# winlaic/ZipVoice

Hardware: AMD Instinct MI355X
Metric: generated mel-frames/s (whole job) + RTF, ZipVoice 123M N_steps=16 batch=32/GPU (higher is better)
Workload: dtype bf16; 1 GPU; C2: ZipVoice 123M, N_steps=16, batch=32/GPU x (3 s prompt + 10 s generated; T=1219 frames), CFG g=1.0 (64 decoder rows per GPU), t_shift=0.5; model=zipvoice (zipvoice_base.json, synthetic seeded weights), global_batch=32, seq_len=1219, parallelism=dp1

## Files before the change

### include/zipvoice_hip.h

```cpp
#ifndef ZIPVOICE_HIP_H
#define ZIPVOICE_HIP_H

#include <stdint.h>

#ifdef __cplusplus
extern "C" {
#endif

typedef struct zv_engine* zv_handle;

enum zv_variant { ZV_ZIPVOICE = 0, ZV_DISTILL = 1, ZV_DIALOG = 2, ZV_DIALOG_STEREO = 3 };
enum zv_precision { ZV_FP32 = 0, ZV_BF16 = 1, ZV_MIXED = 2, ZV_FP8 = 3 };

#define ZV_MAX_STACKS 8

typedef struct {
  int variant;
  int precision;
  int feat_dim;
  int num_stacks;
  int downsampling_factor[ZV_MAX_STACKS];
  int num_layers[ZV_MAX_STACKS];
  int cnn_module_kernel[ZV_MAX_STACKS];
  int fm_decoder_dim, fm_decoder_feedforward_dim, fm_decoder_num_heads;
  int text_encoder_num_layers, text_encoder_feedforward_dim, text_encoder_cnn_module_kernel;
  int text_encoder_num_heads, text_encoder_dim;
  int time_embed_dim, text_embed_dim;
  int query_head_dim, value_head_dim, pos_head_dim, pos_dim;
  int vocab_size, pad_id, spk_a_id, spk_b_id;
} zv_config;

const char* zv_last_error(void);
const char* zv_version(void);

zv_handle zv_create(const zv_config* cfg);
void zv_destroy(zv_handle h);

int zv_set_weight(zv_handle h, const char* name, const float* host_data, int64_t numel);
int zv_finalize(zv_handle h);
int zv_reserve(zv_handle h, int max_batch, int max_frames);
int64_t zv_device_bytes(zv_handle h);

int zv_profile(int enable);
int zv_profile_report(char* buf, int buflen);

int64_t zv_host_block_count(void);

int zv_attn_fallbacks(zv_handle h, int reset, int64_t* host_counts);

int zv_attn2_check(int kernel, int form, int B, int L, int H, int nv, const float* qkp, const float* P,
                   const uint8_t* key_pad, const float* v, const float* y, int force_exact, float* out,
                   int64_t* counts);

int zv_bench_gemm(int M, int N, int K, int variant, int iters, int out_mode, float* ms_out);

int zv_gemm_selftest(int M, int N, int K, int variant, int mode, float* maxdiff, float* maxref);

enum zv_linear_form {
  ZV_LIN_PLAIN = 0,
  ZV_LIN_PLAIN_F32 = 1,
  ZV_LIN_RESID = 2,
  ZV_LIN_RESID_BYP = 3,
  ZV_LIN_RESID_RV = 4,
  ZV_LIN_RESID_RV_COPY = 5,
  ZV_LIN_TRANS = 6,
  ZV_LIN_NA = 7,
  ZV_LIN_GLU = 8,
  ZV_LIN_GLU_DW = 9
};
typedef struct {
  int M, N, K, split, form, act;
  int rows_per_group;
  int rpb;
  int guard;
  const float* A; const float* W; const float* bias;
  const float* resid;
  const float* orig;
  const float* byp;
  const float* rowvec;
  const uint8_t* rowmask;
  const float* dw_w;
  const float* dw_b;
  int dw_ks, dw_L;
  float* C; int64_t ldc;
  uint16_t* Ch; uint16_t* Cl; int64_t ldch;
  uint16_t* Cth; uint16_t* Ctl; int64_t ldct;
  int launch[8];
  int num_cus;
} zv_linear_check_args;
int zv_linear_check(zv_linear_check_args* a);

typedef struct {
  int M, H, form, rows_per_group, part_slots, guard;
  float log_scale;
  const float* x; const float* W1; const float* b1; const float* W2; const float* b2;
  const float* resid;
  const float* rowvec;
  const float* orig;
  const float* byp;
  const float* nb;
  float* C; int64_t ldc;
  uint16_t* Ch; uint16_t* Cl; uint16_t* C2h; uint16_t* C2l; int64_t ldch;
  int launch[8];
  int num_cus;
} zv_ffn_check_args;
int zv_ffn_check(zv_ffn_check_args* a);

typedef struct {
  int B, L, C, ks, split, guard;
  const float* g; const float* w; const float* bias;
  int64_t ldin;
  uint16_t* Oh; uint16_t* Ol; int64_t ldout;
  uint8_t* q; uint8_t* qs; int64_t ldq;
  int launch[8];
  int num_cus;
} zv_dwconv_check_args;
int zv_dwconv_check(zv_dwconv_check_args* a);

enum zv_stackedge_kind { ZV_SE_DOWNSAMPLE = 0, ZV_SE_UPSAMPLE = 1, ZV_SE_MASK = 2, ZV_SE_ENTRY = 3, ZV_SE_BIASNORM = 4 };
typedef struct {
  int kind, B, L, C, ds, guard, rows_per_group;
  float log_scale;
  const float* x; const float* w; const float* nb; const float* orig; const float* rowvec;
  const uint8_t* mask;
  float* out;
  uint8_t* mout;
  uint16_t* h; uint16_t* l; uint16_t* h2; uint16_t* l2; int64_t ldact;
  uint8_t* q2; uint8_t* qs2; int64_t ldq;
  int launch[8];
  int num_cus;
} zv_stackedge_check_args;
int zv_stackedge_check(zv_stackedge_check_args* a);

enum zv_bigvgan_check_kind { ZV_BV_FILTER = 0, ZV_BV_ACT = 1, ZV_BV_CONV = 2, ZV_BV_CONVT = 3, ZV_BV_AVG = 4,
                             ZV_BV_POST = 5, ZV_BV_IM2COL = 6, ZV_BV_STEP = 7 };
typedef struct {
  int kind, split, mode, guard;
  int B, Lmax, Ls, halo, scale;
  int C, Cout, ks, d, u, n, layout, flag;
  float div, sub, bias0;
  unsigned stale;
  const int* lens;
  const float* x; const float* x1; const float* x2;
  const float* w; const float* bias; const float* alpha; const float* ibeta;
  const float* w2; const float* bias2; const float* alpha2; const float* ibeta2;
  const float* taps; const float* resid;
  const uint16_t* ah; const uint16_t* al;
  float* out; uint16_t* oh; uint16_t* ol; int64_t ld;
  int launch[8];
  int num_cus;
} zv_bigvgan_check_args;
int zv_bigvgan_check(zv_bigvgan_check_args* a);

int zv_attn_plan(int split, int sa_plo, int tpm, int L, int nv_na, int64_t* lds_sa, int64_t* lds_na,
                 int64_t* lds_stats, int* fits);

int zv_mx8_quantize(const float* x, int rows, int K, uint8_t* q, uint8_t* s);
int zv_mx8_gemm_check(int M, int N, int K, const float* A, const float* W, float* C, uint8_t* Aq,
                      uint8_t* As);

int zv_fm_decoder(zv_handle h, const float* t, const float* guidance, const float* xt,
                  const float* text_c, const float* speech_c, const uint8_t* pad, int N,
                  int T, int Fx, float* v_out, void* stream);

int zv_velocity(zv_handle h, float t, float guidance_scale, const float* x,
                const float* text_c, const float* speech_c, const uint8_t* pad, int B, int T,
                float* v_out, void* stream);

int zv_euler_sample(zv_handle h, float* x, const float* text_c, const float* speech_c,
                    const uint8_t* pad, int B, int T, int num_step, float guidance_scale,
                    float t_start, float t_end, float t_shift, void* stream);

int zv_velocity_rows(zv_handle h, float t, const float* guidance_rows, const float* x,
                     const float* text_c, const float* speech_c, const uint8_t* pad, int B,
                     int T, float* v_out, void* stream);
int zv_euler_sample_rows(zv_handle h, float* x, const float* text_c, const float* speech_c,
                         const uint8_t* pad, int B, int T, int num_step,
                         const float* guidance_rows, float t_start, float t_end,
                         float t_shift, void* stream);

int zv_text_encode(zv_handle h, const int64_t* tokens, const uint8_t* pad,
                   const int8_t* spk, int B, int S, float* out, void* stream);

int zv_text_condition(zv_handle h, const float* embed, int B, int S, const int32_t* tok_lens,
                      const int32_t* feat_lens, int T, float* out, void* stream);

int zv_speech_condition(zv_handle h, const float* prompt, int B, int Tp, int F,
                        const int32_t* prompt_lens, int T, float* out, void* stream);

typedef struct zv_vocoder* zv_vocoder_handle;

typedef struct {
  int precision;
  int n_mels;
  int dim;
  int intermediate_dim;
  int num_layers;
  int n_fft;
  int hop;
  int embed_kernel;
  int dw_kernel;
} zv_vocoder_config;

zv_vocoder_handle zv_vocoder_create(const zv_vocoder_config* cfg);
void zv_vocoder_destroy(zv_vocoder_handle v);
int zv_vocoder_set_weight(zv_vocoder_handle v, const char* name, const float* host_data,
                          int64_t numel);
int zv_vocoder_finalize(zv_vocoder_handle v);
int zv_vocoder_decode(zv_vocoder_handle v, const float* mel, int layout, float feat_scale,
                      float feat_bias, const int32_t* lens, int B, int T, float* wav, int clamp,
                      void* stream);
int64_t zv_vocoder_device_bytes(zv_vocoder_handle v);

typedef struct zv_bigvgan* zv_bigvgan_handle;

typedef struct {
  int precision;
  int num_mels;
  int upsample_initial_channel;
  int num_upsamples;
  int upsample_rates[8];
  int upsample_kernel_sizes[8];
  int num_kernels;
  int resblock_kernel_sizes[3];
  int resblock_dilation_sizes[3][3];
  int snake_logscale;
  int use_tanh_at_final;
  int use_bias_at_final;
} zv_bigvgan_config;

zv_bigvgan_handle zv_bigvgan_create(const zv_bigvgan_config* cfg);
void zv_bigvgan_destroy(zv_bigvgan_handle v);
int zv_bigvgan_set_weight(zv_bigvgan_handle v, const char* name, const float* host_data,
                          int64_t numel);
int zv_bigvgan_finalize(zv_bigvgan_handle v);
int zv_bigvgan_decode(zv_bigvgan_handle v, const float* mel, int layout, float feat_scale,
                      float feat_bias, const int32_t* lens, int B, int T, float* wav,
                      void* stream);
int64_t zv_bigvgan_device_bytes(zv_bigvgan_handle v);

typedef struct zv_fbank* zv_fbank_handle;
zv_fbank_handle zv_fbank_create(int n_fft, int hop, int n_mels, const float* host_window,
                                const float* host_fb);
void zv_fbank_destroy(zv_fbank_handle f);
int zv_fbank_configure(zv_fbank_handle f, int frame_offset, float mag_eps, float log_floor);
int zv_fbank_extract(zv_fbank_handle f, const float* wav, int64_t wav_ld, const int32_t* lens,
                     int B, int T_out, float* out, int64_t out_ld, void* stream);

typedef struct zv_resample* zv_resample_handle;
zv_resample_handle zv_resample_create(int o, int n, int S, const int32_t* host_start,
                                      const float* host_table);
void zv_resample_destroy(zv_resample_handle h);
int zv_resample_apply(zv_resample_handle h, const float* wav, int64_t wav_ld, const int32_t* lens,
                      int R, float* out, int64_t out_ld, int64_t out_cols, void* stream);
int64_t zv_resample_device_bytes(zv_resample_handle h);

typedef struct zv_wavjoin* zv_wavjoin_handle;
// ... 16 lines not shown
```

### zipvoice_amd/csrc/zv_checks.inc

```
#pragma once

namespace {

struct ChkDev {
  std::vector<void*> ptrs;
  void* raw(size_t bytes) {
    void* p = nullptr;
    ZV_CHECK(ZV_BLOCKING(hipMalloc(&p, bytes + 256)));
    ptrs.push_back(p);
    return p;
  }
  template <typename T> T* make(size_t n) { return reinterpret_cast<T*>(raw(n * sizeof(T))); }
  template <typename T> T* zero(size_t n) {
    T* d = make<T>(n);
    ZV_CHECK(ZV_BLOCKING(hipMemset(d, 0, n * sizeof(T))));
    return d;
  }
  template <typename T> T* up(const T* host, size_t n) {
    T* d = make<T>(n);
    ZV_CHECK(ZV_BLOCKING(hipMemcpy(d, host, n * sizeof(T), hipMemcpyHostToDevice)));
    return d;
  }
  template <typename T> void down(T* host, const T* dev, size_t n) {
    ZV_CHECK(ZV_BLOCKING(hipMemcpy(host, dev, n * sizeof(T), hipMemcpyDeviceToHost)));
// ... 302 lines not shown
  p.Bh = reinterpret_cast<const bf16*>(dWq); p.ldb = K; p.Bs = dWs; p.ldbs = K / MX8_BLOCK;
  p.bias = dev.zero<float>((size_t)N); p.C = dC; p.ldc = N; p.resid = dC; p.rows_per_group = 1; p.rpb = 1;
  launch_gemm<128, 128, 2, 2, 8, EPI_STD, 2, 2, MX8_KSTEP, 0, 0, 1>(p, 1, s, "mx8_check", true, -1);
  ZV_CHECK(ZV_BLOCKING(hipDeviceSynchronize()));
  dev.down(C, dC, (size_t)M * N);
  if (Aq) dev.down(Aq, dAq, (size_t)M * K);
  if (As) dev.down(As, dAs, (size_t)M * K / MX8_BLOCK);
  ZV_API_END
}

int zv_linear_check(zv_linear_check_args* a) {
  ZV_API_BEGIN
  ZV_REQUIRE(a && a->M > 0 && a->N > 0 && a->K > 0 && a->A && a->W && a->bias && a->guard >= 0 &&
                 (a->split == 1 || a->split == 2 || a->split == 3) && a->form >= ZV_LIN_PLAIN &&
                 a->form <= ZV_LIN_GLU_DW,
             "zv_linear_check: bad arguments");
  const int M = a->M, N = a->N, K = a->K, form = a->form, G = a->guard;
  const bool split3 = a->split == 3;
  const bool fused = form >= ZV_LIN_TRANS;
  const bool resid = form >= ZV_LIN_RESID && form <= ZV_LIN_RESID_RV_COPY;
  const bool rv = form == ZV_LIN_RESID_RV || form == ZV_LIN_RESID_RV_COPY;
  const bool wantC = form == ZV_LIN_PLAIN_F32 || (resid && form != ZV_LIN_RESID_RV_COPY);
  const bool wantT = form == ZV_LIN_TRANS || form == ZV_LIN_NA;
  ZV_REQUIRE(a->split != 2 || (form == ZV_LIN_PLAIN && !a->act) || form == ZV_LIN_TRANS,
             "zv_linear_check: split 2 is the plain form without activation, or TRANS");
  ZV_REQUIRE(wantC == (a->C != nullptr) && (!a->C || a->ldc >= N) && (!resid || a->resid) &&
                 (form != ZV_LIN_RESID_BYP || (a->orig && a->byp)) &&
                 (!rv || (a->rowvec && a->rows_per_group > 0)) && (form != ZV_LIN_RESID_RV_COPY || a->ldc >= N),
             "zv_linear_check: the form's fp32 operands");
  const bool glu = form == ZV_LIN_GLU || form == ZV_LIN_GLU_DW;
  const int wch = form == ZV_LIN_NA ? N / 3 : glu ? N / 2 : N;
  const bool needCh = form == ZV_LIN_PLAIN || form == ZV_LIN_RESID_RV_COPY || form == ZV_LIN_NA || glu;
  ZV_REQUIRE((!needCh || a->Ch) && (form != ZV_LIN_PLAIN_F32 || !a->Ch) && (form != ZV_LIN_TRANS || !a->Ch) &&
                 (!a->Ch || a->ldch >= wch) && (a->Cl != nullptr) == (split3 && a->Ch != nullptr),
             "zv_linear_check: the form's 16-bit outputs (Cl with split 3 only)");
  ZV_REQUIRE(wantT == (a->Cth != nullptr) && (!wantT || (a->rpb > 0 && a->ldct >= a->rpb)) &&
                 (a->Ctl != nullptr) == (split3 && wantT),
             "zv_linear_check: the transposed outputs");
  ZV_REQUIRE((form != ZV_LIN_NA || N % 48 == 0) && (!glu || N % 32 == 0), "zv_linear_check: NA / GLU widths");
  const int dwk = a->dw_ks;
  ZV_REQUIRE(form != ZV_LIN_GLU_DW || (a->dw_w && a->dw_b && a->dw_L > 0 && M % a->dw_L == 0),
             "zv_linear_check: GLU_DW needs the taps, the conv bias and whole utterances of dw_L rows");
  ZV_REQUIRE(form != ZV_LIN_GLU_DW || (a->split == 1 && N == 2 * 512 && (dwk == 7 || dwk == 15 || dwk == 31)),
             "zv_linear_check: GLU_DW is the 16-bit product at 512 channels with kernel size 7, 15 or 31");
  ZV_REQUIRE(form != ZV_LIN_GLU_DW || a->ldch % 8 == 0, "zv_linear_check: GLU_DW output rows of a multiple of 8 elements");

  LinearPolicy policy;
  WeightStore store;
  std::vector<int> perm(N);
  for (int n = 0; n < N; ++n) perm[n] = n;
  if (form == ZV_LIN_NA) perm = zv_engine::perm_na(N / 3);
  if (glu) perm = zv_engine::perm_glu(N / 2);
  std::vector<float> wp((size_t)N * K), bp(N);
  for (int n = 0; n < N; ++n) {
    memcpy(&wp[(size_t)n * K], a->W + (size_t)perm[n] * K, (size_t)K * sizeof(float));
    bp[n] = a->bias[perm[n]];
  }
  const Linear Lw = store.make_linear(wp.data(), N, K, bp.data());

  ChkDev dev;
  hipStream_t s = nullptr;
  Act A;
  {
    std::vector<bf16> h, l;
    A.ld = round_up(K, 64);
    chk_act(a->A, M, K, A.ld, split3, h, l);
    A.h = dev.up(h.data(), h.size());
    if (split3) A.l = dev.up(l.data(), l.size());
  }
  const long rows = (long)M + 2 * G;
  float* dC = nullptr;
  bf16 *dCh = nullptr, *dCl = nullptr, *dCth = nullptr, *dCtl = nullptr;
  const int nutt = wantT ? cdiv(M, a->rpb) : 0, rows_t = form == ZV_LIN_NA ? N / 3 : N;
  const long trows = wantT ? (long)nutt * rows_t + 2 * G : 0;
  if (a->C) {
    std::vector<float> hc(a->C, a->C + (size_t)rows * a->ldc);
    if (resid)
      for (long m = 0; m < M; ++m)
        memcpy(&hc[(size_t)(G + m) * a->ldc], a->resid + m * N, (size_t)N * sizeof(float));
    dC = dev.up(hc.data(), hc.size());
  }
  if (a->Ch) dCh = reinterpret_cast<bf16*>(dev.up(a->Ch, (size_t)rows * a->ldch));
  if (a->Cl) dCl = reinterpret_cast<bf16*>(dev.up(a->Cl, (size_t)rows * a->ldch));
  if (a->Cth) dCth = reinterpret_cast<bf16*>(dev.up(a->Cth, (size_t)trows * a->ldct));
  if (a->Ctl) dCtl = reinterpret_cast<bf16*>(dev.up(a->Ctl, (size_t)trows * a->ldct));
  const uint8_t* dmask = a->rowmask ? dev.up(a->rowmask, (size_t)M) : nullptr;

  if (!fused) {
    Out o;
    o.act_fn = a->act;
    if (dC) { o.C = dC + (size_t)G * a->ldc; o.ldc = a->ldc; }
    if (dCh) { o.act.h = dCh + (size_t)G * a->ldch; o.act.ld = a->ldch; }
    if (dCl) o.act.l = dCl + (size_t)G * a->ldch;
    if (resid) {
      if (o.C) {
        o.resid = o.C;
      } else {
        o.ldc = a->ldc;
        std::vector<float> r = chk_pad(a->resid, M, N, a->ldc);
        o.resid = dev.up(r.data(), r.size());
      }
    }
    if (form == ZV_LIN_RESID_BYP) {
      std::vector<float> og = chk_pad(a->orig, M, N, a->ldc);
      o.orig = dev.up(og.data(), og.size());
      o.byp = dev.up(a->byp, (size_t)N);
    }
    if (rv) {
      o.rowvec = dev.up(a->rowvec, (size_t)cdiv(M, a->rows_per_group) * N);
      o.rowvec_ld = N; o.rows_per_group = a->rows_per_group;
    }
    if (a->split == 2) policy.attn_in_wsplit(Lw, A, M, o, s);
    else if (split3) policy.linear16<3>(Lw, A, M, o, s);
    else policy.linear16<1>(Lw, A, M, o, s);
  } else {
    GemmParams p = LinearPolicy::gp_linear(Lw, A, M);
    if (a->split == 2) p.Al = nullptr;
    if (dCh) { p.Ch = dCh + (size_t)G * a->ldch; p.ldch = a->ldch; }
    if (dCl) p.Cl = dCl + (size_t)G * a->ldch;
    if (wantT) {
      p.Cth = dCth + (size_t)G * a->ldct;
      if (dCtl) p.Ctl = dCtl + (size_t)G * a->ldct;
      p.ldct = a->ldct; p.rpb = a->rpb; p.sCt = (long)rows_t * a->ldct;
    }
    if (glu) p.rowmask = dmask;
    if (form == ZV_LIN_GLU_DW) {
      p.dw_w = dev.up(a->dw_w, (size_t)(N / 2) * dwk); p.dw_b = dev.up(a->dw_b, (size_t)(N / 2));
      p.dw_out = p.Ch; p.ld_dw = p.ldch; p.dw_L = a->dw_L;
      ZV_REQUIRE(policy.glu_dw_fits(p, N / 2, dwk),
                 "zv_linear_check: GLU_DW operands (the engine would take the unfused pair)");
      policy.launch_glu_dw(p, dwk, s, "glu_dw_check");
    } else if (form == ZV_LIN_NA) {
      if (split3) policy.launch_na_in<3>(p, s); else policy.launch_na_in<1>(p, s);
    } else if (form == ZV_LIN_TRANS) {
      if (split3) policy.launch_value_t<3>(p, false, true, s);
      else policy.launch_value_t<1>(p, a->split == 2, Lw.lo != nullptr, s);
    } else {
      if (split3) policy.launch_glu_in<3>(p, false, s); else policy.launch_glu_in<1>(p, false, s);
    }
  }
  ZV_CHECK(ZV_BLOCKING(hipDeviceSynchronize()));
  chk_record(a->launch, &a->num_cus);
  if (a->C) dev.down(a->C, dC, (size_t)rows * a->ldc);
  if (a->Ch) dev.down(a->Ch, reinterpret_cast<uint16_t*>(dCh), (size_t)rows * a->ldch);
  if (a->Cl) dev.down(a->Cl, reinterpret_cast<uint16_t*>(dCl), (size_t)rows * a->ldch);
  if (a->Cth) dev.down(a->Cth, reinterpret_cast<uint16_t*>(dCth), (size_t)trows * a->ldct);
  if (a->Ctl) dev.down(a->Ctl, reinterpret_cast<uint16_t*>(dCtl), (size_t)trows * a->ldct);
  ZV_API_END
}

int zv_ffn_check(zv_ffn_check_args* a) {
  ZV_API_BEGIN
  ZV_REQUIRE(a && a->M > 0 && a->H > 0 && a->H % (2 * FFN_HC) == 0 && a->form >= 0 && a->form <= 3 &&
                 a->guard >= 0 && a->part_slots >= 0 && a->x && a->W1 && a->b1 && a->W2 && a->b2 &&
                 a->resid && a->C && a->ldc >= FFN_D && (!a->Ch || a->ldch >= FFN_D),
             "zv_ffn_check: bad arguments");
  const int M = a->M, H = a->H, form = a->form, G = a->guard, D = FFN_D;
  const bool norm = form == 3, byp = form == 2 || norm, rv = a->rowvec != nullptr;
  ZV_REQUIRE((form == 1) == (rv && !norm) || norm, "zv_ffn_check: the row vector belongs to form 1 (or 3)");
  ZV_REQUIRE((!rv || a->rows_per_group > 0) && (!byp || (a->orig && a->byp)) && (!norm || a->nb) &&
                 (form == 0 || a->Ch) && (norm || (!a->Cl && !a->C2h && !a->C2l)) &&
                 (!a->C2l || a->C2h),
             "zv_ffn_check: the form's operands");
  ZV_REQUIRE(a->part_slots <= zv_num_cus(), "zv_ffn_check: more lines than CUs");
  WeightStore store;
  const Linear L1 = store.make_linear(a->W1, H, D, a->b1);
  const Linear L2 = store.make_linear(a->W2, D, H, a->b2);
  ChkDev dev;
  hipStream_t s = nullptr;
  const long n = (long)H * D;
  bf16* w1f = dev.make<bf16>((size_t)n);
  bf16* w2f = dev.make<bf16>((size_t)n);
  ffn_pack_weights(L1, L2, H, w1f, w2f, s);
  FfnParams q{};
  q.H = H; q.nseg = 1;
  FfnSeg& g = q.seg[0];
  g.M = M;
  {
    std::vector<bf16> h, l;
    chk_act(a->x, M, D, D, false, h, l);
    g.X = dev.up(h.data(), h.size());
    q.ldx = D;
  }
  q.W1f = w1f; q.b1 = L1.b; q.W2f = w2f; q.b2 = L2.b;
  const long rows = (long)M + 2 * G;
  std::vector<float> hc(a->C, a->C + (size_t)rows * a->ldc);
  for (long m = 0; m < M; ++m)
    memcpy(&hc[(size_t)(G + m) * a->ldc], (norm ? a->orig : a->resid) + m * D, (size_t)D * sizeof(float));
  float* dC = dev.up(hc.data(), hc.size());
  g.C = dC + (size_t)G * a->ldc; q.ldc = a->ldc;
  auto padded = [&](const float* x) {
    std::vector<float> v = chk_pad(x, M, D, a->ldc);
    return dev.up(v.data(), v.size());
  };
  if (norm) { g.resid = padded(a->resid); g.orig = g.C; }
  else { g.resid = g.C; if (byp) g.orig = padded(a->orig); }
  if (byp) q.byp = dev.up(a->byp, (size_t)D);
  if (norm) { q.nb = dev.up(a->nb, (size_t)D); q.log_scale = a->log_scale; }
  if (rv) {
    g.rowvec = dev.up(a->rowvec, (size_t)cdiv(M, a->rows_per_group) * D);
    q.rowvec_ld = D; q.rows_per_group = a->rows_per_group;
  }
  uint16_t* host16[4] = {a->Ch, a->Cl, a->C2h, a->C2l};
  bf16* dev16[4] = {};
  for (int i = 0; i < 4; ++i)
    if (host16[i]) dev16[i] = reinterpret_cast<bf16*>(dev.up(host16[i], (size_t)rows * a->ldch));
  q.ldch = a->Ch ? a->ldch : 0;
  auto inner = [&](bf16* p) { return p ? p + (size_t)G * a->ldch : nullptr; };
  g.Ch = inner(dev16[0]); g.Cl = inner(dev16[1]); g.C2h = inner(dev16[2]); g.C2l = inner(dev16[3]);
  if (a->part_slots > 0) {
    q.part_slots = a->part_slots;
    q.part = dev.zero<float>((size_t)a->part_slots * FFN_PART_FLOATS);
    q.flag = dev.zero<unsigned>((size_t)a->part_slots + 64);
  }
  ZV_CHECK(ZV_BLOCKING(hipDeviceSynchronize()));
  launch_ffn(q, s, norm ? "ffn_norm_check" : "ffn_check");
  ZV_CHECK(ZV_BLOCKING(hipDeviceSynchronize()));
  chk_record(a->launch, &a->num_cus);
  volatile unsigned* e = zv_dev_err_host();
  if (*e != 0) {
    *e = 0;
    throw std::runtime_error("zv_ffn_check: the device error word was set (a C item outwaited its producer)");
  }
  dev.down(a->C, dC, (size_t)rows * a->ldc);
  for (int i = 0; i < 4; ++i)
    if (host16[i]) dev.down(host16[i], reinterpret_cast<uint16_t*>(dev16[i]), (size_t)rows * a->ldch);
  ZV_API_END
}

int zv_dwconv_check(zv_dwconv_check_args* a) {
  ZV_API_BEGIN
  ZV_REQUIRE(a && a->B > 0 && a->L > 0 && a->C > 0 && a->ks > 0 && (a->split == 1 || a->split == 3) &&
                 a->guard >= 0 && a->g && a->w && a->bias && a->Oh && a->ldin >= a->C && a->ldout >= a->C,
             "zv_dwconv_check: bad arguments");
  ZV_REQUIRE((a->Ol != nullptr) == (a->split == 3), "zv_dwconv_check: Ol with split 3 only");
  ZV_REQUIRE(!a->q || (a->qs && a->ldq >= a->C && a->ldq % MX8_KSTEP == 0),
             "zv_dwconv_check: the fp8 copy needs its scales and a row stride that is a multiple of 128");
  const int B = a->B, L = a->L, C = a->C, G = a->guard;
  const long M = (long)B * L, rows = M + 2 * G;
  const bool split3 = a->split == 3;
  ChkDev dev;
  hipStream_t s = nullptr;
  std::vector<bf16> h, l;
  chk_act(a->g, M, C, a->ldin, split3, h, l);
  const bf16* ih = dev.up(h.data(), h.size());
  const bf16* il = split3 ? dev.up(l.data(), l.size()) : nullptr;
  const float* w = dev.up(a->w, (size_t)C * a->ks);
  const float* bias = dev.up(a->bias, (size_t)C);
  bf16* dOh = reinterpret_cast<bf16*>(dev.up(a->Oh, (size_t)rows * a->ldout));
  bf16* dOl = split3 ? reinterpret_cast<bf16*>(dev.up(a->Ol, (size_t)rows * a->ldout)) : nullptr;
  const long ldqs = a->ldq / MX8_BLOCK;
  uint8_t* dq = a->q ? dev.up(a->q, (size_t)rows * a->ldq) : nullptr;
  uint8_t* dqs = a->q ? dev.up(a->qs, (size_t)rows * ldqs) : nullptr;
  launch_dwconv(ih, il, a->ldin, w, bias, dOh + (size_t)G * a->ldout, dOl ? dOl + (size_t)G * a->ldout : nullptr,
                a->ldout, B, L, C, a->ks, s, dq ? dq + (size_t)G * a->ldq : nullptr,
                dqs ? dqs + (size_t)G * ldqs : nullptr, a->ldq);
  ZV_CHECK(ZV_BLOCKING(hipDeviceSynchronize()));
  chk_record(a->launch, &a->num_cus);
  dev.down(a->Oh, reinterpret_cast<uint16_t*>(dOh), (size_t)rows * a->ldout);
  if (dOl) dev.down(a->Ol, reinterpret_cast<uint16_t*>(dOl), (size_t)rows * a->ldout);
  if (dq) {
    dev.down(a->q, dq, (size_t)rows * a->ldq);
    dev.down(a->qs, dqs, (size_t)rows * ldqs);
  }
  ZV_API_END
}

int zv_stackedge_check(zv_stackedge_check_args* a) {
  ZV_API_BEGIN
  ZV_REQUIRE(a && a->kind >= ZV_SE_DOWNSAMPLE && a->kind <= ZV_SE_BIASNORM && a->B > 0 && a->L > 0 &&
                 a->guard >= 0 && (a->kind == ZV_SE_MASK || (a->C > 0 && a->C % 4 == 0 && a->x)),
             "zv_stackedge_check: bad arguments");
  const int kind = a->kind, B = a->B, L = a->L, C = a->C, ds = a->ds, G = a->guard;
  const bool resample = kind <= ZV_SE_MASK;
  ZV_REQUIRE(!resample || ds >= 1, "zv_stackedge_check: the downsampling factor");
  const int dL = resample ? (L + ds - 1) / ds : 0;
  const long M = (long)B * L, Md = (long)B * dL;
  ChkDev dev;
  hipStream_t s = nullptr;
  EdgeLaunch ran{};
  auto up32 = [&](long n, const float* fill) {
    std::vector<float> hc(a->out, a->out + (size_t)(n + 2 * G) * C);
    if (fill) memcpy(&hc[(size_t)G * C], fill, (size_t)n * C * sizeof(float));
    return dev.up(hc.data(), hc.size());
  };
  auto up16 = [&](uint16_t* p, long n) {
    return p ? reinterpret_cast<bf16*>(dev.up(p, (size_t)(n + 2 * G) * a->ldact)) : nullptr;
  };
  auto in16 = [&](bf16* p) { return p ? p + (size_t)G * a->ldact : nullptr; };
  auto down16 = [&](uint16_t* p, bf16* d, long n) {
    if (p) dev.down(p, reinterpret_cast<uint16_t*>(d), (size_t)(n + 2 * G) * a->ldact);
  };
  if (kind == ZV_SE_DOWNSAMPLE) {
    ZV_REQUIRE(a->w && a->out, "zv_stackedge_check: downsample needs the weights and out");
    const float* in = dev.up(a->x, (size_t)M * C);
    const float* w = dev.up(a->w, (size_t)ds);
    float* d = up32(Md, nullptr);
    ran = launch_downsample(in, d + (size_t)G * C, B, L, dL, C, ds, w, s);
    ZV_CHECK(ZV_BLOCKING(hipDeviceSynchronize()));
    dev.down(a->out, d, (size_t)(Md + 2 * G) * C);
  } else if (kind == ZV_SE_UPSAMPLE) {
    ZV_REQUIRE(a->w && a->orig && a->out, "zv_stackedge_check: upsample needs the scale, orig and out");
    const float* d = dev.up(a->x, (size_t)Md * C);
    const float* sc = dev.up(a->w, (size_t)C);
    float* o = up32(M, a->orig);
    float* main = o + (size_t)G * C;
    ran = launch_upsample_combine(main, d, sc, main, B, L, dL, C, ds, s);
    ZV_CHECK(ZV_BLOCKING(hipDeviceSynchronize()));
    dev.down(a->out, o, (size_t)(M + 2 * G) * C);
  } else if (kind == ZV_SE_MASK) {
    ZV_REQUIRE(a->mask && a->mout, "zv_stackedge_check: the mask and its output");
    const uint8_t* in = dev.up(a->mask, (size_t)M);
    uint8_t* o = dev.up(a->mout, (size_t)(Md + 2 * G));
    ran = launch_mask_downsample(in, o + G, B, L, dL, ds, s);
    ZV_CHECK(ZV_BLOCKING(hipDeviceSynchronize()));
    dev.down(a->mout, o, (size_t)(Md + 2 * G));
  } else if (kind == ZV_SE_ENTRY) {
    ZV_REQUIRE(a->h && a->h2 && a->ldact >= C && a->ldact % 4 == 0 && (!a->rowvec || a->rows_per_group > 0),
               "zv_stackedge_check: stack entry writes h (src) and h2 (cur), rows of a multiple of 4");
    const float* src = dev.up(a->x, (size_t)M * C);
    const float* rv = a->rowvec ? dev.up(a->rowvec, (size_t)cdiv(M, a->rows_per_group) * C) : nullptr;
    float* cur = a->out ? up32(M, nullptr) : nullptr;
    bf16 *h = up16(a->h, M), *l = up16(a->l, M), *h2 = up16(a->h2, M), *l2 = up16(a->l2, M);
    ran = launch_stack_entry(src, rv, cur ? cur + (size_t)G * C : nullptr, in16(h), in16(l), in16(h2), in16(l2),
                             a->ldact, M, C, rv ? a->rows_per_group : 1, s);
    ZV_CHECK(ZV_BLOCKING(hipDeviceSynchronize()));
    if (cur) dev.down(a->out, cur, (size_t)(M + 2 * G) * C);
    down16(a->h, h, M); down16(a->l, l, M); down16(a->h2, h2, M); down16(a->l2, l2, M);
  } else {
    ZV_REQUIRE(a->nb && a->w && a->orig && a->out && a->h && a->ldact >= C && a->ldact % 4 == 0 &&
                   (!a->l2 || a->h2) && (!a->rowvec || a->rows_per_group > 0),
// ... 298 lines not shown
```

### zipvoice_amd/csrc/zv_engine.hip

```cpp
#include <math.h>
#include <stdlib.h>
#include <string.h>

#include <map>
#include <memory>
#include <mutex>
#include <string>
#include <exception>
#include <functional>
#include <tuple>
#include <vector>


#include "zv_common.h"
#include "zv_gemm.inc"
#include "zv_gemm256.inc"
#include "zv_ffn.inc"
#include "zv_attn.inc"
#include "zv_elem.inc"
#include "zv_flash.inc"
#include "zv_flash2.inc"
#include "zv_weights.inc"
#include "zv_linear.inc"
#include "../../include/zipvoice_hip.h"

static thread_local std::string g_last_error;
ZvProfiler g_zv_prof;

namespace {

struct LayerW {
  Linear attn_in;
  float* pos_w = nullptr;
  Linear sa_in[2], sa_out[2];
  Linear ff_in[3], ff_out[3];
  bf16* ffn_w1f[3] = {nullptr, nullptr, nullptr};
  bf16* ffn_w2f[3] = {nullptr, nullptr, nullptr};
  Linear na_in, na_out;
  Linear conv_in[2], conv_out[2];
  Linear conv_sa_out[2];
  float* dw_w[2] = {nullptr, nullptr};
  float* dw_b[2] = {nullptr, nullptr};
  int ks = 0;
  float* bypass = nullptr;
  float* bypass_mid = nullptr;
  float* norm_bias = nullptr;
  float norm_log_scale = 0.f;
};

struct StackW {
  int ds = 1;
  std::vector<LayerW> layers;
  float* pos_w_all = nullptr;
  Linear time_emb;
  float* ds_w = nullptr;
  float* combiner = nullptr;
};

struct ZipformerW {
  int dim = 0, ff = 0, heads = 0, qd = 0, pd = 0, vd = 0, pos_dim = 0, temb_dim = -1;
  std::vector<Linear> in_proj, out_proj;
  std::vector<StackW> stacks;
  bool has_time = false, has_guid = false;
  Linear te0, te2, guid;
  bool b2 = false;
};

static unsigned long g_ws_generation = 0;

struct DBuf {
  void* p = nullptr;
  size_t bytes = 0;
  template <typename T> T* get(size_t n) {
    size_t need = n * sizeof(T) + 256;
    if (need > bytes) {
      ++g_ws_generation;
      if (p) { ZV_CHECK(ZV_BLOCKING(hipDeviceSynchronize())); ZV_CHECK(ZV_BLOCKING(hipFree(p))); }
      ZV_CHECK(ZV_BLOCKING(hipMalloc(&p, need)));
      ZV_CHECK(ZV_BLOCKING(hipMemset(p, 0, need)));
      ZV_CHECK(ZV_BLOCKING(hipDeviceSynchronize()));
      bytes = need;
    }
    return reinterpret_cast<T*>(p);
  }
  ~DBuf() { if (p) (void)ZV_BLOCKING(hipFree(p)); }
};

struct ActBuf {
  DBuf h, l, q, qs;
  Act get(long rows, long ld, bool split, bool fp8 = false, long cols = 0, bool with16 = true) {
    Act a;
    a.ld = ld;
    a.h = with16 ? h.get<bf16>((size_t)rows * ld) : nullptr;
    a.l = split ? l.get<bf16>((size_t)rows * ld) : nullptr;
    if (fp8) {
      a.ldq = round_up(cols ? cols : ld, MX8_KSTEP);
      a.q = q.get<uint8_t>((size_t)rows * a.ldq);
      a.qs = qs.get<uint8_t>((size_t)rows * a.ldq / MX8_BLOCK);
    }
    return a;
  }
  size_t bytes() const { return h.bytes + l.bytes + q.bytes + qs.bytes; }
};

struct Workspace {
  DBuf main, dsrc, cur, temb0, temb1, tstack, tvec, gvec, posP, mask2, maskds, vout, stats;
  ActBuf xin, main_a, dsrc_a, cur_a, qkp, W, hidden, na_y, na_xt, na_o, sa_vt, sa_o, glu, dw, emb;
  ActBuf cur8;
  ActBuf dwo;
  DBuf ffn_part, ffn_flag;
  static constexpr int POSP_STACKS = 8;
  DBuf posPs[POSP_STACKS];
  struct PosPKey { int L = -1, nl = 0; const void* w = nullptr; const void* buf = nullptr; };
  PosPKey posk[POSP_STACKS];
  size_t bytes() const {
    size_t s = 0;
    for (const DBuf& b : posPs) s += b.bytes;
    for (const DBuf* b : {&main, &dsrc, &cur, &temb0, &temb1, &tstack, &tvec, &gvec, &posP, &mask2,
                          &maskds, &vout, &stats, &ffn_part, &ffn_flag})
      s += b->bytes;
    for (const ActBuf* b : {&xin, &main_a, &dsrc_a, &cur_a, &qkp, &W, &hidden, &na_y, &na_xt, &na_o,
                            &sa_vt, &sa_o, &glu, &dw, &emb, &cur8, &dwo})
      s += b->bytes();
    return s;
  }
};

struct Pass {
  bool io_split = false;
  bool posp_reuse = false;
  long batch_rows = 0;
};

constexpr int ZV_STREAM_SET = 4;
struct StreamSet { hipStream_t s[ZV_STREAM_SET] = {}; int dev = -1; };
static std::mutex g_stream_pool_mu;
static std::vector<StreamSet>& stream_pool_free() { static std::vector<StreamSet> v; return v; }
static StreamSet acquire_stream_set() {
  int dev = 0;
  ZV_CHECK(hipGetDevice(&dev));
  {
    std::lock_guard<std::mutex> lock(g_stream_pool_mu);
    auto& fr = stream_pool_free();
    for (size_t i = 0; i < fr.size(); ++i)
      if (fr[i].dev == dev) {
        StreamSet set = fr[i];
        fr.erase(fr.begin() + i);
        return set;
      }
  }
  StreamSet set;
  set.dev = dev;
  for (int i = 0; i < ZV_STREAM_SET; ++i)
    ZV_CHECK(ZV_BLOCKING(hipStreamCreateWithFlags(&set.s[i], hipStreamNonBlocking)));
  return set;
}
static void release_stream_set(const StreamSet& set) {
  if (set.dev < 0) return;
  for (hipStream_t st : set.s)
    if (st) (void)ZV_BLOCKING(hipStreamSynchronize(st));
  std::lock_guard<std::mutex> lock(g_stream_pool_mu);
  stream_pool_free().push_back(set);
}

}

struct zv_engine : LinearPolicy {
  zv_config cfg;
  WeightStore store;
  ZipformerW dec, txt;
  float* embed_table = nullptr;
  float* spk_table = nullptr;
  float* temb_freqs = nullptr;
  Workspace ws_dec, ws_txt;
  static constexpr int MAX_SPLIT = 4;
  Workspace ws_split[MAX_SPLIT - 1];
  int split_streams = 3;
  long split_min_rows = 0;
  hipStream_t split_stream[MAX_SPLIT - 1] = {};
  hipEvent_t split_fork = nullptr, split_join[MAX_SPLIT - 1] = {};

  bool materialize_attn = false;
  int ffn_fused = 2;
  long ffn_min_rows = 15000;
  int fp8_fuse = 7;
  int sa_tp = 1;
  bool mixed_sa = true;
  bool attn_b2 = false, attn_b2_dec = false;
  int attn2_exact = 0;
  int glu_dw = 1;
  unsigned* attn_fallback = nullptr;

  explicit zv_engine(const zv_config& c) : cfg(c) {
    auto envi = [](const char* k, int d) { const char* v = getenv(k); return v ? atoi(v) : d; };
    materialize_attn = envi("ZV_ATTN_MATERIALIZE", 0) == 1;
    graph_mode = envi("ZV_GRAPH", 2);
    sa_tp = envi("ZV_SA_TP", 1);
    fp8_fuse = envi("ZV_FP8_FUSE", 7);
    ffn_fused = envi("ZV_FFN", 2);
    ffn_min_rows = envi("ZV_FFN_MIN_ROWS", 15000);
    ffn_persist = envi("ZV_FFN_PERSIST", 1);
    split_streams = envi("ZV_SPLIT_STREAMS", 3);
    split_min_rows = envi("ZV_SPLIT_MIN_ROWS", 8192);
    mixed_sa = envi("ZV_MIXED_SA", 1) != 0;
    attn_b2 = envi("ZV_ATTN2", 1) != 0 && (cfg.precision == ZV_BF16 || cfg.precision == ZV_FP8);
    attn_b2_dec = attn_b2 || (envi("ZV_ATTN2", 1) != 0 && cfg.precision == ZV_MIXED);
    attn2_exact = envi("ZV_ATTN2_EXACT", 0) != 0;
    glu_dw = envi("ZV_GLU_DW", 1);
  }
  struct GraphKey {
    int B, T, N, has_pad;
    float g, t0, t1, shift;
    int cfg_mode;
    unsigned long gen;
    bool operator<(const GraphKey& o) const {
      return std::tie(B, T, N, has_pad, g, t0, t1, shift, cfg_mode, gen) <
             std::tie(o.B, o.T, o.N, o.has_pad, o.g, o.t0, o.t1, o.shift, o.cfg_mode, o.gen);
    }
  };
  static constexpr size_t MAX_GRAPHS = 8, MAX_SEEN = 256;
  struct GraphEntry { hipGraphExec_t exec; unsigned long last_use; };
  std::map<GraphKey, GraphEntry> graphs;
  std::map<GraphKey, int> graph_seen;
  unsigned long graph_clock = 0;
  hipStream_t gstream = nullptr;
  hipEvent_t gev_in = nullptr, gev_out = nullptr;
  DBuf gx, gtc, gsc, gpad, ggrows;
  int graph_mode = 2;

  int ffn_persist = 1;
  void attach_ffn_scratch(FfnParams& q, Workspace& ws) {
    if (!ffn_persist) return;
    const int cus = zv_num_cus();
    q.part = ws.ffn_part.get<float>((size_t)cus * FFN_PART_FLOATS);
    unsigned* fl = ws.ffn_flag.get<unsigned>((size_t)cus + 64);
    q.flag = fl;
    q.part_slots = cus;
  }
  void ffn_site(FfnParams q, Workspace& ws, hipStream_t s, const char* tag) {
    attach_ffn_scratch(q, ws);
    launch_ffn(q, s, tag);
  }

  void check_dev_err() {
    volatile unsigned* e = zv_dev_err_host();
    if (*e == 0) return;
    ZV_CHECK(ZV_BLOCKING(hipDeviceSynchronize()));
    auto clear = [](Workspace& w) {
      if (w.ffn_flag.p) ZV_CHECK(ZV_BLOCKING(hipMemset(w.ffn_flag.p, 0, w.ffn_flag.bytes)));
    };
    clear(ws_dec); clear(ws_txt);
    for (Workspace& w : ws_split) clear(w);
    ZV_CHECK(ZV_BLOCKING(hipDeviceSynchronize()));
    *e = 0;
    throw std::runtime_error("fused FeedForward: a C item waited more than 2 s for its producer's tiles; "
                             "the outputs of the calls since the previous one are invalid (schedule flags reset)");
  }

  void drop_graphs() {
    for (auto& kv : graphs) (void)ZV_BLOCKING(hipGraphExecDestroy(kv.second.exec));
    graphs.clear();
  }
  void evict_lru_graph() {
    auto victim = graphs.begin();
    for (auto it = graphs.begin(); it != graphs.end(); ++it)
      if (it->second.last_use < victim->second.last_use) victim = it;
    ZV_CHECK(ZV_BLOCKING(hipStreamSynchronize(gstream)));
    ZV_CHECK(ZV_BLOCKING(hipGraphExecDestroy(victim->second.exec)));
    graphs.erase(victim);
  }

  StreamSet streams;
  hipStream_t engine_stream(int slot) {
    static_assert(MAX_SPLIT <= ZV_STREAM_SET, "stream set holds the split streams and the graph stream");
    if (streams.dev < 0) streams = acquire_stream_set();
    if (!streams.s[slot]) ZV_CHECK(ZV_BLOCKING(hipStreamCreateWithFlags(&streams.s[slot], hipStreamNonBlocking)));
    return streams.s[slot];
  }

  ~zv_engine() {
    drop_graphs();
    release_stream_set(streams);
    if (gev_in) (void)ZV_BLOCKING(hipEventDestroy(gev_in));
    if (gev_out) (void)ZV_BLOCKING(hipEventDestroy(gev_out));
    for (int i = 0; i < MAX_SPLIT - 1; ++i)
      if (split_join[i]) (void)ZV_BLOCKING(hipEventDestroy(split_join[i]));
    if (split_fork) (void)ZV_BLOCKING(hipEventDestroy(split_fork));
  }

  Linear make_linear(const std::string& prefix, int N, int K, bool bias, bool keep_f32,
                     const std::vector<int>* perm = nullptr, bool fp8 = false) {
    const auto& w = store.take(prefix + ".weight", (size_t)N * K);
    const std::vector<float>* b = bias ? &store.take(prefix + ".bias", N) : nullptr;
    std::vector<float> wp, bp;
    if (perm) {
      wp.resize((size_t)N * K);
      for (int n = 0; n < N; ++n)
        memcpy(&wp[(size_t)n * K], &w[(size_t)(*perm)[n] * K], (size_t)K * sizeof(float));
      if (b) {
        bp.resize(N);
        for (int n = 0; n < N; ++n) bp[n] = (*b)[(*perm)[n]];
      }
    }
    const float* rows = perm ? wp.data() : w.data();
    Linear L = store.make_linear(rows, N, K, !b ? nullptr : perm ? bp.data() : b->data());
    if (fp8 && cfg.precision == ZV_FP8 && K % MX8_KSTEP == 0) {
      L.Kq = K;
      std::vector<float> wz((size_t)L.Npad * K, 0.f);
      memcpy(wz.data(), rows, (size_t)N * K * sizeof(float));
      std::vector<uint8_t> q((size_t)L.Npad * K), sc((size_t)L.Npad * K / MX8_BLOCK);
      mx8_quantize_host(wz.data(), K, L.Npad, K, q.data(), K, sc.data());
      L.q8 = store.upload(q.data(), q.size());
      L.s8 = store.upload(sc.data(), sc.size());
    }
    if (keep_f32) L.w32 = store.upload(w.data(), (size_t)N * K);
    return L;
  }
  Linear make_linear_kcat(const std::string& pa, int Ka, const std::string& pb, int Kb, int N,
                          bool b_split = false) {
    const int K = Ka + (b_split ? 3 : 1) * Kb;
    const auto& wa = store.take(pa + ".weight", (size_t)N * Ka);
    const auto& wb = store.take(pb + ".weight", (size_t)N * Kb);
    std::vector<float> w((size_t)N * K);
    for (int n = 0; n < N; ++n) {
      float* row = &w[(size_t)n * K];
      memcpy(row, &wa[(size_t)n * Ka], (size_t)Ka * sizeof(float));
      for (int blk = 0; Ka + blk * Kb < K; ++blk)
        for (int k = 0; k < Kb; ++k) {
          const float v = wb[(size_t)n * Kb + k];
          row[Ka + blk * Kb + k] = blk == 2 ? v - (float)(bf16)v : v;
        }
    }
    const auto& ba = store.take(pa + ".bias", N);
    const auto& bb = store.take(pb + ".bias", N);
    std::vector<float> b(N);
    for (int n = 0; n < N; ++n) b[n] = ba[n] + bb[n];
    return store.make_linear(w.data(), N, K, b.data());
  }
  static std::vector<int> perm_na(int hid) {
    std::vector<int> p(3 * hid);
    for (int g = 0; g < hid / 16; ++g)
      for (int i = 0; i < 16; ++i) {
        p[g * 48 + i] = g * 16 + i;
        p[g * 48 + 16 + i] = hid + g * 16 + i;
        p[g * 48 + 32 + i] = 2 * hid + g * 16 + i;
      }
    return p;
  }
  static std::vector<int> perm_glu(int C) {
    std::vector<int> p(2 * C);
    for (int g = 0; g < C / 16; ++g)
      for (int i = 0; i < 16; ++i) {
        p[g * 32 + i] = g * 16 + i;
        p[g * 32 + 16 + i] = C + g * 16 + i;
      }
    return p;
  }
  std::string stage_rows_scaled(const std::string& prefix, int N, int K, int r0, int r1, float f) {
    std::vector<float> w = store.take(prefix + ".weight", (size_t)N * K), b = store.take(prefix + ".bias", N);
    for (int n = r0; n < r1; ++n) {
      for (int k = 0; k < K; ++k) w[(size_t)n * K + k] *= f;
      b[n] *= f;
    }
    const std::string np = prefix + "#b2";
    store.derived[np + ".weight"] = std::move(w);
    store.derived[np + ".bias"] = std::move(b);
    return np;
  }
  std::string stage_value_heads16(const std::string& prefix, int heads, int vd, int K) {
    const auto& w = store.take(prefix + ".weight", (size_t)heads * vd * K);
    const auto& b = store.take(prefix + ".bias", (size_t)heads * vd);
    std::vector<float> w2((size_t)heads * 16 * K, 0.f), b2((size_t)heads * 16, 0.f);
    for (int h = 0; h < heads; ++h) {
      for (int d = 0; d < vd; ++d) {
        memcpy(&w2[(size_t)(h * 16 + d) * K], &w[(size_t)(h * vd + d) * K], (size_t)K * sizeof(float));
        b2[h * 16 + d] = b[h * vd + d];
      }
      b2[h * 16 + 12] = 1.f;
    }
    const std::string np = prefix + "#v16";
    store.derived[np + ".weight"] = std::move(w2);
    store.derived[np + ".bias"] = std::move(b2);
    return np;
  }
  Linear make_small(const std::string& prefix, int N, int K, bool bias) {
    Linear L;
    L.N = N; L.K = K;
    L.w32 = store.upload_key(prefix + ".weight", (size_t)N * K);
    if (bias) L.b = store.upload_key(prefix + ".bias", N);
    return L;
  }

  void build_zipformer(ZipformerW& Z, const std::string& pre, int dim, int ff, int heads,
                       const std::vector<int>& ds, const std::vector<int>& layers,
                       const std::vector<int>& ks, std::vector<int> in_dims,
                       std::vector<int> out_dims, bool two_stream, int temb_dim, bool guid,
                       bool is_decoder = false, bool b2 = false) {
    Z.dim = dim; Z.ff = ff; Z.heads = heads; Z.b2 = b2;
    Z.qd = cfg.query_head_dim; Z.pd = cfg.pos_head_dim; Z.vd = cfg.value_head_dim;
    Z.pos_dim = cfg.pos_dim; Z.temb_dim = temb_dim;
    ZV_REQUIRE(Z.qd == ATT_QD && Z.pd == ATT_PD, "engine supports query_head_dim=32, pos_head_dim=4");
    ZV_REQUIRE(Z.pos_dim % 2 == 0 && Z.pos_dim <= POSP_MAXD, "pos_dim must be even and <= 64");
    ZV_REQUIRE(heads * Z.vd <= 64, "num_heads * value_head_dim must be <= 64");
    for (size_t i = 0; i < in_dims.size(); ++i) {
      std::string s = two_stream ? "." + std::to_string(i) : "";
      Z.in_proj.push_back(make_linear(pre + "in_proj" + s, dim, in_dims[i], true, false));
      Z.out_proj.push_back(make_linear(pre + "out_proj" + s, out_dims[i], dim, true, false));
    }
    const int qkp = (2 * Z.qd + Z.pd) * heads;
    for (size_t s = 0; s < ds.size(); ++s) {
      StackW S;
      S.ds = ds[s];
      std::string sp = pre + "encoders." + std::to_string(s) + ".";
      std::string ep = S.ds != 1 ? sp + "encoder." : sp;
      if (S.ds != 1) {
        ZV_REQUIRE(S.ds <= 8, "downsampling factor > 8 unsupported");
        const auto& b = store.take(sp + "downsample.bias", S.ds);
        float mx = -INFINITY;
        for (float v : b) mx = std::max(mx, v);
        std::vector<float> w(S.ds);
        float sum = 0.f;
        for (int k = 0; k < S.ds; ++k) { w[k] = expf(b[k] - mx); sum += w[k]; }
        for (int k = 0; k < S.ds; ++k) w[k] /= sum;
        S.ds_w = store.dalloc<float>(S.ds);
        ZV_CHECK(ZV_BLOCKING(hipMemcpy(S.ds_w, w.data(), S.ds * sizeof(float), hipMemcpyHostToDevice)));
        S.combiner = store.upload_key(sp + "out_combiner.bypass_scale", dim);
      }
      if (temb_dim > 0) S.time_emb = make_small(ep + "time_emb.1", dim, temb_dim, true);
      const size_t pw_n = (size_t)heads * Z.pd * Z.pos_dim;
      S.pos_w_all = store.dalloc<float>(pw_n * std::max(layers[s], 1));
      for (int li = 0; li < layers[s]; ++li) {
        std::string lp = ep + "layers." + std::to_string(li) + ".";
        LayerW W;
        W.attn_in = make_linear(b2 ? stage_rows_scaled(lp + "self_attn_weights.in_proj", qkp, dim,
                                                            heads * Z.qd, qkp, 1.4426950408889634f)
                                        : lp + "self_attn_weights.in_proj",
                                qkp, dim, true, false);
        {
          const auto& pw = store.take(lp + "self_attn_weights.linear_pos.weight", pw_n);
          W.pos_w = S.pos_w_all + li * pw_n;
          ZV_CHECK(ZV_BLOCKING(hipMemcpy(W.pos_w, pw.data(), pw_n * sizeof(float), hipMemcpyHostToDevice)));
        }
        for (int a = 0; a < 2; ++a) {
          std::string ap = lp + "self_attn" + std::to_string(a + 1) + ".";
          if (b2) {
            ZV_REQUIRE(Z.vd <= 12, "value_head_dim <= 12 for the padded value heads");
            W.sa_in[a] = make_linear(stage_value_heads16(ap + "in_proj", heads, Z.vd, dim), heads * 16, dim,
                                     true, false);
          } else {
            W.sa_in[a] = make_linear(ap + "in_proj", heads * Z.vd, dim, true, false);
          }
          W.sa_out[a] = make_linear(ap + "out_proj", dim, heads * Z.vd, true, false);
        }
        const int hs[3] = {ff * 3 / 4, ff, ff * 5 / 4};
        for (int f = 0; f < 3; ++f) {
          std::string fp = lp + "feed_forward" + std::to_string(f + 1) + ".";
          W.ff_in[f] = make_linear(fp + "in_proj", hs[f], dim, true, false, nullptr, is_decoder);
          W.ff_out[f] = make_linear(fp + "out_proj", dim, hs[f], true, false, nullptr, is_decoder);
          if (ffn_fused && is_decoder && dim == FFN_D && hs[f] % (2 * FFN_HC) == 0 &&
              (cfg.precision == ZV_BF16 || cfg.precision == ZV_MIXED)) {
            const long n = (long)hs[f] * FFN_D;
            W.ffn_w1f[f] = store.dalloc<bf16>(n);
            W.ffn_w2f[f] = store.dalloc<bf16>(n);
            ffn_pack_weights(W.ff_in[f], W.ff_out[f], hs[f], W.ffn_w1f[f], W.ffn_w2f[f], nullptr);
            ZV_CHECK(ZV_BLOCKING(hipDeviceSynchronize()));
          }
        }
        const int hid = 3 * dim / 4;
        ZV_REQUIRE(hid % 16 == 0 && dim % 64 == 0, "encoder dim must be a multiple of 64");
        const std::vector<int> pna = perm_na(hid), pglu = perm_glu(dim);
        W.na_in = make_linear(lp + "nonlin_attention.in_proj", 3 * hid, dim, true, false, &pna);
        W.na_out = make_linear(lp + "nonlin_attention.out_proj", dim, hid, true, false, nullptr, is_decoder);
        W.ks = ks[s];
        for (int c = 0; c < 2; ++c) {
          std::string cp = lp + "conv_module" + std::to_string(c + 1) + ".";
          W.conv_in[c] = make_linear(cp + "in_proj", 2 * dim, dim, true, false, &pglu, is_decoder);
          W.conv_out[c] = make_linear(cp + "out_proj", dim, dim, true, false, nullptr, is_decoder);
          if (is_decoder && (cfg.precision == ZV_BF16 || cfg.precision == ZV_MIXED))
            W.conv_sa_out[c] = make_linear_kcat(cp + "out_proj", dim,
                                                lp + "self_attn" + std::to_string(c + 1) + ".out_proj",
                                                heads * Z.vd, dim, cfg.precision == ZV_MIXED && mixed_sa);
          W.dw_w[c] = store.upload_key(cp + "depthwise_conv.weight", (size_t)dim * W.ks);
          W.dw_b[c] = store.upload_key(cp + "depthwise_conv.bias", dim);
        }
        W.bypass = store.upload_key(lp + "bypass.bypass_scale", dim);
        W.bypass_mid = store.upload_key(lp + "bypass_mid.bypass_scale", dim);
        W.norm_bias = store.upload_key(lp + "norm.bias", dim);
        W.norm_log_scale = store.take(lp + "norm.log_scale", 1)[0];
        S.layers.push_back(std::move(W));
      }
      Z.stacks.push_back(std::move(S));
    }
    if (temb_dim > 0) {
      Z.has_time = true;
      Z.te0 = make_small(pre + "time_embed.0", 2 * temb_dim, temb_dim, true);
      Z.te2 = make_small(pre + "time_embed.2", temb_dim, 2 * temb_dim, true);
      if (guid) {
        Z.has_guid = true;
        Z.guid = make_small(pre + "guidance_scale_embed", temb_dim, temb_dim, false);
      }
    }
  }

  bool stereo() const { return cfg.variant == ZV_DIALOG_STEREO; }
  bool distill() const { return cfg.variant == ZV_DISTILL; }
  bool dialog() const { return cfg.variant == ZV_DIALOG || cfg.variant == ZV_DIALOG_STEREO; }

  void finalize() {
    const int F = cfg.feat_dim;
    std::vector<int> ds, nl, ks;
    for (int s = 0; s < cfg.num_stacks; ++s) {
      ds.push_back(cfg.downsampling_factor[s]);
      nl.push_back(cfg.num_layers[s]);
      ks.push_back(cfg.cnn_module_kernel[s]);
    }
    std::vector<int> in_dims = stereo() ? std::vector<int>{5 * F, 3 * F} : std::vector<int>{3 * F};
    std::vector<int> out_dims = stereo() ? std::vector<int>{2 * F, F} : std::vector<int>{F};
    build_zipformer(dec, "fm_decoder.", cfg.fm_decoder_dim, cfg.fm_decoder_feedforward_dim,
                    cfg.fm_decoder_num_heads, ds, nl, ks, in_dims, out_dims, stereo(),
                    cfg.time_embed_dim, distill(), true, attn_b2_dec);
    build_zipformer(txt, "text_encoder.", cfg.text_encoder_dim, cfg.text_encoder_feedforward_dim,
                    cfg.text_encoder_num_heads, {1}, {cfg.text_encoder_num_layers},
                    {cfg.text_encoder_cnn_module_kernel}, {cfg.text_embed_dim}, {F}, false, -1,
                    false, attn_b2);
    embed_table = store.upload_key("embed.weight", (size_t)cfg.vocab_size * cfg.text_embed_dim);
    if (dialog()) spk_table = store.upload_key("spk_embed.weight", (size_t)2 * F);
    const int half = cfg.time_embed_dim / 2;
    std::vector<float> fr(half);
    for (int k = 0; k < half; ++k)
      fr[k] = expf((float)(-log(10000.0)) * (float)k / (float)half);
    temb_freqs = store.dalloc<float>(half);
    ZV_CHECK(ZV_BLOCKING(hipMemcpy(temb_freqs, fr.data(), half * sizeof(float), hipMemcpyHostToDevice)));
    attn_fallback = store.dalloc<unsigned>(4);
    ZV_CHECK(ZV_BLOCKING(hipMemset(attn_fallback, 0, 4 * sizeof(unsigned))));
    size_t expected = count_expected();
    if (expected != store.staged.size())
      throw std::invalid_argument("state dict has " + std::to_string(store.staged.size()) +
                                  " tensors, config expects " + std::to_string(expected) +
                                  " (unexpected keys present)");
    store.staged.clear();
    store.derived.clear();
    store.ready = true;
  }

  size_t count_expected() const {
    auto zf = [&](const ZipformerW& Z) {
      size_t n = 4 * Z.in_proj.size();
      for (const auto& S : Z.stacks) {
        if (S.ds != 1) n += 2;
        if (Z.temb_dim > 0) n += 2;
        n += S.layers.size() * 43;
      }
      if (Z.has_time) n += 4;
      if (Z.has_guid) n += 1;
      return n;
    };
    return zf(dec) + zf(txt) + 1 + (dialog() ? 1 : 0);
  }

  void small_linear(const Linear& L, const float* in, int ldin, int M, float* out, int ldout,
                    int pre, const float* add, hipStream_t s) {
    if (M > 0 && L.K <= 8192) {
      hipLaunchKernelGGL(zv_small_linear_rows_kernel, dim3((unsigned)M, (unsigned)cdiv(L.N, SL_NB)), dim3(256),
                         (size_t)L.K * sizeof(float), s,
                         in, ldin, L.w32, L.K, L.b, add, out, ldout, M, L.N, L.K, pre);
    } else {
      const long n = (long)M * L.N;
      hipLaunchKernelGGL(zv_small_linear_kernel, dim3((unsigned)cdiv(n, 4L)), dim3(256), 0, s, in, ldin, L.w32,
                         L.K, L.b, add, out, ldout, M, L.N, L.K, pre);
    }
    ZV_LAUNCH_CHECK();
  }

  bool fp8_mode() const { return cfg.precision == ZV_FP8; }

  template <int SPLIT, int TPM>
  static void attn_na_v1(const FlashParams& f, int hid, hipStream_t s) {
    constexpr int QTILES = SPLIT == 3 ? 4 : 8;
    if (hid <= 128) launch_attn_na<SPLIT, 1, QTILES, TPM>(f, s);
    else if (hid <= 256) launch_attn_na<SPLIT, 2, QTILES, TPM>(f, s);
    else launch_attn_na<SPLIT, 3, QTILES, TPM>(f, s);
  }
  template <int SPLIT>
  void attn_na(const FlashParams& f, int hid, bool a2, bool tp_na, hipStream_t s) {
    if constexpr (SPLIT == 1) {
      if (a2) return launch_attn_na_b2(f, hid, na_b2_form(f.L), s);
      if (tp_na) return attn_na_v1<1, 1>(f, hid, s);
    }
    attn_na_v1<SPLIT, 0>(f, hid, s);
  }
  template <int SPLIT>
  void attn_sa(const FlashParams& f, bool a2, hipStream_t s) {
    if constexpr (SPLIT == 1) {
      if (a2) return launch_attn_sa_b2(f, sa_b2_form(f.L), s);
      if (sa_tp) {
        if (sa_tp == 3) launch_attn_sa_tp<0, 1>(f, s);
        else launch_attn_sa_tp<0>(f, s);
        return;
      }
    }
    launch_attn_sa<SPLIT>(f, s);
  }

  template <int SPLIT>
  void layer(const Pass& pass, const ZipformerW& Z, const LayerW& W, Workspace& ws, float* src,
             Act src_a, float* cur, Act cur_a, int B, int L, const uint8_t* pad, const float* posP,
             const float* temb, bool has_next, hipStream_t s, bool fresh8 = false) {
    const bool split = SPLIT == 3;
    const long M = (long)B * L;
    const long Mtot = pass.batch_rows > 0 ? pass.batch_rows * (long)L : M;
    const int D = Z.dim, H = Z.heads;
    const long Lpad = round_up(L, 64);
    const char* tag_att = split ? "gemm_attn_fp32" : "gemm_attn_bf16";
    const int qkpN = W.attn_in.N;
    Act qkp = ws.qkp.get(M, qkpN, split);
    {
      Out o; o.act = qkp;
      if (SPLIT == 1 && pass.io_split) attn_in_wsplit(W.attn_in, src_a, M, o, s);
      else linear<SPLIT>(W.attn_in, src_a, M, o, s);
    }
    const bool tp_na = SPLIT == 1 && sa_tp;
    const int sa_plo = (SPLIT == 1 && sa_tp) ? 0 : -1;
    const bool a2 = SPLIT == 1 && Z.b2;
    const bool materialize = materialize_attn || (a2 ? !fused_attn2_fits(L, W.na_in.N / 3)
                                                     : !fused_attn_fits<SPLIT>(L, W.na_in.N / 3, sa_plo, tp_na ? 1 : 0));
    Act Wt;
    FlashParams fp{};
    if (materialize) {
      Wt = ws.W.get((long)H * M, Lpad, split);
      AttnParams ap{qkp.h, qkp.l, qkpN, posP, pad, Wt.h, Wt.l, Lpad, B, L, H, a2 ? 1 : 0};
      launch_attn_softmax<SPLIT>(ap, s);
    } else {
      fp.qh = qkp.h; fp.ql = qkp.l; fp.ldq = qkpN; fp.P = posP; fp.key_pad = pad;
      fp.B = B; fp.L = L; fp.H = H;
      fp.force_exact = attn2_exact; fp.fallback = attn_fallback;
      if (!a2) {
        fp.stats = ws.stats.get<float2>((size_t)M);
        if constexpr (SPLIT == 1)
          if (tp_na) launch_attn_stats<1, 1>(fp, s);
          else launch_attn_stats<1>(fp, s);
        else launch_attn_stats<SPLIT>(fp, s);
      }
    }
    const bool f8 = SPLIT == 1 && fp8_mode() && W.ff_in[0].q8 != nullptr;
    Act c8;
    if (f8) {
      c8 = ws.cur8.get(M, D, false, true, D, false);
      cur_a.q = c8.q; cur_a.qs = c8.qs; cur_a.ldq = c8.ldq;
      if (!fresh8 || !(fp8_fuse & 4)) pack8(cur_a, M, D, s);
    }
    Out res;
    res.C = cur; res.ldc = D; res.resid = cur; res.act = cur_a;
    auto ffn_params = [&](int f) {
      FfnParams q{};
      q.H = W.ff_in[f].N; q.nseg = 1;
      q.seg[0].M = (int)M; q.seg[0].X = cur_a.h; q.ldx = cur_a.ld;
      q.W1f = W.ffn_w1f[f]; q.b1 = W.ff_in[f].b; q.W2f = W.ffn_w2f[f]; q.b2 = W.ff_out[f].b;
      return q;
    };
    auto ff = [&](int f, const Out& oe) {
      if constexpr (SPLIT == 1) {
        if (ffn_fused && W.ffn_w1f[f] && !(f8 && W.ff_in[f].q8) && oe.C && oe.resid &&
            !oe.act.l && !oe.residh && Mtot >= ffn_min_rows && cur_a.ld % 8 == 0) {
          FfnParams q = ffn_params(f);
          FfnSeg& g = q.seg[0];
          g.resid = oe.resid; g.C = oe.C; q.ldc = oe.ldc; g.Ch = oe.act.h; q.ldch = oe.act.ld;
          g.rowvec = oe.rowvec; q.rowvec_ld = oe.rowvec_ld; q.rows_per_group = oe.rows_per_group;
          g.orig = oe.orig; q.byp = oe.byp;
          ffn_site(q, ws, s, "ffn_bf16");
          return;
        }
      }
      const bool f8f = f8 && W.ff_in[f].q8 && W.ff_out[f].q8;
      Act hid = ws.hidden.get(M, W.ff_in[f].N, split, f8f, W.ff_in[f].N, !f8f);
      Out o1; o1.act = hid; o1.act_fn = 1;
      linear<SPLIT>(W.ff_in[f], cur_a, M, o1, s);
      linear<SPLIT>(W.ff_out[f], hid, M, oe, s);
    };
    {
      Out e1 = res;
      e1.resid = src;
      if (temb) { e1.rowvec = temb; e1.rowvec_ld = D; e1.rows_per_group = L; }
      ff(0, e1);
    }
    {
      const int hid = W.na_in.N / 3;
      Act y = ws.na_y.get(M, hid, split);
      Act xt = ws.na_xt.get((long)B * hid, Lpad, split);
      GemmParams p = gp_linear(W.na_in, cur_a, M);
      p.Ch = y.h; p.Cl = y.l; p.ldch = y.ld;
      p.Cth = xt.h; p.Ctl = xt.l; p.ldct = Lpad; p.rpb = L; p.sCt = (long)hid * Lpad;
      launch_na_in<SPLIT>(p, s);
      Act nao = ws.na_o.get(M, round_up(hid, 64), split, f8, hid);
      if (materialize) {
        GemmParams q{};
        q.M = L; q.N = hid; q.K = L; q.nz2 = B; q.Brows = hid;
        q.Ah = Wt.h; q.Al = Wt.l; q.lda = Lpad; q.sA2 = (long)L * Lpad;
        q.Bh = xt.h; q.Bl = xt.l; q.ldb = Lpad; q.sB2 = (long)hid * Lpad;
        q.Ch = nao.h; q.Cl = nao.l; q.ldch = nao.ld; q.sCh2 = (long)L * nao.ld;
        q.mulh = y.h; q.mull = y.l; q.ldmul = y.ld; q.smul2 = (long)L * y.ld;
        q.rows_per_group = 1; q.rpb = 1;
        launch_gemm<128, 128, 2, 2, SPLIT, EPI_STD>(q, B, s, tag_att);
      } else {
        FlashParams f = fp;
        f.vh = xt.h; f.vl = xt.l; f.ldv = Lpad; f.sv_b = (long)hid * Lpad; f.vrows_per_head = 0;
        f.nv = hid;
        f.mulh = y.h; f.mull = y.l; f.ldmul = y.ld;
        f.oh = nao.h; f.ol = nao.l; f.ldo = nao.ld; f.ocol_per_head = 0;
        attn_na<SPLIT>(f, hid, a2, tp_na, s);
      }
      if (f8) pack8(nao, M, hid, s);
      linear<SPLIT>(W.na_out, nao, M, res, s);
    }
    const bool kcat = SPLIT == 1 && !f8 && temb && W.conv_sa_out[0].hi &&
                      !materialize && (W.conv_sa_out[0].K == D + H * Z.vd || sa_tp);
    Act dwo;
    if (kcat) dwo = ws.dwo.get(M, round_up(W.conv_sa_out[0].K, 64), false);
    const bool sa_split = kcat && pass.io_split && W.conv_sa_out[0].K == D + 3 * H * Z.vd;
    ZV_REQUIRE(!kcat || sa_split || W.conv_sa_out[0].K == D + H * Z.vd, "conv + SelfAttention out-projection width");
    auto self_attn = [&](int a) {
      const int vd = Z.vd, HV = H * vd;
      const int VR = W.sa_in[a].N, vph = VR / H;
      Act vt = ws.sa_vt.get((long)B * VR, Lpad, split);
      Act o = ws.sa_o.get(M, 64, split);
      if (kcat) { o = dwo; o.h += D; }
      GemmParams p = gp_linear(W.sa_in[a], cur_a, M);
      p.Cth = vt.h; p.Ctl = vt.l; p.ldct = Lpad; p.rpb = L; p.sCt = (long)VR * Lpad;
      launch_value_t<SPLIT>(p, sa_split, W.sa_in[a].lo != nullptr, s);
      if (materialize) {
        GemmParams q{};
        q.M = L; q.N = vd; q.K = L; q.nz2 = B; q.Brows = vd;
        q.Ah = Wt.h; q.Al = Wt.l; q.lda = Lpad; q.sA1 = M * Lpad; q.sA2 = (long)L * Lpad;
        q.Bh = vt.h; q.Bl = vt.l; q.ldb = Lpad; q.sB1 = (long)vph * Lpad; q.sB2 = (long)VR * Lpad;
        q.Ch = o.h; q.Cl = o.l; q.ldch = o.ld; q.sCh1 = vd; q.sCh2 = (long)L * o.ld;
        q.rows_per_group = 1; q.rpb = 1;
        launch_gemm<128, 16, 4, 1, SPLIT, EPI_STD>(q, H * B, s, tag_att);
      } else {
        FlashParams f = fp;
        f.vh = vt.h; f.vl = vt.l; f.ldv = Lpad; f.sv_b = (long)VR * Lpad; f.vrows_per_head = vph;
        f.nv = vd;
        f.oh = o.h; f.ol = o.l; f.ldo = o.ld; f.ocol_per_head = vd;
        if (sa_split) { f.ol = o.h + HV; f.oh2 = o.h + 2 * HV; }
        attn_sa<SPLIT>(f, a2, s);
      }
      Out e = res;
      if (temb) { e.rowvec = temb; e.rowvec_ld = D; e.rows_per_group = L; }
      if (kcat) e.C = nullptr;
      linear<SPLIT>(W.sa_out[a], o, M, e, s);
    };
    auto conv = [&](int c) {
      const bool g8 = f8 && W.conv_in[c].q8;
      Act dw = kcat ? dwo : ws.dw.get(M, D, split, f8, D);
      bool fused = false;
      if constexpr (SPLIT == 1) {
        if (glu_dw && !f8) {
          GemmParams p = gp_linear(W.conv_in[c], cur_a, M);
          p.Ch = dw.h; p.ldch = dw.ld; p.rowmask = pad;
          p.dw_w = W.dw_w[c]; p.dw_b = W.dw_b[c]; p.dw_out = dw.h; p.ld_dw = dw.ld; p.dw_L = L;
          fused = glu_dw_fits(p, D, W.ks);
          if (fused) launch_glu_dw(p, W.ks, s, "gemm_bf16_glu_dw");
        }
      }
      if (!fused) {
        Act g = ws.glu.get(M, D, split);
        GemmParams p = g8 ? gp_linear8(W.conv_in[c], cur_a, M) : gp_linear(W.conv_in[c], cur_a, M);
        p.Ch = g.h; p.Cl = g.l; p.ldch = g.ld; p.rowmask = pad;
        launch_glu_in<SPLIT>(p, g8, s);
        const bool dq = f8 && (fp8_fuse & 2);
        launch_dwconv(g.h, g.l, g.ld, W.dw_w[c], W.dw_b[c], dw.h, dw.l, dw.ld, B, L, D, W.ks, s,
                      dq ? dw.q : nullptr, dw.qs, dw.ldq);
        if (f8 && !dq) pack8(dw, M, D, s);
      }
      if (kcat) {
        Out e = res;
        e.rowvec = temb; e.rowvec_ld = D; e.rows_per_group = L;
        linear<SPLIT>(W.conv_sa_out[c], dw, M, e, s);
      } else {
        linear<SPLIT>(W.conv_out[c], dw, M, res, s);
      }
    };
    self_attn(0);
    conv(0);
    {
      Out e = res; e.byp = W.bypass_mid;
      e.orig = src;
      ff(1, e);
    }
    self_attn(1);
    conv(1);
    const bool ffn_norm = SPLIT == 1 && ffn_fused >= 2 && W.ffn_w1f[2] && !f8 && D == FFN_D &&
                          Mtot >= ffn_min_rows && cur_a.ld == src_a.ld && cur_a.ld % 8 == 0;
    if (ffn_norm) {
      FfnParams q = ffn_params(2);
      FfnSeg& g = q.seg[0];
      g.resid = cur; g.orig = src; g.C = src; q.ldc = D;
      g.Ch = src_a.h; g.Cl = src_a.l; q.ldch = src_a.ld;
      q.byp = W.bypass; q.nb = W.norm_bias; q.log_scale = W.norm_log_scale;
      g.rowvec = temb; q.rowvec_ld = D; q.rows_per_group = L;
      g.C2h = has_next ? cur_a.h : nullptr; g.C2l = has_next ? cur_a.l : nullptr;
      ffn_site(q, ws, s, "ffn_norm_bf16");
    } else {
      Out e = res;
      e.act = Act{};
      ff(2, e);
    }
    if (!ffn_norm) {
      const bool q2 = f8 && has_next && (fp8_fuse & 4);
      ZV_REQUIRE(!q2 || D % 256 == 0, "fp8 BiasNorm copy: channels a multiple of 256");
      launch_biasnorm_bypass(cur, src, W.norm_bias, W.norm_log_scale, W.bypass, src, src_a.h, src_a.l,
                             has_next ? cur_a.h : nullptr, has_next ? cur_a.l : nullptr, D, temb, L, M, D,
                             q2 ? c8.q : nullptr, q2 ? c8.qs : nullptr, q2 ? c8.ldq : 0L, s);
    }
  }

  template <int SPLIT>
  void stack(const Pass& pass, const ZipformerW& Z, const StackW& S, int si, Workspace& ws, float* src,
             Act src_a, int B, int L, const uint8_t* pad, const float* temb, hipStream_t s) {
    const long M = (long)B * L;
    const bool split = SPLIT == 3;
    float* cur = ws.cur.get<float>(M * Z.dim);
    Act cur_a = ws.cur_a.get(M, Z.dim, split);
    launch_stack_entry(src, temb, nullptr, src_a.h, src_a.l, cur_a.h, cur_a.l, Z.dim, M, Z.dim, L, s);
    const int R = 2 * L - 1, HPD = Z.heads * Z.pd, nl = (int)S.layers.size();
    const size_t pn = (size_t)std::max(nl, 1) * R * HPD;
    const bool own = si >= 0 && si < Workspace::POSP_STACKS;
    float* posP = own ? ws.posPs[si].get<float>(pn) : ws.posP.get<float>(pn);
    bool reuse = false;
    if (own) {
      Workspace::PosPKey& k = ws.posk[si];
      reuse = pass.posp_reuse && k.L == L && k.nl == nl && k.w == S.pos_w_all && k.buf == posP;
      k = Workspace::PosPKey{L, nl, S.pos_w_all, posP};
    }
    if (!reuse) {
      hipLaunchKernelGGL(zv_posp_kernel, dim3((unsigned)cdiv((long)nl * R * HPD, 256L)), dim3(256), 0, s, S.pos_w_all, posP,
                         L, nl, HPD, Z.pos_dim);
      ZV_LAUNCH_CHECK();
    }
    for (size_t li = 0; li < S.layers.size(); ++li)
      layer<SPLIT>(pass, Z, S.layers[li], ws, src, src_a, cur, cur_a, B, L, pad,
                   posP + li * (size_t)R * HPD, temb, li + 1 < S.layers.size(), s, li > 0);
  }

  template <int SPLIT>
  void zipformer(const Pass& pass, const ZipformerW& Z, Workspace& ws, Act xin, int sidx, int N,
                 int T, const uint8_t* pad, const float* t, const float* g, float* out, hipStream_t s) {
    const long M = (long)N * T;
    const int D = Z.dim;
    const bool split = SPLIT == 3;
    float* main = ws.main.get<float>(M * D);
    const bool ios = SPLIT == 1 && pass.io_split;
    Act main_a = ws.main_a.get(M, D, split || ios);
    {
      Out o; o.C = main; o.ldc = D;
      if (ios) linear<3>(Z.in_proj[sidx], xin, M, o, s);
      else linear<SPLIT>(Z.in_proj[sidx], xin, M, o, s);
    }
    float* tstack = nullptr;
    if (Z.has_time) {
      const int E = Z.temb_dim;
      float* e0 = ws.temb0.get<float>((size_t)N * 2 * E);
      float* e1 = ws.temb1.get<float>((size_t)N * 2 * E);
      hipLaunchKernelGGL(zv_timestep_embed_kernel, grid1d(N * E), dim3(256), 0, s, t, temb_freqs,
                         e0, N, E);
      ZV_LAUNCH_CHECK();
      if (Z.has_guid) {
        hipLaunchKernelGGL(zv_timestep_embed_kernel, grid1d(N * E), dim3(256), 0, s, g,
                           temb_freqs, e1, N, E);
        ZV_LAUNCH_CHECK();
        small_linear(Z.guid, e1, E, N, e0, E, 0, e0, s);
      }
      small_linear(Z.te0, e0, E, N, e1, 2 * E, 0, nullptr, s);
      small_linear(Z.te2, e1, 2 * E, N, e0, E, 1, nullptr, s);
      tstack = ws.tstack.get<float>(Z.stacks.size() * (size_t)N * D);
      for (size_t si = 0; si < Z.stacks.size(); ++si)
        small_linear(Z.stacks[si].time_emb, e0, E, N, tstack + si * (size_t)N * D, D, 1, nullptr,
                     s);
    }
    for (size_t si = 0; si < Z.stacks.size(); ++si) {
      const StackW& S = Z.stacks[si];
      const float* te = tstack ? tstack + si * (size_t)N * D : nullptr;
      if (S.ds == 1) {
        stack<SPLIT>(pass, Z, S, (int)si, ws, main, main_a, N, T, pad, te, s);
      } else {
        const int dL = (T + S.ds - 1) / S.ds;
        float* d = ws.dsrc.get<float>((size_t)N * dL * D);
        Act d_a = ws.dsrc_a.get((long)N * dL, D, split || ios);
        launch_downsample(main, d, N, T, dL, D, S.ds, S.ds_w, s);
        uint8_t* pds = nullptr;
        if (pad) {
          pds = ws.maskds.get<uint8_t>((size_t)N * dL);
          launch_mask_downsample(pad, pds, N, T, dL, S.ds, s);
        }
        stack<SPLIT>(pass, Z, S, (int)si, ws, d, d_a, N, dL, pds, te, s);
        launch_upsample_combine(main, d, S.combiner, main, N, T, dL, D, S.ds, s);
      }
    }
    ZV_REQUIRE(Z.stacks.back().ds == 1, "last stack must have downsampling factor 1");
    {
      Out o; o.C = out; o.ldc = Z.out_proj[sidx].N;
      if (ios) linear<3>(Z.out_proj[sidx], main_a, M, o, s);
      else linear<SPLIT>(Z.out_proj[sidx], main_a, M, o, s);
    }
  }

  Act build_xin(Workspace& ws, const float* x, const float* tc, const float* sc, int B, int T,
                int Fx, int copies, int zero_speech, hipStream_t s) {
    const int Ft = cfg.feat_dim, Fin = 2 * Fx + Ft;
    const bool split = cfg.precision == ZV_FP32 || cfg.precision == ZV_MIXED;
    const long N = (long)copies * B;
    Act xin = ws.xin.get(N * T, round_up(Fin, 64), split);
    if (Fx % 4 == 0 && Ft % 4 == 0 && xin.ld % 4 == 0)
      hipLaunchKernelGGL(zv_build_input4_kernel, grid1d(N * T * Fin / 4), dim3(256), 0, s, x, tc, sc,
                         xin.h, xin.l, xin.ld, B, T, Fx, Ft, Fx, copies, zero_speech);
    else
      hipLaunchKernelGGL(zv_build_input_kernel, grid1d(N * T * Fin), dim3(256), 0, s, x, tc, sc,
                         xin.h, xin.l, xin.ld, B, T, Fx, Ft, Fx, copies, zero_speech);
    ZV_LAUNCH_CHECK();
    return xin;
  }

  void decoder_rows(const Pass& pass, Workspace& ws, Act xin, int sidx, int N, int T,
                    const uint8_t* pad, const float* t, const float* g, float* out, hipStream_t s) {
    if (cfg.precision == ZV_FP32) zipformer<3>(pass, dec, ws, xin, sidx, N, T, pad, t, g, out, s);
    else zipformer<1>(pass, dec, ws, xin, sidx, N, T, pad, t, g, out, s);
  }

  bool cfg_doubles(float g, const float* grows, bool cfg_rows) const {
    return !distill() && (grows ? cfg_rows : g != 0.0f);
  }
  bool splits_rows(long N, int T) const { return split_streams >= 2 && N >= 2 && N * T >= split_min_rows; }

  void decoder(Act xin, int Fin, int N, int T, const uint8_t* pad, const float* t, const float* g,
               float* out, bool posp_reuse, hipStream_t s) {
    int sidx = 0;
    if (stereo()) sidx = (Fin == dec.in_proj[0].K) ? 0 : 1;
    ZV_REQUIRE(Fin == dec.in_proj[sidx].K, "decoder input width does not match in_proj");
    Pass pass;
    pass.io_split = cfg.precision == ZV_MIXED;
    pass.posp_reuse = posp_reuse;
    if (!splits_rows(N, T)) {
      decoder_rows(pass, ws_dec, xin, sidx, N, T, pad, t, g, out, s);
      return;
    }
    const int parts = std::min(split_streams, std::min(N, MAX_SPLIT));
    if (!split_fork) {
      ZV_CHECK(ZV_BLOCKING(hipEventCreateWithFlags(&split_fork, hipEventDisableTiming)));
      for (int i = 0; i < MAX_SPLIT - 1; ++i)
        ZV_CHECK(ZV_BLOCKING(hipEventCreateWithFlags(&split_join[i], hipEventDisableTiming)));
    }
    for (int i = 1; i < parts; ++i)
      if (!split_stream[i - 1]) split_stream[i - 1] = engine_stream(i - 1);
    const int outN = dec.out_proj[sidx].N;
// ... 628 lines not shown
```

### zipvoice_amd/csrc/zv_ffn.inc

```
#pragma once
#include <cstddef>
#include "zv_gemm256.inc"
#include "zv_weights.inc"

typedef unsigned v4u32_t __attribute__((ext_vector_type(4)));
typedef unsigned v2u32_t __attribute__((ext_vector_type(2)));
constexpr int FFN_D = 512, FFN_BM = 128, FFN_HC = 32, FFN_SLOT = 32768, FFN_MAXSEG = 4;
constexpr long FFN_PART_FLOATS = (long)FFN_BM * FFN_D;

struct FfnSeg {
  int M, rb0;
  const bf16* X;
  const float* resid; float* C;
  bf16* Ch;
  const float* rowvec;
  const float* orig;
  bf16* Cl; bf16* C2h; bf16* C2l;
};

struct FfnParams {
  int H;
  int R, nseg;
  FfnSeg seg[FFN_MAXSEG];
  long ldx, ldc, ldch, rowvec_ld; int rows_per_group;
  const bf16* W1f; const float* b1;
  const bf16* W2f; const float* b2;
  const float* byp;
  const float* nb; float log_scale;
  float norm_scale;
  float* sink;
  int w;
  float* part; unsigned* flag; int part_slots;
  unsigned* err;
  unsigned long long* dbg;
};

#ifndef FFN_NORM_LDS
#define FFN_NORM_LDS 1
#endif
#ifndef FFN_XOVL
#define FFN_XOVL 1
#endif
constexpr int FFN_NCONST = 3 * FFN_D + 4 * 2 * FFN_D;
inline size_t ffn_lds_bytes(int H, bool norm = false) {
  return 4 * FFN_SLOT + ((size_t)H + FFN_HC) * 4 +
         (norm && FFN_NORM_LDS ? FFN_NCONST * 4 : 0);
}

#ifdef ZV_OPERAND_F16
#define FFN_MFMA "v_mfma_f32_32x32x16_f16"
#else
#define FFN_MFMA "v_mfma_f32_32x32x16_bf16"
#endif
#ifndef FFN_BIAS_ACC
#define FFN_BIAS_ACC 1
#endif
__device__ __forceinline__ void ffn_mma_v0(f32x16& acc, const bf16x8& a, const bf16x8& b) {
  asm volatile(FFN_MFMA " %0, %1, %2, 0" : "=&v"(acc) : "v"(a), "v"(b));
}
__device__ __forceinline__ void ffn_mma_v(f32x16& acc, const bf16x8& a, const bf16x8& b) {
  asm volatile(FFN_MFMA " %0, %1, %2, %0" : "+v"(acc) : "v"(a), "v"(b));
}
#ifndef FFN_OUT_ASM
#define FFN_OUT_ASM 1
#endif
__device__ __forceinline__ void ffn_mma_a(f32x16& acc, const bf16x8& a, const bf16x8& b) {
#if FFN_OUT_ASM
  asm volatile(FFN_MFMA " %0, %1, %2, %0" : "+a"(acc) : "v"(a), "v"(b));
#else
  acc = ZV_MFMA_32x32x16(a, b, acc, 0, 0, 0);
#endif
}
struct FfnAct { float t, m, q; };
__device__ __forceinline__ void ffn_act_op(int sub, float& y, FfnAct& a, float b, float c0, float cq) {
  if (sub == 0) {
#if FFN_BIAS_ACC
    asm volatile("v_fmamk_f32 %0, %1, 0x3fb8aa3b, %2" : "=&v"(a.t) : "v"(y), "v"(c0));
#else
    asm volatile("v_add_f32 %0, %0, %2\n\tv_fmamk_f32 %1, %0, 0x3fb8aa3b, %3" : "+&v"(y), "=&v"(a.t) : "v"(b), "v"(c0));
#endif
  } else if (sub == 1) {
    asm volatile("v_min_f32 %0, 0x42fc0000, %1\n\tv_exp_f32 %0, %0" : "=&v"(a.m) : "v"(a.t));
  } else if (sub == 2) {
    asm volatile("v_add_f32 %0, 1.0, %0\n\tv_log_f32 %0, %0" : "+v"(a.m));
  } else {
    asm volatile("v_fmamk_f32 %1, %0, 0xbda3d70a, %4\n\tv_max_f32 %2, %2, %3\n\tv_fmamk_f32 %0, %2, 0x3f317218, %1"
                 : "+&v"(y), "=&v"(a.q), "+&v"(a.m) : "v"(a.t), "v"(cq));
  }
}

#ifndef FFN_DMA_K0
#define FFN_DMA_K0 1
#define FFN_DMA_K1 17
#define FFN_DMA_K2 33
#define FFN_DMA_K3 49
#endif
#ifndef FFN_TIMING
#define FFN_TIMING 0
#endif
#ifndef FFN_PD
#define FFN_PD 12
#endif
#ifndef FFN_PD_OPRE
#define FFN_PD_OPRE 8
#endif
#ifndef FFN_PD_NORM
#define FFN_PD_NORM 16
#endif
constexpr int FFN_DBG_WORDS = 10;
#ifndef FFN_X_NOACT
#define FFN_X_NOACT 0
#endif
#ifndef FFN_X_NOW1
#define FFN_X_NOW1 0
#endif
#ifndef FFN_X_NOW2
#define FFN_X_NOW2 0
#endif
#ifndef FFN_EPI_T
#define FFN_EPI_T 1
#endif
#ifndef FFN_PT
#define FFN_PT 16
#endif
#ifndef FFN_EPI_NT
#define FFN_EPI_NT 1
#endif
#ifndef FFN_PT_NORM
#define FFN_PT_NORM 8
#endif
constexpr unsigned long long FFN_SPIN_TICKS = 200000000;

template <bool RV, bool ORIG, bool COPY, int ABL = 0, int NORM = 0, bool TP = true>
__global__ __launch_bounds__(256, 1) void zv_ffn_kernel(FfnParams p) {
  extern __shared__ __attribute__((aligned(16))) unsigned char smem[];
  const int tid = threadIdx.x, lane = tid & 63;
  const int wave = __builtin_amdgcn_readfirstlane(tid >> 6);
  const int tl = lane & 31, hh = lane >> 5;
  const int nc = p.H / FFN_HC;
  float* b1s = reinterpret_cast<float*>(smem + 4 * FFN_SLOT);
  const long Wtot = (long)p.R * nc;
  const long start = (long)blockIdx.x * p.w;
  if (start >= Wtot) return;
  const long end = min(start + (long)p.w, Wtot);

  auto dma = [&](const bf16* W, int c, int slot, int half) {
    const unsigned long long a = (unsigned long long)W + (unsigned long long)((long)c * FFN_SLOT + wave * 8192 + half * 4096);
    const unsigned long long b =
        ((unsigned long long)(unsigned)__builtin_amdgcn_readfirstlane((unsigned)(a >> 32)) << 32) |
        (unsigned long long)(unsigned)__builtin_amdgcn_readfirstlane((unsigned)a);
    glds16s_x4(reinterpret_cast<const void*>(b), (unsigned)lane * 16u, smem + slot * FFN_SLOT + wave * 8192 + half * 4096);
  };
  auto item_at = [&](long ps, int& r, int& ca, int& cb) {
    r = (int)(ps / nc);
    const int c = (int)(ps - (long)r * nc);
    if (c != 0) { ca = 0; cb = nc - c; }
    else if (ps + nc <= end) { ca = 0; cb = nc; }
    else { ca = nc - (int)(end - ps); cb = nc; }
  };

  int r, ca, cb;
  item_at(start, r, ca, cb);
  dma(p.W1f, ca, 0, 0); dma(p.W1f, ca, 0, 1);
  dma(p.W1f, ca + 1, 1, 0); dma(p.W1f, ca + 1, 1, 1);
  for (int i = tid; i < p.H + FFN_HC; i += 256) b1s[i] = i < p.H ? p.b1[i] : 0.f;
  constexpr bool NLDS = NORM && FFN_NORM_LDS;
  float* ncs = b1s + p.H + FFN_HC;
  if constexpr (NLDS) {
    for (int i = tid; i < FFN_D; i += 256) {
      ncs[i] = p.b2[i];
      ncs[FFN_D + i] = p.nb[i];
      ncs[2 * FFN_D + i] = p.byp[i];
    }
  }

  float c0 = -5.77078016355585362f, cq = -0.035f;
  asm volatile("" : "+v"(c0), "+v"(cq));
  const int lfrag = lane * 16;
  int lfrag2 = lane * 16 + 2 * FFN_SLOT;
  asm volatile("" : "+v"(lfrag2));
  auto w1f = [&](int sl, int s) { return *reinterpret_cast<const bf16x8*>(smem + sl * FFN_SLOT + s * 1024 + lfrag); };
  auto w2f = [&](int sl, int i) { return *reinterpret_cast<const bf16x8*>(smem + sl * FFN_SLOT + i * 1024 + lfrag2); };
  auto put = [&](bf16x8 (&hb)[2], int rr, float y) { hb[rr >> 3][rr & 7] = (bf16)y; };
  const __amdgpu_buffer_rsrc_t part_rs = __builtin_amdgcn_make_buffer_rsrc(p.part, 0, 0x7fffffff, 0x00020000);

#if FFN_TIMING
  unsigned long long tm_vm = 0, tm_bar = 0, tm_steps = 0, tm_epi = 0, tm_x = 0, tm_items = 0, tm_loop = 0;
  const unsigned long long tm_t0 = __builtin_amdgcn_s_memtime(), tm_r0 = __builtin_amdgcn_s_memrealtime();
#endif
  auto item = [&](auto KIND_, int r, int ca, int cb, bool has_next, int nca) {
    constexpr int KIND = decltype(KIND_)::value;
    constexpr bool split_in = KIND == 2, split_out = KIND == 1;
    const int nxt_c0 = has_next ? nca : cb - 1;
    const int nxt_c1 = has_next ? nca + 1 : cb - 1;
    f32x16 out[16];
    int sg = 0;
#pragma unroll
    for (int i = 1; i < FFN_MAXSEG; ++i) sg = (i < p.nseg && r >= p.seg[i].rb0) ? i : sg;
    typedef __attribute__((address_space(4))) const FfnSeg KSeg;
    KSeg& S = ((KSeg*)((__attribute__((address_space(4))) const char*)__builtin_amdgcn_kernarg_segment_ptr() +
                       offsetof(FfnParams, seg)))[sg];
    const int t0 = (r - S.rb0) * FFN_BM + wave * 32;

    if constexpr (split_in) {
      if (tid == 0) {
        GLOBAL unsigned* fl = (GLOBAL unsigned*)(p.flag + blockIdx.x + 1);
        const unsigned long long t_give_up = wall_clock64() + FFN_SPIN_TICKS;
        while (__hip_atomic_load(fl, __ATOMIC_RELAXED, __HIP_MEMORY_SCOPE_AGENT) == 0u) {
          __builtin_amdgcn_s_sleep(2);
          if (wall_clock64() > t_give_up) {
            if (p.err) __hip_atomic_store(p.err, 1u, __ATOMIC_RELAXED, __HIP_MEMORY_SCOPE_SYSTEM);
            break;
          }
        }
        __builtin_amdgcn_fence(__ATOMIC_ACQUIRE, "agent");
        __hip_atomic_store(fl, 0u, __ATOMIC_RELAXED, __HIP_MEMORY_SCOPE_AGENT);
      }
      asm volatile("s_waitcnt vmcnt(0)" ::: "memory");
      __syncthreads();
      int lv = lane;
      asm volatile("" : "+v"(lv));
      const f32x4* src = reinterpret_cast<const f32x4*>(p.part + (long)(blockIdx.x + 1) * FFN_PART_FLOATS) + wave * 4096 + lv;
      static_for<16>([&](auto J_) {
        constexpr int j = decltype(J_)::value;
        f32x4 v[4];
#pragma unroll
        for (int q = 0; q < 4; ++q) v[q] = src[(j * 4 + q) * 64];
        out[j] = f32x16{v[0][0], v[0][1], v[0][2], v[0][3], v[1][0], v[1][1], v[1][2], v[1][3],
                        v[2][0], v[2][1], v[2][2], v[2][3], v[3][0], v[3][1], v[3][2], v[3][3]};
        __builtin_amdgcn_sched_barrier(0);
      });
    } else {
#pragma unroll
      for (int j = 0; j < 16; ++j) out[j] = f32x16{};
    }
#pragma unroll
    for (int j = 0; j < 16; ++j) asm volatile("" : "+a"(out[j]));
#if FFN_TIMING
    const unsigned long long tx0 = __builtin_amdgcn_s_memtime();
    ++tm_items;
#endif
    const bool nrv = NLDS && !split_out && S.rowvec != nullptr && p.rows_per_group >= 32;
    const int nrv_g0 = nrv ? min(t0, S.M - 1) / p.rows_per_group : 0;
    f32x4 nrvv[4];
    if constexpr (NLDS && !split_out) {
      if (nrv) {
        const int g1 = min(nrv_g0 + 1, (S.M - 1) / p.rows_per_group);
#pragma unroll
        for (int q = 0; q < 4; ++q) {
          const int f = (q * 64 + lane) * 4;
          const int grp = f < FFN_D ? nrv_g0 : g1;
          nrvv[q] = *reinterpret_cast<const f32x4*>(S.rowvec + (long)grp * p.rowvec_ld + (f & (FFN_D - 1)));
        }
      }
    }
    bf16x8 xf[32];
    {
      const int tr = min(t0 + tl, S.M - 1);
      const bf16* xr = S.X + (long)tr * p.ldx + 8 * hh;
#pragma unroll
      for (int s = 0; s < 32; ++s) xf[s] = *reinterpret_cast<const bf16x8*>(xr + 16 * s);
    }
    wait_vmcnt<FFN_XOVL ? 32 : 0>();
    if constexpr (NLDS && !split_out) {
      if (nrv) {
#pragma unroll
        for (int q = 0; q < 4; ++q)
          *reinterpret_cast<f32x4*>(ncs + 3 * FFN_D + wave * 2 * FFN_D + (q * 64 + lane) * 4) = nrvv[q];
      }
    }
    __syncthreads();
#if FFN_TIMING
    tm_x += __builtin_amdgcn_s_memtime() - tx0;
#endif

    auto bias4 = [&](int c, int q) { return *reinterpret_cast<const f32x4*>(b1s + c * FFN_HC + 8 * q + 4 * hh); };
    auto bias_tile = [&](int c) {
      const f32x4 q0 = bias4(c, 0), q1 = bias4(c, 1), q2 = bias4(c, 2), q3 = bias4(c, 3);
      return f32x16{q0[0], q0[1], q0[2], q0[3], q1[0], q1[1], q1[2], q1[3],
                    q2[0], q2[1], q2[2], q2[3], q3[0], q3[1], q3[2], q3[3]};
    };
    f32x16 h0, h1;
#if FFN_BIAS_ACC
    h0 = bias_tile(ca);
    h1 = bias_tile(ca + 1);
#endif
    {
      bf16x8 f[4];
#pragma unroll
      for (int q = 0; q < 4; ++q) f[q] = w1f(0, q);
      static_for<32>([&](auto S_) {
        constexpr int s = decltype(S_)::value;
        if constexpr (s == 0 && !FFN_BIAS_ACC) ffn_mma_v0(h0, f[0], xf[0]);
        else ffn_mma_v(h0, f[s & 3], xf[s]);
        if constexpr (s + 4 < 32) f[s & 3] = w1f(0, s + 4);
      });
    }
    asm volatile("s_nop 7\n\ts_nop 7\n\ts_nop 3" : "+v"(h0));
    __builtin_amdgcn_s_barrier();

    auto sync = [&]() {
#if FFN_TIMING
      const unsigned long long ts0 = __builtin_amdgcn_s_memtime();
#endif
      wait_vmcnt<0>();
      asm volatile("s_waitcnt lgkmcnt(0)" ::: "memory");
#if FFN_TIMING
      const unsigned long long ts1 = __builtin_amdgcn_s_memtime();
#endif
      __builtin_amdgcn_s_barrier();
#if FFN_TIMING
      const unsigned long long ts2 = __builtin_amdgcn_s_memtime();
      tm_vm += ts1 - ts0;
      tm_bar += ts2 - ts1;
      ++tm_steps;
#endif
      asm volatile("s_nop 7\n\ts_nop 7\n\ts_nop 3" ::: "memory");
    };
    auto w1_next = [&](int c) { return c + 2 <= cb - 1 ? c + 2 : (c + 2 == cb ? nxt_c0 : nxt_c1); };

    bf16x8 hb0[2], hb1[2];
    {
      const int c1 = w1_next(ca);
      dma(p.W1f, c1, 0, 0); dma(p.W1f, c1, 0, 1);
      dma(p.W2f, ca, 2, 0); dma(p.W2f, ca, 2, 1);
      f32x4 bq = FFN_BIAS_ACC ? f32x4{} : bias4(ca, 0);
      FfnAct a{};
      bf16x8 f[4];
#pragma unroll
      for (int q = 0; q < 4; ++q) f[q] = w1f(1, q);
      static_for<32>([&](auto S_) {
        constexpr int s = decltype(S_)::value, rr = s >> 1;
        if constexpr (s == 0 && !FFN_BIAS_ACC) ffn_mma_v0(h1, f[0], xf[0]);
        else ffn_mma_v(h1, f[s & 3], xf[s]);
        if constexpr (s + 4 < 32) f[s & 3] = w1f(1, s + 4);
        if constexpr ((rr & 3) == 0 && (s & 1) == 0 && !FFN_BIAS_ACC) bq = bias4(ca, rr >> 2);
        float y = h0[rr];
        ffn_act_op(2 * (s & 1), y, a, bq[rr & 3], c0, cq);
        ffn_act_op(2 * (s & 1) + 1, y, a, bq[rr & 3], c0, cq);
        h0[rr] = y;
        if constexpr (s & 1) put(hb0, rr, y);
      });
#if FFN_BIAS_ACC
      h0 = bias_tile(min(ca + 2, nc));
#endif
      asm volatile("s_nop 7\n\ts_nop 7\n\ts_nop 3" : "+v"(h1));
      sync();
      asm volatile("" ::"v"(f[0]), "v"(f[1]), "v"(f[2]), "v"(f[3]));
    }

    const int m = t0 + tl;
    const bool row_ok = m < S.M;
    const long mr = min(m, S.M - 1);
    const float* rrow = S.resid + mr * p.ldc;
    const float* orow = (ORIG || NORM) ? S.orig + mr * p.ldc : nullptr;
    constexpr bool OPRE = ORIG && !NORM;
    constexpr int PD = NORM ? FFN_PD_NORM : OPRE ? FFN_PD_OPRE : FFN_PD;
    f32x4 rr[32][2], ro[OPRE ? 32 : 1][2];
    auto prefetch = [&](int g) {
      if (g < 32) {
        const int n = 16 * g + 8 * hh;
        rr[g][0] = *reinterpret_cast<const f32x4*>(rrow + n);
        rr[g][1] = *reinterpret_cast<const f32x4*>(rrow + n + 4);
        if constexpr (OPRE) {
          ro[g][0] = *reinterpret_cast<const f32x4*>(orow + n);
          ro[g][1] = *reinterpret_cast<const f32x4*>(orow + n + 4);
        }
      }
    };

    constexpr bool EPT = FFN_EPI_T && TP && !NORM && ABL != 3;
    constexpr bool EPN = FFN_EPI_NT && TP && NORM && NLDS && ABL != 3 && !split_out;
    constexpr bool TORIG = EPT && ORIG;
    constexpr int PT = NORM ? FFN_PT_NORM : FFN_PT;
    int lve = lane;
    asm volatile("" : "+v"(lve));
    const int lr = lve >> 5, lc = lve & 31, ltl = lve & 31, lhh = lve >> 5;
    const int wrows = max(0, min(32, S.M - t0));
    f32x4 tq[EPT ? 64 : EPN ? 128 : 1], to[TORIG ? 64 : 1];
    const __amdgpu_buffer_rsrc_t rs_r =
        __builtin_amdgcn_make_buffer_rsrc(const_cast<float*>(S.resid + (long)t0 * p.ldc), 0, wrows * (int)p.ldc * 4, 0x00020000);
    const __amdgpu_buffer_rsrc_t rs_o = __builtin_amdgcn_make_buffer_rsrc(
        (TORIG || EPN) ? const_cast<float*>(S.orig + (long)t0 * p.ldc) : p.sink, 0,
        (TORIG || EPN) ? wrows * (int)p.ldc * 4 : 0, 0x00020000);
    const int toff = (lr * (int)p.ldc + 4 * lc) * 4, tstep = 2 * (int)p.ldc * 4;
    const bool has_rv = EPT && RV;
    const bool rv_two = has_rv && p.rows_per_group >= 32;
    const int rv_g0 = has_rv ? min(t0, S.M - 1) / p.rows_per_group : 0;
    const int rv_g1 = has_rv ? min(rv_g0 + 1, (S.M - 1) / p.rows_per_group) : 0;
    const int rv_bnd = has_rv ? (rv_g0 + 1) * p.rows_per_group - t0 : 0;
    constexpr bool TCONST = EPT && !ORIG;
    f32x4 cb2[TCONST ? 4 : 1], cby[TCONST ? 4 : 1], crv0[TCONST ? 4 : 1], crv1[TCONST ? 4 : 1];
    auto load_consts = [&]() {
      if constexpr (TCONST) {
#pragma unroll
        for (int ps = 0; ps < 4; ++ps) {
          const int col = ps * 128 + 4 * lc;
          if constexpr (EPT) cb2[ps] = *reinterpret_cast<const f32x4*>(p.b2 + col);
          if constexpr (TORIG) cby[ps] = *reinterpret_cast<const f32x4*>(p.byp + col);
          if (rv_two) {
            crv0[ps] = *reinterpret_cast<const f32x4*>(S.rowvec + (long)rv_g0 * p.rowvec_ld + col);
            crv1[ps] = *reinterpret_cast<const f32x4*>(S.rowvec + (long)rv_g1 * p.rowvec_ld + col);
          }
        }
      }
    };
    auto tprefetch = [&](int k) {
      if constexpr (EPN) {
        if (k < 128) {
          int so = (k & 15) * tstep;
          asm volatile("" : "+s"(so));
          tq[k] = __builtin_bit_cast(f32x4, __builtin_amdgcn_raw_buffer_load_b128(
              k < 64 ? rs_r : rs_o, toff, so + ((k >> 4) & 3) * 512, 0));
        }
      }
      if constexpr (EPT) {
        if (k < 64) {
          const int off = toff + (k & 15) * tstep + (k >> 4) * 512;
          tq[k] = __builtin_bit_cast(f32x4, __builtin_amdgcn_raw_buffer_load_b128(rs_r, off, 0, 0));
          if constexpr (ORIG) to[k] = __builtin_bit_cast(f32x4, __builtin_amdgcn_raw_buffer_load_b128(rs_o, off, 0, 0));
        }
      }
    };

    auto step = [&](auto MODE_, auto PAR_, int c, f32x16& cur, f32x16& nxt, bf16x8 (&hbw)[2], const bf16x8 (&hbr)[2]) {
      constexpr int MODE = decltype(MODE_)::value, PAR = decltype(PAR_)::value;
      constexpr int s1 = (PAR + 1) & 1, s2 = (PAR + 1) & 1;
      const int c1 = w1_next(c);
      if constexpr (MODE == 2) {
        if constexpr ((EPT || EPN) && !split_out) {
          load_consts();
#pragma unroll
          for (int k = 0; k < PT; ++k) tprefetch(k);
        } else {
#pragma unroll
          for (int g = 0; g < PD; ++g) prefetch(g);
        }
        __builtin_amdgcn_sched_barrier(0);
      }
      bf16x8 fa[4], fb[4];
#pragma unroll
      for (int q = 0; q < 4; ++q) {
        if constexpr (MODE == 0) fa[q] = w1f(s1, q);
        fb[q] = w2f(s2, q);
      }
      f32x4 bq = FFN_BIAS_ACC ? f32x4{} : bias4(c, 0);
      FfnAct a{};
      float y = 0.f;
      static_for<64>([&](auto K_) {
        constexpr int k = decltype(K_)::value, i = k >> 1;
        if constexpr ((k & 1) == 0) {
          if constexpr (MODE == 0) {
            if constexpr (i == 0 && !FFN_BIAS_ACC) ffn_mma_v0(nxt, fa[0], xf[0]);
            else ffn_mma_v(nxt, fa[i & 3], xf[i]);
            if constexpr (i + 4 < 32 && !FFN_X_NOW1) fa[i & 3] = w1f(s1, i + 4);
          }
        } else {
          ffn_mma_a(out[i >> 1], fb[i & 3], hbr[i & 1]);
          if constexpr (i + 4 < 32 && !FFN_X_NOW2) fb[i & 3] = w2f(s2, i + 4);
        }
        if constexpr (ABL != 1 && MODE <= 1) {
          if constexpr (k == FFN_DMA_K0) dma(p.W1f, c1, PAR, 0);
          if constexpr (k == FFN_DMA_K1) dma(p.W1f, c1, PAR, 1);
          if constexpr (k == FFN_DMA_K2) dma(p.W2f, c, 2 + PAR, 0);
          if constexpr (k == FFN_DMA_K3) dma(p.W2f, c, 2 + PAR, 1);
        }
        if constexpr (MODE <= 1) {
          constexpr int rg = k >> 2, sub = k & 3;
          if constexpr (sub == 0) {
            if constexpr ((rg & 3) == 0 && !FFN_BIAS_ACC) bq = bias4(c, rg >> 2);
            y = cur[rg];
          }
          if constexpr (!FFN_X_NOACT) ffn_act_op(sub, y, a, bq[rg & 3], c0, cq);
          if constexpr (sub == 3) put(hbw, rg, y);
        }
      });
#if FFN_BIAS_ACC
      if constexpr (MODE == 0) {
        asm volatile("" ::"v"(hbw[0]), "v"(hbw[1]));
        cur = bias_tile(c + 2);
      }
#endif
      if constexpr (MODE <= 1) sync();
      if constexpr (MODE == 0)
        asm volatile("" ::"v"(hbr[0]), "v"(hbr[1]), "v"(fa[0]), "v"(fa[1]), "v"(fa[2]), "v"(fa[3]),
                     "v"(fb[0]), "v"(fb[1]), "v"(fb[2]), "v"(fb[3]));
      else
        asm volatile("" ::"v"(hbr[0]), "v"(hbr[1]), "v"(fb[0]), "v"(fb[1]), "v"(fb[2]), "v"(fb[3]));
    };
    using M0 = std::integral_constant<int, 0>;
    using P0 = std::integral_constant<int, 0>;
    using P1 = std::integral_constant<int, 1>;
#if FFN_TIMING
    const unsigned long long tl0 = __builtin_amdgcn_s_memtime();
#endif
    for (int c = ca + 1; c <= cb - 3; c += 2) {
      step(M0{}, P1{}, c, h1, h0, hb1, hb0);
      step(M0{}, P0{}, c + 1, h0, h1, hb0, hb1);
    }
#if FFN_TIMING
    tm_loop += __builtin_amdgcn_s_memtime() - tl0;
#endif
    step(std::integral_constant<int, 1>{}, P1{}, cb - 1, h1, h0, hb1, hb0);
    step(std::integral_constant<int, 2>{}, P0{}, cb, h0, h1, hb0, hb1);
    asm volatile("s_nop 7\n\ts_nop 7\n\ts_nop 3" ::: "memory");
#if FFN_TIMING
    const unsigned long long te0 = __builtin_amdgcn_s_memtime();
#endif

    float* Cp = S.C;
    bf16* Chp = S.Ch;
    if constexpr (NORM) asm volatile("" : "+s"(Cp), "+s"(Chp));
    const unsigned long long c_base = row_ok ? (unsigned long long)(Cp + (long)m * p.ldc) : (unsigned long long)(p.sink + lane * 8);
    const unsigned c_mul = row_ok ? 4u : 0u;
    const unsigned long long h_base = (COPY && row_ok) ? (unsigned long long)(Chp + (long)m * p.ldch)
                                                       : (unsigned long long)(p.sink + 512 + lane * 4);
    const unsigned h_mul = (COPY && row_ok) ? 2u : 0u;
    if constexpr (ABL == 3 && !split_out) {
#pragma unroll
      for (int j = 0; j < 16; ++j) asm volatile("" : "+a"(out[j]));
    } else if constexpr (split_out) {
      int lv = lane;
      asm volatile("" : "+v"(lv));
      const int base = (wave * 4096 + lv) * 16;
#pragma unroll
      for (int j = 0; j < 16; ++j) asm volatile("" : "+a"(out[j]));
      static_for<16>([&](auto J_) {
        constexpr int j = decltype(J_)::value;
#pragma unroll
        for (int q = 0; q < 4; ++q) {
          const f32x4 v = {out[j][4 * q], out[j][4 * q + 1], out[j][4 * q + 2], out[j][4 * q + 3]};
          __builtin_amdgcn_raw_buffer_store_b128(v, part_rs, base + (j * 4 + q) * 1024,
                                                 (int)(blockIdx.x * FFN_PART_FLOATS * 4), 16);
        }
        __builtin_amdgcn_sched_barrier(0);
      });
      asm volatile("s_waitcnt vmcnt(0)" ::: "memory");
      __syncthreads();
      if (tid == 0) {
        unsigned long long fa = (unsigned long long)(p.flag + blockIdx.x);
        asm volatile("" : "+v"(fa));
        __hip_atomic_store((GLOBAL unsigned*)fa, 1u, __ATOMIC_RELAXED, __HIP_MEMORY_SCOPE_AGENT);
      }
    } else if constexpr (EPN) {
      __builtin_amdgcn_s_barrier();
      float* tb = reinterpret_cast<float*>(smem + 2 * FFN_SLOT) + wave * 4096;
      float ssr[16];
#pragma unroll
      for (int i = 0; i < 16; ++i) ssr[i] = 0.f;
      static_for<4>([&](auto P_) {
        constexpr int ps = decltype(P_)::value;
        static_for<4>([&](auto J_) {
          constexpr int jj = decltype(J_)::value, j = 4 * ps + jj;
#pragma unroll
          for (int q = 0; q < 4; ++q) {
            const int ch = (8 * jj + 2 * q + lhh) ^ (ltl & 7);
            *reinterpret_cast<f32x4*>(tb + ltl * 128 + ch * 4) =
                f32x4{out[j][4 * q], out[j][4 * q + 1], out[j][4 * q + 2], out[j][4 * q + 3]};
          }
        });
        __builtin_amdgcn_sched_barrier(0);
        int plr = lr, plc = lc;
        asm volatile("" : "+v"(plr), "+v"(plc));
        const int col = ps * 128 + 4 * plc;
        const f32x4 bb = *reinterpret_cast<const f32x4*>(ncs + col);
        const f32x4 nbv = *reinterpret_cast<const f32x4*>(ncs + FFN_D + col);
        static_for<16>([&](auto I_) {
          constexpr int i = decltype(I_)::value, k = 16 * ps + i;
          tprefetch(k + PT);
          const int row = 2 * i + plr;
          const f32x4 a = *reinterpret_cast<const f32x4*>(tb + row * 128 + ((plc ^ (row & 7)) * 4));
#pragma unroll
          for (int e = 0; e < 4; ++e) {
            const float x = tq[k][e] + (a[e] + bb[e]);
            const float d = x - nbv[e];
            ssr[i] += d * d;
            out[4 * ps + (i >> 2)][4 * (i & 3) + e] = x;
          }
          if constexpr ((i & 3) == 3) asm volatile("" : "+a"(out[4 * ps + (i >> 2)]));
          __builtin_amdgcn_sched_barrier(0);
        });
      });
#pragma unroll
      for (int i = 0; i < 16; ++i) {
#pragma unroll
        for (int o = 1; o < 32; o <<= 1) ssr[i] += __shfl_xor(ssr[i], o, 64);
        ssr[i] = rsqrtf(ssr[i] / (float)FFN_D) * p.norm_scale;
      }
      auto rsrc = [&](void* base, long ld, int esz) {
        return __builtin_amdgcn_make_buffer_rsrc(base ? base : (void*)p.sink, 0, base ? wrows * (int)ld * esz : 0, 0x00020000);
      };
      bf16* Clp = S.Cl;
      bf16* C2hp = S.C2h;
      bf16* C2lp = S.C2l;
      asm volatile("" : "+s"(Clp), "+s"(C2hp), "+s"(C2lp));
      const __amdgpu_buffer_rsrc_t rs_c = rsrc(Cp + (long)t0 * p.ldc, p.ldc, 4);
      const __amdgpu_buffer_rsrc_t rs_h = rsrc(Chp + (long)t0 * p.ldch, p.ldch, 2);
      const __amdgpu_buffer_rsrc_t rs_l = rsrc(Clp ? Clp + (long)t0 * p.ldch : nullptr, p.ldch, 2);
      const __amdgpu_buffer_rsrc_t rs_2h = rsrc(C2hp ? C2hp + (long)t0 * p.ldch : nullptr, p.ldch, 2);
      const __amdgpu_buffer_rsrc_t rs_2l = rsrc(C2lp ? C2lp + (long)t0 * p.ldch : nullptr, p.ldch, 2);
      const int hoff = (lr * (int)p.ldch + 4 * lc) * 2, hstep = 2 * (int)p.ldch * 2;
      const int rv_b = nrv ? (nrv_g0 + 1) * p.rows_per_group - t0 : 1 << 30;
      static_for<4>([&](auto P_) {
        constexpr int ps = decltype(P_)::value;
        int plr = lr, plc = lc;
        asm volatile("" : "+v"(plr), "+v"(plc));
        const int col = ps * 128 + 4 * plc;
        const f32x4 byv = *reinterpret_cast<const f32x4*>(ncs + 2 * FFN_D + col);
        f32x4 w0{}, w1{};
        if (nrv) {
          w0 = *reinterpret_cast<const f32x4*>(ncs + 3 * FFN_D + wave * 2 * FFN_D + col);
          w1 = *reinterpret_cast<const f32x4*>(ncs + 3 * FFN_D + wave * 2 * FFN_D + FFN_D + col);
        }
        static_for<16>([&](auto I_) {
          constexpr int i = decltype(I_)::value, k = 16 * ps + i;
          tprefetch(64 + k + PT);
          const int row = 2 * i + plr;
          f32x4 y;
#pragma unroll
          for (int e = 0; e < 4; ++e) {
            const float o = tq[64 + k][e];
            y[e] = o + (out[4 * ps + (i >> 2)][4 * (i & 3) + e] * ssr[i] - o) * byv[e];
          }
          int fo = i * tstep, ho = i * hstep;
          asm volatile("" : "+s"(fo), "+s"(ho));
          fo += ps * 512;
          ho += ps * 256;
          __builtin_amdgcn_raw_buffer_store_b128(__builtin_bit_cast(v4u32_t, y), rs_c, toff, fo, 0);
          bf16x4 h, l;
#pragma unroll
          for (int e = 0; e < 4; ++e) h[e] = (bf16)y[e];
          __builtin_amdgcn_raw_buffer_store_b64(__builtin_bit_cast(v2u32_t, h), rs_h, hoff, ho, 0);
          if (Clp) {
#pragma unroll
            for (int e = 0; e < 4; ++e) l[e] = (bf16)(y[e] - (float)h[e]);
            __builtin_amdgcn_raw_buffer_store_b64(__builtin_bit_cast(v2u32_t, l), rs_l, hoff, ho, 0);
          }
          if (C2hp) {
            if (nrv) {
              const bool second = row >= rv_b;
#pragma unroll
              for (int e = 0; e < 4; ++e) y[e] += second ? w1[e] : w0[e];
            }
#pragma unroll
            for (int e = 0; e < 4; ++e) h[e] = (bf16)y[e];
            __builtin_amdgcn_raw_buffer_store_b64(__builtin_bit_cast(v2u32_t, h), rs_2h, hoff, ho, 0);
            if (C2lp) {
#pragma unroll
              for (int e = 0; e < 4; ++e) l[e] = (bf16)(y[e] - (float)h[e]);
              __builtin_amdgcn_raw_buffer_store_b64(__builtin_bit_cast(v2u32_t, l), rs_2l, hoff, ho, 0);
            }
          }
          __builtin_amdgcn_sched_barrier(0);
        });
      });
    } else if constexpr (NORM) {
      float ss = 0.f;
      f32x4 rq[32][2];
      auto pre_o = [&](int g) {
        if (g < 32) {
          const int n = 16 * g + 8 * hh;
          rq[g][0] = *reinterpret_cast<const f32x4*>(orow + n);
          rq[g][1] = *reinterpret_cast<const f32x4*>(orow + n + 4);
        }
      };
      static_for<32>([&](auto G_) {
        constexpr int g = decltype(G_)::value, j = g >> 1, pp = g & 1;
        if constexpr (g + PD < 32) prefetch(g + PD);
        else pre_o(g + PD - 32);
        const int n = 16 * g + 8 * hh;
        float v[8];
#pragma unroll
        for (int e = 0; e < 4; ++e) {
          const auto sw = __builtin_amdgcn_permlane32_swap(__float_as_uint(out[j][8 * pp + e]),
                                                           __float_as_uint(out[j][8 * pp + 4 + e]), false, false);
          v[e] = __uint_as_float(sw[0]);
          v[4 + e] = __uint_as_float(sw[1]);
        }
        const float* b2c = NLDS ? ncs : p.b2;
        const f32x4 b0 = *reinterpret_cast<const f32x4*>(b2c + n);
        const f32x4 b1 = *reinterpret_cast<const f32x4*>(b2c + n + 4);
        const float* nbc = NLDS ? ncs + FFN_D : p.nb;
        const f32x4 n0 = *reinterpret_cast<const f32x4*>(nbc + n);
        const f32x4 n1 = *reinterpret_cast<const f32x4*>(nbc + n + 4);
#pragma unroll
        for (int e = 0; e < 4; ++e) {
          v[e] = rr[g][0][e] + (v[e] + b0[e]);
          v[4 + e] = rr[g][1][e] + (v[4 + e] + b1[e]);
          const float d0 = v[e] - n0[e], d1 = v[4 + e] - n1[e];
          ss += d0 * d0 + d1 * d1;
          out[j][8 * pp + e] = v[e];
          out[j][8 * pp + 4 + e] = v[4 + e];
        }
      });
      ss += __shfl_xor(ss, 32, 64);
      const float scale = rsqrtf(ss / (float)FFN_D) * p.norm_scale;
      const float* vrow = (S.rowvec && !nrv) ? S.rowvec + (mr / p.rows_per_group) * p.rowvec_ld : nullptr;
      const int vl_off = 3 * FFN_D + wave * 2 * FFN_D + ((t0 + tl >= (nrv_g0 + 1) * p.rows_per_group) ? FFN_D : 0);
      bf16* Clp = S.Cl;
      bf16* C2hp = S.C2h;
      bf16* C2lp = S.C2l;
      asm volatile("" : "+s"(Clp), "+s"(C2hp), "+s"(C2lp));
      auto adr16 = [&](bf16* base, long oh) {
        unsigned long long a = row_ok ? (unsigned long long)(base + oh) : (unsigned long long)(p.sink + 512 + lane * 4);
        asm volatile("" : "+v"(a));
        return (GLOBAL bf16x8*)a;
      };
      auto adr32 = [&](float* base, long o) {
        unsigned long long a = row_ok ? (unsigned long long)(base + o) : (unsigned long long)(p.sink + lane * 8);
        asm volatile("" : "+v"(a));
        return (GLOBAL f32x4*)a;
      };
      static_for<32>([&](auto G_) {
        constexpr int g = decltype(G_)::value, j = g >> 1, pp = g & 1;
        pre_o(g + PD);
        const int n = 16 * g + 8 * hh;
        const float* byc = NLDS ? ncs + 2 * FFN_D : p.byp;
        const f32x4 c0v = *reinterpret_cast<const f32x4*>(byc + n);
        const f32x4 c1v = *reinterpret_cast<const f32x4*>(byc + n + 4);
        float y[8];
#pragma unroll
        for (int e = 0; e < 4; ++e) {
          y[e] = rq[g][0][e] + (out[j][8 * pp + e] * scale - rq[g][0][e]) * c0v[e];
          y[4 + e] = rq[g][1][e] + (out[j][8 * pp + 4 + e] * scale - rq[g][1][e]) * c1v[e];
        }
        const long o = (long)m * p.ldc + n, oh = (long)m * p.ldch + n;
        GLOBAL f32x4* ca = adr32(Cp, o);
        ca[0] = f32x4{y[0], y[1], y[2], y[3]};
        ca[1] = f32x4{y[4], y[5], y[6], y[7]};
        bf16x8 h, l;
#pragma unroll
        for (int e = 0; e < 8; ++e) h[e] = (bf16)y[e];
        *adr16(Chp, oh) = h;
        if (Clp) {
#pragma unroll
          for (int e = 0; e < 8; ++e) l[e] = (bf16)(y[e] - (float)h[e]);
          if (row_ok) *reinterpret_cast<bf16x8*>(Clp + oh) = l;
        }
        if (C2hp) {
          if (nrv) {
            const f32x4 w0 = *reinterpret_cast<const f32x4*>(ncs + vl_off + n);
            const f32x4 w1 = *reinterpret_cast<const f32x4*>(ncs + vl_off + n + 4);
#pragma unroll
            for (int e = 0; e < 4; ++e) { y[e] += w0[e]; y[4 + e] += w1[e]; }
          } else if (vrow) {
            const f32x4 w0 = *reinterpret_cast<const f32x4*>(vrow + n);
            const f32x4 w1 = *reinterpret_cast<const f32x4*>(vrow + n + 4);
#pragma unroll
            for (int e = 0; e < 4; ++e) { y[e] += w0[e]; y[4 + e] += w1[e]; }
          }
#pragma unroll
          for (int e = 0; e < 8; ++e) { h[e] = (bf16)y[e]; l[e] = (bf16)(y[e] - (float)h[e]); }
          if (row_ok) {
            *reinterpret_cast<bf16x8*>(C2hp + oh) = h;
            if (C2lp) *reinterpret_cast<bf16x8*>(C2lp + oh) = l;
          }
        }
      });
    } else if constexpr (EPT) {
      __builtin_amdgcn_s_barrier();
      float* tb = reinterpret_cast<float*>(smem + 2 * FFN_SLOT) + wave * 4096;
      const __amdgpu_buffer_rsrc_t rs_c = __builtin_amdgcn_make_buffer_rsrc(Cp + (long)t0 * p.ldc, 0, wrows * (int)p.ldc * 4, 0x00020000);
      const __amdgpu_buffer_rsrc_t rs_h =
          __builtin_amdgcn_make_buffer_rsrc(COPY ? (void*)(Chp + (long)t0 * p.ldch) : (void*)p.sink, 0, COPY ? wrows * (int)p.ldch * 2 : 0, 0x00020000);
      const int hoff = (lr * (int)p.ldch + 4 * lc) * 2, hstep = 2 * (int)p.ldch * 2;
      static_for<4>([&](auto P_) {
        constexpr int ps = decltype(P_)::value;
        static_for<4>([&](auto J_) {
          constexpr int jj = decltype(J_)::value, j = 4 * ps + jj;
#pragma unroll
          for (int q = 0; q < 4; ++q) {
            const int ch = (8 * jj + 2 * q + lhh) ^ (ltl & 7);
            *reinterpret_cast<f32x4*>(tb + ltl * 128 + ch * 4) =
                f32x4{out[j][4 * q], out[j][4 * q + 1], out[j][4 * q + 2], out[j][4 * q + 3]};
          }
        });
        __builtin_amdgcn_sched_barrier(0);
        const int col = ps * 128 + 4 * lc;
        f32x4 bb, sc4{};
        if constexpr (TCONST) bb = cb2[ps];
        else {
          bb = *reinterpret_cast<const f32x4*>(p.b2 + col);
          if constexpr (ORIG) sc4 = *reinterpret_cast<const f32x4*>(p.byp + col);
        }
        const f32x4 rv0 = crv0[ps], rv1 = crv1[ps];
        static_for<16>([&](auto I_) {
          constexpr int i = decltype(I_)::value, k = 16 * ps + i;
          tprefetch(k + PT);
          const int row = 2 * i + lr;
          const f32x4 a = *reinterpret_cast<const f32x4*>(tb + row * 128 + ((lc ^ (row & 7)) * 4));
          f32x4 v;
#pragma unroll
          for (int e = 0; e < 4; ++e) v[e] = tq[k][e] + (a[e] + bb[e]);
          const int mrow = t0 + row;
          if constexpr (RV) {
            const bool second = row >= rv_bnd;
            f32x4 w;
#pragma unroll
            for (int e = 0; e < 4; ++e) w[e] = second ? rv1[e] : rv0[e];
#pragma unroll
            for (int e = 0; e < 4; ++e) v[e] += w[e];
          }
          if constexpr (ORIG) {
#pragma unroll
            for (int e = 0; e < 4; ++e) v[e] = to[k][e] + (v[e] - to[k][e]) * sc4[e];
          }
          __builtin_amdgcn_raw_buffer_store_b128(__builtin_bit_cast(v4u32_t, v), rs_c, toff + i * tstep + ps * 512, 0, 0);
          if constexpr (COPY) {
            bf16x4 h;
#pragma unroll
            for (int e = 0; e < 4; ++e) h[e] = (bf16)v[e];
            __builtin_amdgcn_raw_buffer_store_b64(__builtin_bit_cast(v2u32_t, h), rs_h, hoff + i * hstep + ps * 256, 0, 0);
          }
          __builtin_amdgcn_sched_barrier(0);
        });
      });
    } else {
      const float* vrow = RV ? S.rowvec + (mr / p.rows_per_group) * p.rowvec_ld : nullptr;
      static_for<32>([&](auto G_) {
        constexpr int g = decltype(G_)::value, j = g >> 1, pp = g & 1;
        prefetch(g + PD);
        const int n = 16 * g + 8 * hh;
        float v[8];
#pragma unroll
        for (int e = 0; e < 4; ++e) {
          const auto sw = __builtin_amdgcn_permlane32_swap(__float_as_uint(out[j][8 * pp + e]),
                                                           __float_as_uint(out[j][8 * pp + 4 + e]), false, false);
          v[e] = __uint_as_float(sw[0]);
          v[4 + e] = __uint_as_float(sw[1]);
        }
        const f32x4 b0 = *reinterpret_cast<const f32x4*>(p.b2 + n);
        const f32x4 b1 = *reinterpret_cast<const f32x4*>(p.b2 + n + 4);
#pragma unroll
        for (int e = 0; e < 4; ++e) {
          v[e] = rr[g][0][e] + (v[e] + b0[e]);
          v[4 + e] = rr[g][1][e] + (v[4 + e] + b1[e]);
        }
        if constexpr (RV) {
          const f32x4 w0 = *reinterpret_cast<const f32x4*>(vrow + n);
          const f32x4 w1 = *reinterpret_cast<const f32x4*>(vrow + n + 4);
#pragma unroll
          for (int e = 0; e < 4; ++e) { v[e] += w0[e]; v[4 + e] += w1[e]; }
        }
        if constexpr (ORIG) {
          const f32x4 s0 = *reinterpret_cast<const f32x4*>(p.byp + n);
          const f32x4 s1 = *reinterpret_cast<const f32x4*>(p.byp + n + 4);
#pragma unroll
          for (int e = 0; e < 4; ++e) {
            v[e] = ro[g][0][e] + (v[e] - ro[g][0][e]) * s0[e];
            v[4 + e] = ro[g][1][e] + (v[4 + e] - ro[g][1][e]) * s1[e];
          }
        }
        unsigned long long cadr = c_base + (unsigned long long)(n * c_mul);
        asm volatile("" : "+v"(cadr));
        *(GLOBAL f32x4*)(cadr) = f32x4{v[0], v[1], v[2], v[3]};
        *(GLOBAL f32x4*)(cadr + 16) = f32x4{v[4], v[5], v[6], v[7]};
        if constexpr (COPY) {
          bf16x8 h;
#pragma unroll
          for (int e = 0; e < 8; ++e) h[e] = (bf16)v[e];
          unsigned long long ha2 = h_base + (unsigned long long)(n * h_mul);
          asm volatile("" : "+v"(ha2));
          *(GLOBAL bf16x8*)(ha2) = h;
        }
      });
    }
#if FFN_TIMING
    asm volatile("s_waitcnt vmcnt(0)" ::: "memory");
    tm_epi += __builtin_amdgcn_s_memtime() - te0;
#endif
  };

  long pos = start;
  for (;;) {
    const bool split_in = ca > 0, split_out = cb < nc;
    const long npos = split_out ? (long)(r + 1) * nc : (split_in ? end : pos + nc);
    const bool has_next = npos < end;
    int nr = 0, nca = 0, ncb = 0;
    if (has_next) item_at(npos, nr, nca, ncb);
    if (split_out) item(std::integral_constant<int, 1>{}, r, ca, cb, has_next, nca);
    else if (split_in) item(std::integral_constant<int, 2>{}, r, ca, cb, has_next, nca);
    else item(std::integral_constant<int, 0>{}, r, ca, cb, has_next, nca);
    if (!has_next) break;
    pos = npos; r = nr; ca = nca; cb = ncb;
  }
#if FFN_TIMING
  if (lane == 0) {
    unsigned long long* d = p.dbg + ((long)blockIdx.x * 4 + wave) * FFN_DBG_WORDS;
    d[0] = __builtin_amdgcn_s_memtime() - tm_t0;
    d[1] = __builtin_amdgcn_s_memrealtime() - tm_r0;
    d[2] = tm_vm; d[3] = tm_bar; d[4] = tm_steps; d[5] = (unsigned long long)p.w;
    d[6] = tm_epi; d[7] = tm_x; d[8] = tm_items; d[9] = tm_loop;
  }
#endif
}

static __global__ void zv_ffn_pack_w1_kernel(const bf16* W, long ldw, int H, bf16* out) {
  const long i = blockIdx.x * 256L + threadIdx.x;
  if (i >= (long)H * FFN_D) return;
  const int j = (int)(i & 7);
  long r = i >> 3;
  const int l = (int)(r & 63); r >>= 6;
  const int s = (int)(r & 31), c = (int)(r >> 5);
  out[i] = W[(long)(32 * c + (l & 31)) * ldw + 16 * s + 8 * (l >> 5) + j];
}
static __global__ void zv_ffn_pack_w2_kernel(const bf16* W, long ldw, int H, bf16* out) {
  const long i = blockIdx.x * 256L + threadIdx.x;
  if (i >= (long)H * FFN_D) return;
  const int j = (int)(i & 7);
  long r = i >> 3;
  const int l = (int)(r & 63); r >>= 6;
  const int s = (int)(r & 1); r >>= 1;
  const int jb = (int)(r & 15), c = (int)(r >> 4);
  out[i] = W[(long)(32 * jb + (l & 31)) * ldw + 32 * c + 16 * s + 8 * (j >> 2) + 4 * (l >> 5) + (j & 3)];
}
static void ffn_pack_weights(const Linear& L1, const Linear& L2, int H, bf16* w1f, bf16* w2f, hipStream_t s) {
  const long n = (long)H * FFN_D;
  hipLaunchKernelGGL(zv_ffn_pack_w1_kernel, dim3(cdiv(n, 256)), dim3(256), 0, s, L1.hi, (long)L1.Kpad, H, w1f);
  hipLaunchKernelGGL(zv_ffn_pack_w2_kernel, dim3(cdiv(n, 256)), dim3(256), 0, s, L2.hi, (long)L2.Kpad, H, w2f);
  ZV_LAUNCH_CHECK();
}

struct FfnSchedule { int w, blocks; };
inline FfnSchedule ffn_schedule(int R, int nc, int blocks_max, bool persistent) {
  if (!persistent || R <= blocks_max) return {nc, R};
  const long W = (long)R * nc;
  long w = (W + blocks_max - 1) / blocks_max;
  w = std::max<long>(round_up(w, 2), nc);
  return {(int)w, (int)((W + w - 1) / w)};
}

template <bool RV, bool ORIG, bool COPY, int ABL = 0, int NORM = 0, bool TP = true>
static void launch_ffn_t(const FfnParams& p, int blocks, hipStream_t s, const char* tag) {
  static unsigned long long attr = 0;
  const size_t lds = ffn_lds_bytes(p.H, NORM != 0);
  if (!((attr >> zv_cur_device()) & 1)) {
    ZV_CHECK(hipFuncSetAttribute((const void*)zv_ffn_kernel<RV, ORIG, COPY, ABL, NORM, TP>,
                                 hipFuncAttributeMaxDynamicSharedMemorySize, 160 * 1024));
    attr |= 1ull << zv_cur_device();
  }
  double M = 0, extra = 0;
  for (int i = 0; i < p.nseg; ++i) {
    const FfnSeg& g = p.seg[i];
    M += g.M;
    if (NORM) extra += (double)g.M * FFN_D * ((g.Cl ? 2 : 0) + (g.C2h ? 2 : 0) + (g.C2l ? 2 : 0));
  }
  const double outs = M * FFN_D;
  const double bytes = outs * 2 + 2.0 * FFN_D * p.H * 2 +
                       (NORM ? outs * (4 + 4 + 4 + 2) + extra : outs * (8 + (COPY ? 2 : 0) + (ORIG ? 4 : 0)));
  g_zv_last_launch = ZvLaunchRec{FFN_BM, FFN_D, 1, (int)RV | (int)ORIG << 1 | (int)COPY << 2 | (int)TP << 3, NORM,
                                 0, blocks, p.w};
  ZvProfScope prof(tag, 4.0 * M * FFN_D * (double)p.H, bytes, s);
  hipLaunchKernelGGL((zv_ffn_kernel<RV, ORIG, COPY, ABL, NORM, TP>), dim3(blocks), dim3(256), lds, s, p);
  ZV_LAUNCH_CHECK();
}

template <int ABL = 0>
static void launch_ffn(FfnParams p, hipStream_t s, const char* tag, int blocks_max = 0) {
  ZV_REQUIRE(p.H > 0 && p.H % (2 * FFN_HC) == 0 && ffn_lds_bytes(p.H, p.nb != nullptr) <= 160 * 1024,
             "fused FeedForward: hidden width a multiple of 64 (LDS: at most 8160, 2496 with the BiasNorm epilogue)");
  ZV_REQUIRE(p.nseg >= 1 && p.nseg <= FFN_MAXSEG, "fused FeedForward: 1..4 row ranges");
  ZV_REQUIRE(p.W1f && p.W2f && p.b1 && p.b2 && p.ldx % 8 == 0 && p.ldx >= FFN_D && p.ldc % 4 == 0 &&
                 p.ldc >= FFN_D && (p.ldch == 0 || (p.ldch % 8 == 0 && p.ldch >= FFN_D)),
             "fused FeedForward operands (16-B aligned rows of at least 512)");
  const bool rv = p.seg[0].rowvec != nullptr, og = p.seg[0].orig != nullptr, cp = p.seg[0].Ch != nullptr;
  int R = 0;
  for (int i = 0; i < p.nseg; ++i) {
    FfnSeg& g = p.seg[i];
    ZV_REQUIRE(g.M > 0 && g.X && g.resid && g.C && (g.Ch != nullptr) == cp && (g.rowvec != nullptr) == rv &&
                   (g.orig != nullptr) == og && (!g.Ch || p.ldch > 0),
               "fused FeedForward row range operands");
    g.rb0 = R;
    R += cdiv(g.M, FFN_BM);
  }
  ZV_REQUIRE(og == (p.byp != nullptr) && (!rv || p.rows_per_group > 0), "fused FeedForward bypass / row vector");
  p.R = R;
  p.sink = zv_epi_sink();
  p.err = zv_dev_err_word();
  const int nc = p.H / FFN_HC;
  const bool pers = p.part && p.flag;
  int bmax = blocks_max > 0 ? std::min(blocks_max, zv_num_cus()) : zv_num_cus();
  if (pers) {
    ZV_REQUIRE(p.part_slots > 0, "fused FeedForward: persistent scratch without its slot count");
    bmax = std::min(bmax, p.part_slots);
  }
  const FfnSchedule sc = ffn_schedule(R, nc, bmax, pers);
  ZV_REQUIRE(!pers || sc.w == nc || sc.blocks <= bmax, "fused FeedForward: more lines than scratch slots");
  p.w = sc.w;
  if (p.nb) {
    for (int i = 0; i < p.nseg; ++i)
      ZV_REQUIRE(p.seg[i].orig && p.seg[i].C == p.seg[i].orig && p.seg[i].Ch,
                 "fused FeedForward + BiasNorm operands");
    ZV_REQUIRE(p.byp, "fused FeedForward + BiasNorm bypass");
    p.norm_scale = expf(p.log_scale);
    if (p.seg[0].rowvec && p.rows_per_group < 32) launch_ffn_t<false, false, true, 0, 1, false>(p, sc.blocks, s, tag);
    else launch_ffn_t<false, false, true, 0, 1>(p, sc.blocks, s, tag);
    return;
  }
  if constexpr (ABL != 0) { launch_ffn_t<false, false, true, ABL>(p, sc.blocks, s, tag); return; }
  if (!rv && !og && cp) launch_ffn_t<false, false, true>(p, sc.blocks, s, tag);
  else if (!rv && !og && !cp) launch_ffn_t<false, false, false>(p, sc.blocks, s, tag);
  else if (rv && !og && cp) {
    if (p.rows_per_group >= 32) launch_ffn_t<true, false, true>(p, sc.blocks, s, tag);
    else launch_ffn_t<true, false, true, 0, 0, false>(p, sc.blocks, s, tag);
  }
  else if (!rv && og && cp) launch_ffn_t<false, true, true>(p, sc.blocks, s, tag);
  else throw std::invalid_argument("fused FeedForward: unsupported epilogue combination");
}
```

### zipvoice_amd/engine.py

```python
from __future__ import annotations

import ctypes
import os
from typing import Dict, Optional

import numpy as np
import torch

from .config import ModelConfig
from .weights import check_state_dict

LIB_NAME = "libzipvoice_hip.so"
LIB_PATH = os.path.join(os.path.dirname(os.path.abspath(__file__)), LIB_NAME)
LIB_F16_PATH = os.path.join(os.path.dirname(os.path.abspath(__file__)), "libzipvoice_hip_f16.so")
MAX_STACKS = 8
VARIANT_ID = {"zipvoice": 0, "zipvoice_distill": 1, "zipvoice_dialog": 2,
              "zipvoice_dialog_stereo": 3}
PRECISION_ID = {"fp32": 0, "bf16": 1}
MODES = {"fp32": ("bf16", 0), "bf16": ("bf16", 1), "fp16": ("f16", 2),
         "fp16_plain": ("f16", 1), "bf16_mixed": ("bf16", 2), "fp8": ("bf16", 3)}


class ZvConfig(ctypes.Structure):
    _fields_ = [
        ("variant", ctypes.c_int), ("precision", ctypes.c_int), ("feat_dim", ctypes.c_int),
        ("num_stacks", ctypes.c_int),
        ("downsampling_factor", ctypes.c_int * MAX_STACKS),
        ("num_layers", ctypes.c_int * MAX_STACKS),
        ("cnn_module_kernel", ctypes.c_int * MAX_STACKS),
        ("fm_decoder_dim", ctypes.c_int), ("fm_decoder_feedforward_dim", ctypes.c_int),
        ("fm_decoder_num_heads", ctypes.c_int),
        ("text_encoder_num_layers", ctypes.c_int), ("text_encoder_feedforward_dim", ctypes.c_int),
        ("text_encoder_cnn_module_kernel", ctypes.c_int),
        ("text_encoder_num_heads", ctypes.c_int), ("text_encoder_dim", ctypes.c_int),
        ("time_embed_dim", ctypes.c_int), ("text_embed_dim", ctypes.c_int),
        ("query_head_dim", ctypes.c_int), ("value_head_dim", ctypes.c_int),
        ("pos_head_dim", ctypes.c_int), ("pos_dim", ctypes.c_int),
        ("vocab_size", ctypes.c_int), ("pad_id", ctypes.c_int), ("spk_a_id", ctypes.c_int),
        ("spk_b_id", ctypes.c_int),
    ]


class ZvLinearCheckArgs(ctypes.Structure):
    _fields_ = [(n, ctypes.c_int) for n in ("M", "N", "K", "split", "form", "act", "rows_per_group",
                                            "rpb", "guard")] + [
        (n, ctypes.c_void_p) for n in ("A", "W", "bias", "resid", "orig", "byp", "rowvec", "rowmask",
                                       "dw_w", "dw_b")] + [
        ("dw_ks", ctypes.c_int), ("dw_L", ctypes.c_int),
        ("C", ctypes.c_void_p), ("ldc", ctypes.c_int64),
        ("Ch", ctypes.c_void_p), ("Cl", ctypes.c_void_p), ("ldch", ctypes.c_int64),
        ("Cth", ctypes.c_void_p), ("Ctl", ctypes.c_void_p), ("ldct", ctypes.c_int64),
        ("launch", ctypes.c_int * 8), ("num_cus", ctypes.c_int)]


class ZvFfnCheckArgs(ctypes.Structure):
    _fields_ = [(n, ctypes.c_int) for n in ("M", "H", "form", "rows_per_group", "part_slots", "guard")] + [
        ("log_scale", ctypes.c_float)] + [
        (n, ctypes.c_void_p) for n in ("x", "W1", "b1", "W2", "b2", "resid", "rowvec", "orig", "byp", "nb")] + [
        ("C", ctypes.c_void_p), ("ldc", ctypes.c_int64),
        ("Ch", ctypes.c_void_p), ("Cl", ctypes.c_void_p), ("C2h", ctypes.c_void_p), ("C2l", ctypes.c_void_p),
        ("ldch", ctypes.c_int64),
        ("launch", ctypes.c_int * 8), ("num_cus", ctypes.c_int)]


class ZvDwconvCheckArgs(ctypes.Structure):
    _fields_ = [(n, ctypes.c_int) for n in ("B", "L", "C", "ks", "split", "guard")] + [
        (n, ctypes.c_void_p) for n in ("g", "w", "bias")] + [
        ("ldin", ctypes.c_int64),
        ("Oh", ctypes.c_void_p), ("Ol", ctypes.c_void_p), ("ldout", ctypes.c_int64),
        ("q", ctypes.c_void_p), ("qs", ctypes.c_void_p), ("ldq", ctypes.c_int64),
        ("launch", ctypes.c_int * 8), ("num_cus", ctypes.c_int)]


class ZvStackedgeCheckArgs(ctypes.Structure):
    _fields_ = [(n, ctypes.c_int) for n in ("kind", "B", "L", "C", "ds", "guard", "rows_per_group")] + [
        ("log_scale", ctypes.c_float)] + [
        (n, ctypes.c_void_p) for n in ("x", "w", "nb", "orig", "rowvec", "mask", "out", "mout",
                                       "h", "l", "h2", "l2")] + [
        ("ldact", ctypes.c_int64),
        ("q2", ctypes.c_void_p), ("qs2", ctypes.c_void_p), ("ldq", ctypes.c_int64),
        ("launch", ctypes.c_int * 8), ("num_cus", ctypes.c_int)]


class ZvBigvganCheckArgs(ctypes.Structure):
    _fields_ = [(n, ctypes.c_int) for n in ("kind", "split", "mode", "guard", "B", "Lmax", "Ls", "halo", "scale",
                                            "C", "Cout", "ks", "d", "u", "n", "layout", "flag")] + [
        (n, ctypes.c_float) for n in ("div", "sub", "bias0")] + [
        ("stale", ctypes.c_uint)] + [
        (n, ctypes.c_void_p) for n in ("lens", "x", "x1", "x2", "w", "bias", "alpha", "ibeta", "w2", "bias2",
                                       "alpha2", "ibeta2", "taps", "resid", "ah", "al", "out", "oh", "ol")] + [
        ("ld", ctypes.c_int64),
        ("launch", ctypes.c_int * 8), ("num_cus", ctypes.c_int)]


_P = ctypes.c_void_p
_I = ctypes.c_int
_F = ctypes.c_float
SIGNATURES = {
    "zv_last_error": (ctypes.c_char_p, []),
    "zv_version": (ctypes.c_char_p, []),
    "zv_create": (_P, [ctypes.POINTER(ZvConfig)]),
    "zv_destroy": (None, [_P]),
    "zv_set_weight": (_I, [_P, ctypes.c_char_p, _P, ctypes.c_int64]),
    "zv_finalize": (_I, [_P]),
    "zv_reserve": (_I, [_P, _I, _I]),
    "zv_device_bytes": (ctypes.c_int64, [_P]),
    "zv_profile": (_I, [_I]),
    "zv_bench_gemm": (_I, [_I, _I, _I, _I, _I, _I, ctypes.POINTER(ctypes.c_float)]),
    "zv_gemm_selftest": (_I, [_I, _I, _I, _I, _I, ctypes.POINTER(ctypes.c_float), ctypes.POINTER(ctypes.c_float)]),
    "zv_linear_check": (_I, [ctypes.POINTER(ZvLinearCheckArgs)]),
    "zv_ffn_check": (_I, [ctypes.POINTER(ZvFfnCheckArgs)]),
    "zv_dwconv_check": (_I, [ctypes.POINTER(ZvDwconvCheckArgs)]),
    "zv_stackedge_check": (_I, [ctypes.POINTER(ZvStackedgeCheckArgs)]),
    "zv_bigvgan_check": (_I, [ctypes.POINTER(ZvBigvganCheckArgs)]),
    "zv_profile_report": (_I, [ctypes.c_char_p, _I]),
    "zv_host_block_count": (ctypes.c_int64, []),
    "zv_attn_fallbacks": (_I, [_P, _I, _P]),
    "zv_attn2_check": (_I, [_I, _I, _I, _I, _I, _I, _P, _P, _P, _P, _P, _I, _P, _P]),
    "zv_attn_plan": (_I, [_I, _I, _I, _I, _I, _P, _P, _P, _P]),
    "zv_mx8_quantize": (_I, [_P, _I, _I, _P, _P]),
    "zv_mx8_gemm_check": (_I, [_I, _I, _I, _P, _P, _P, _P, _P]),
    "zv_fm_decoder": (_I, [_P, _P, _P, _P, _P, _P, _P, _I, _I, _I, _P, _P]),
    "zv_velocity": (_I, [_P, _F, _F, _P, _P, _P, _P, _I, _I, _P, _P]),
    "zv_euler_sample": (_I, [_P, _P, _P, _P, _P, _I, _I, _I, _F, _F, _F, _F, _P]),
    "zv_velocity_rows": (_I, [_P, _F, _P, _P, _P, _P, _P, _I, _I, _P, _P]),
    "zv_euler_sample_rows": (_I, [_P, _P, _P, _P, _P, _I, _I, _I, _P, _F, _F, _F, _P]),
    "zv_text_encode": (_I, [_P, _P, _P, _P, _I, _I, _P, _P]),
    "zv_text_condition": (_I, [_P, _P, _I, _I, _P, _P, _I, _P, _P]),
    "zv_speech_condition": (_I, [_P, _P, _I, _I, _I, _P, _I, _P, _P]),
    "zv_vocoder_create": (_P, [_P]),
    "zv_vocoder_destroy": (None, [_P]),
    "zv_vocoder_set_weight": (_I, [_P, ctypes.c_char_p, _P, ctypes.c_int64]),
    "zv_vocoder_finalize": (_I, [_P]),
    "zv_vocoder_decode": (_I, [_P, _P, _I, _F, _F, _P, _I, _I, _P, _I, _P]),
    "zv_vocoder_device_bytes": (ctypes.c_int64, [_P]),
    "zv_bigvgan_create": (_P, [_P]),
    "zv_bigvgan_destroy": (None, [_P]),
    "zv_bigvgan_set_weight": (_I, [_P, ctypes.c_char_p, _P, ctypes.c_int64]),
    "zv_bigvgan_finalize": (_I, [_P]),
    "zv_bigvgan_decode": (_I, [_P, _P, _I, _F, _F, _P, _I, _I, _P, _P]),
    "zv_bigvgan_device_bytes": (ctypes.c_int64, [_P]),
    "zv_fbank_create": (_P, [_I, _I, _I, _P, _P]),
    "zv_fbank_destroy": (None, [_P]),
    "zv_fbank_extract": (_I, [_P, _P, ctypes.c_int64, _P, _I, _I, _P, ctypes.c_int64, _P]),
    "zv_fbank_configure": (_I, [_P, _I, _F, _F]),
    "zv_resample_create": (_P, [_I, _I, _I, _P, _P]),
    "zv_resample_destroy": (None, [_P]),
    "zv_resample_apply": (_I, [_P, _P, ctypes.c_int64, _P, _I, _P, ctypes.c_int64, ctypes.c_int64, _P]),
    "zv_resample_device_bytes": (ctypes.c_int64, [_P]),
    "zv_wavjoin_create": (_P, [_I, _F, _I, _I, _I]),
    "zv_wavjoin_destroy": (None, [_P]),
    "zv_wavjoin_apply": (_I, [_P, _P, ctypes.c_int64, _P, _P, _I, _I, _P, ctypes.c_int64,
                              ctypes.c_int64, _P, _P, _P]),
    "zv_wavjoin_apply_docs": (_I, [_P, _P, ctypes.c_int64, _P, _P, _I, _I, _P, _I, _P,
                                   ctypes.c_int64, ctypes.c_int64, _P, _P, _P]),
    "zv_wavjoin_device_bytes": (ctypes.c_int64, [_P]),
}

_libs: Dict[str, ctypes.CDLL] = {}
_lib = None


def load_library(path: Optional[str] = None, operand: str = "bf16"):
    global _lib
    if path is None:
        path = ((os.environ.get("ZV_LIB_F16_PATH") or LIB_F16_PATH) if operand == "f16"
                else (os.environ.get("ZV_LIB_PATH") or LIB_PATH))
    if path in _libs:
        return _libs[path]
    if not os.path.exists(path):
        raise RuntimeError(
            f"{os.path.basename(path)} not found at {path}: build it with "
            "`python zipvoice_amd/csrc/build.py` (or __graft_entry__.build()). "
            "There is no CPU fallback for the ZipVoice hot path.")
    lib = ctypes.CDLL(path, mode=ctypes.RTLD_LOCAL)
    for name, (res, args) in SIGNATURES.items():
        if path not in (LIB_PATH, LIB_F16_PATH) and not hasattr(lib, name):
            continue
        fn = getattr(lib, name)
        fn.restype = res
        fn.argtypes = args
    _libs[path] = lib
    if operand != "f16" and _lib is None:
        _lib = lib
    return lib


def _check(rc: int, lib=None):
    if rc != 0:
        msg = (lib or _lib).zv_last_error().decode()
        if "missing weight" in msg or "expected" in msg or "unexpected" in msg:
            raise KeyError(msg)
        raise RuntimeError(f"zipvoice_hip: {msg}")


def make_zv_config(cfg: ModelConfig, precision: str) -> ZvConfig:
    c = ZvConfig()
    c.variant = VARIANT_ID[cfg.variant]
    c.precision = MODES[precision][1]
    c.feat_dim = cfg.feat_dim
    n = len(cfg.fm_decoder_downsampling_factor)
    if n > MAX_STACKS:
        raise ValueError(f"at most {MAX_STACKS} decoder stacks supported")
    c.num_stacks = n
    for i in range(n):
        c.downsampling_factor[i] = cfg.fm_decoder_downsampling_factor[i]
        c.num_layers[i] = cfg.fm_decoder_num_layers[i]
        c.cnn_module_kernel[i] = cfg.fm_decoder_cnn_module_kernel[i]
    for f in ("fm_decoder_dim", "fm_decoder_feedforward_dim", "fm_decoder_num_heads",
              "text_encoder_num_layers", "text_encoder_feedforward_dim",
              "text_encoder_cnn_module_kernel", "text_encoder_num_heads", "text_encoder_dim",
              "time_embed_dim", "text_embed_dim", "query_head_dim", "value_head_dim",
              "pos_head_dim", "pos_dim", "vocab_size", "pad_id", "spk_a_id", "spk_b_id"):
        setattr(c, f, int(getattr(cfg, f)))
    return c
# ... 207 lines not shown
```

Baseline: 81570 mel-frames/s.

## Fuse conv/self-attention out-projection into the following fused FeedForward kernel

Adds a PRE mode to the fused FFN kernel that computes the conv+SelfAttention out-projection (with bias, time-embedding row vector and residual) inside the FFN block, then feeds the bf16 result straight into the first FFN matmul. This removes a separate linear launch and the write and re-read of its output activation between the two stages. Weights for the pre-projection and a re-laid-out W1 are packed at load time. It is enabled by default by raising ZV_FFN to 3. The cost is extra per-block work and register/LDS pressure in an already heavy kernel, and more complex numerics (bf16 rounding of the intermediate in registers).

After: 84960 mel-frames/s (median of 6 runs). +4.2%, better.

```diff
diff --git a/include/zipvoice_hip.h b/include/zipvoice_hip.h
--- a/include/zipvoice_hip.h
+++ b/include/zipvoice_hip.h
@@ -103,6 +103,10 @@
   uint16_t* Ch; uint16_t* Cl; uint16_t* C2h; uint16_t* C2l; int64_t ldch;
   int launch[8];
   int num_cus;
+  int K;
+  const float* A;
+  const float* Wp;
+  const float* bp;
 } zv_ffn_check_args;
 int zv_ffn_check(zv_ffn_check_args* a);
 
diff --git a/zipvoice_amd/csrc/zv_checks.inc b/zipvoice_amd/csrc/zv_checks.inc
--- a/zipvoice_amd/csrc/zv_checks.inc
+++ b/zipvoice_amd/csrc/zv_checks.inc
@@ -478,12 +478,14 @@
 int zv_ffn_check(zv_ffn_check_args* a) {
   ZV_API_BEGIN
   ZV_REQUIRE(a && a->M > 0 && a->H > 0 && a->H % (2 * FFN_HC) == 0 && a->form >= 0 && a->form <= 3 &&
-                 a->guard >= 0 && a->part_slots >= 0 && a->x && a->W1 && a->b1 && a->W2 && a->b2 &&
+                 a->guard >= 0 && a->part_slots >= 0 && (a->x || a->K > 0) && a->W1 && a->b1 && a->W2 && a->b2 &&
                  a->resid && a->C && a->ldc >= FFN_D && (!a->Ch || a->ldch >= FFN_D),
              "zv_ffn_check: bad arguments");
   const int M = a->M, H = a->H, form = a->form, G = a->guard, D = FFN_D;
   const bool norm = form == 3, byp = form == 2 || norm, rv = a->rowvec != nullptr;
-  ZV_REQUIRE((form == 1) == (rv && !norm) || norm, "zv_ffn_check: the row vector belongs to form 1 (or 3)");
+  const bool pre = a->K > 0;
+  ZV_REQUIRE(!pre || (byp && a->A && a->Wp && a->bp), "zv_ffn_check: the pre-projection belongs to forms 2 and 3");
+  ZV_REQUIRE((form == 1) == (rv && !norm) || norm || pre, "zv_ffn_check: the row vector belongs to form 1 (or 3)");
   ZV_REQUIRE((!rv || a->rows_per_group > 0) && (!byp || (a->orig && a->byp)) && (!norm || a->nb) &&
                  (form == 0 || a->Ch) && (norm || (!a->Cl && !a->C2h && !a->C2l)) &&
                  (!a->C2l || a->C2h),
@@ -502,7 +504,17 @@
   q.H = H; q.nseg = 1;
   FfnSeg& g = q.seg[0];
   g.M = M;
-  {
+  if (pre) {
+    const int K = a->K;
+    const Linear Lp = store.make_linear(a->Wp, D, K, a->bp);
+    const int nkp = ffn_pre_chunks(K);
+    bf16* wpf = dev.make<bf16>((size_t)nkp * FFN_HC * D);
+    ffn_pack_pre_weights(L1, H, w1f, Lp, wpf, s);
+    q.Wpf = wpf; q.bp = Lp.b; q.nkp = nkp; q.lda = (long)nkp * FFN_HC + 8;
+    std::vector<bf16> h, l;
+    chk_act(a->A, M, K, q.lda, false, h, l);
+    g.A = dev.up(h.data(), h.size());
+  } else {
     std::vector<bf16> h, l;
     chk_act(a->x, M, D, D, false, h, l);
     g.X = dev.up(h.data(), h.size());
diff --git a/zipvoice_amd/csrc/zv_engine.hip b/zipvoice_amd/csrc/zv_engine.hip
--- a/zipvoice_amd/csrc/zv_engine.hip
+++ b/zipvoice_amd/csrc/zv_engine.hip
@@ -36,6 +36,8 @@
   Linear ff_in[3], ff_out[3];
   bf16* ffn_w1f[3] = {nullptr, nullptr, nullptr};
   bf16* ffn_w2f[3] = {nullptr, nullptr, nullptr};
+  bf16* ffn_w1fp[3] = {nullptr, nullptr, nullptr};
+  bf16* ffn_wpf[2] = {nullptr, nullptr};
   Linear na_in, na_out;
   Linear conv_in[2], conv_out[2];
   Linear conv_sa_out[2];
@@ -181,7 +183,7 @@
   hipEvent_t split_fork = nullptr, split_join[MAX_SPLIT - 1] = {};
 
   bool materialize_attn = false;
-  int ffn_fused = 2;
+  int ffn_fused = 3;
   long ffn_min_rows = 15000;
   int fp8_fuse = 7;
   int sa_tp = 1;
@@ -197,7 +199,7 @@
     graph_mode = envi("ZV_GRAPH", 2);
     sa_tp = envi("ZV_SA_TP", 1);
     fp8_fuse = envi("ZV_FP8_FUSE", 7);
-    ffn_fused = envi("ZV_FFN", 2);
+    ffn_fused = envi("ZV_FFN", 3);
     ffn_min_rows = envi("ZV_FFN_MIN_ROWS", 15000);
     ffn_persist = envi("ZV_FFN_PERSIST", 1);
     split_streams = envi("ZV_SPLIT_STREAMS", 3);
@@ -480,6 +482,13 @@
             W.conv_sa_out[c] = make_linear_kcat(cp + "out_proj", dim,
                                                 lp + "self_attn" + std::to_string(c + 1) + ".out_proj",
                                                 heads * Z.vd, dim, cfg.precision == ZV_MIXED && mixed_sa);
+          if (ffn_fused >= 3 && W.conv_sa_out[c].hi && W.ffn_w1f[c + 1]) {
+            const int f = c + 1;
+            W.ffn_w1fp[f] = store.dalloc<bf16>((long)hs[f] * FFN_D);
+            W.ffn_wpf[c] = store.dalloc<bf16>((long)ffn_pre_chunks(W.conv_sa_out[c].K) * FFN_HC * FFN_D);
+            ffn_pack_pre_weights(W.ff_in[f], hs[f], W.ffn_w1fp[f], W.conv_sa_out[c], W.ffn_wpf[c], nullptr);
+            ZV_CHECK(ZV_BLOCKING(hipDeviceSynchronize()));
+          }
           W.dw_w[c] = store.upload_key(cp + "depthwise_conv.weight", (size_t)dim * W.ks);
           W.dw_b[c] = store.upload_key(cp + "depthwise_conv.bias", dim);
         }
@@ -658,7 +667,8 @@
       q.W1f = W.ffn_w1f[f]; q.b1 = W.ff_in[f].b; q.W2f = W.ffn_w2f[f]; q.b2 = W.ff_out[f].b;
       return q;
     };
-    auto ff = [&](int f, const Out& oe) {
+    std::function<void(FfnParams&, int)> ffn_pre_operands;
+    auto ff = [&](int f, const Out& oe, int pre_c = -1) {
       if constexpr (SPLIT == 1) {
         if (ffn_fused && W.ffn_w1f[f] && !(f8 && W.ff_in[f].q8) && oe.C && oe.resid &&
             !oe.act.l && !oe.residh && Mtot >= ffn_min_rows && cur_a.ld % 8 == 0) {
@@ -667,10 +677,12 @@
           g.resid = oe.resid; g.C = oe.C; q.ldc = oe.ldc; g.Ch = oe.act.h; q.ldch = oe.act.ld;
           g.rowvec = oe.rowvec; q.rowvec_ld = oe.rowvec_ld; q.rows_per_group = oe.rows_per_group;
           g.orig = oe.orig; q.byp = oe.byp;
+          if (pre_c >= 0) ffn_pre_operands(q, pre_c);
           ffn_site(q, ws, s, "ffn_bf16");
           return;
         }
       }
+      ZV_REQUIRE(pre_c < 0, "the pre-projection site fell off the fused FeedForward");
       const bool f8f = f8 && W.ff_in[f].q8 && W.ff_out[f].q8;
       Act hid = ws.hidden.get(M, W.ff_in[f].N, split, f8f, W.ff_in[f].N, !f8f);
       Out o1; o1.act = hid; o1.act_fn = 1;
@@ -718,6 +730,21 @@
     if (kcat) dwo = ws.dwo.get(M, round_up(W.conv_sa_out[0].K, 64), false);
     const bool sa_split = kcat && pass.io_split && W.conv_sa_out[0].K == D + 3 * H * Z.vd;
     ZV_REQUIRE(!kcat || sa_split || W.conv_sa_out[0].K == D + H * Z.vd, "conv + SelfAttention out-projection width");
+    const bool ffn_norm = SPLIT == 1 && ffn_fused >= 2 && W.ffn_w1f[2] && !f8 && D == FFN_D &&
+                          Mtot >= ffn_min_rows && cur_a.ld == src_a.ld && cur_a.ld % 8 == 0;
+    auto pre_fits = [&](int c) {
+      return kcat && ffn_fused >= 3 && D == FFN_D && W.ffn_w1fp[c + 1] && W.ffn_wpf[c] && !cur_a.l &&
+             Mtot >= ffn_min_rows && cur_a.ld % 8 == 0 && dwo.ld % 8 == 0 &&
+             dwo.ld >= (long)ffn_pre_chunks(W.conv_sa_out[c].K) * FFN_HC;
+    };
+    const bool pre_site[2] = {pre_fits(0), pre_fits(1) && ffn_norm};
+    ffn_pre_operands = [&](FfnParams& q, int c) {
+      FfnSeg& g = q.seg[0];
+      g.X = nullptr; g.A = dwo.h; q.lda = dwo.ld;
+      q.W1f = W.ffn_w1fp[c + 1]; q.Wpf = W.ffn_wpf[c]; q.bp = W.conv_sa_out[c].b;
+      q.nkp = ffn_pre_chunks(W.conv_sa_out[c].K);
+      g.rowvec = temb; q.rowvec_ld = D; q.rows_per_group = L;
+    };
     auto self_attn = [&](int a) {
       const int vd = Z.vd, HV = H * vd;
       const int VR = W.sa_in[a].N, vph = VR / H;
@@ -771,7 +798,8 @@
                       dq ? dw.q : nullptr, dw.qs, dw.ldq);
         if (f8 && !dq) pack8(dw, M, D, s);
       }
-      if (kcat) {
+      if (kcat && pre_site[c]) {
+      } else if (kcat) {
         Out e = res;
         e.rowvec = temb; e.rowvec_ld = D; e.rows_per_group = L;
         linear<SPLIT>(W.conv_sa_out[c], dw, M, e, s);
@@ -784,12 +812,10 @@
     {
       Out e = res; e.byp = W.bypass_mid;
       e.orig = src;
-      ff(1, e);
+      ff(1, e, pre_site[0] ? 0 : -1);
     }
     self_attn(1);
     conv(1);
-    const bool ffn_norm = SPLIT == 1 && ffn_fused >= 2 && W.ffn_w1f[2] && !f8 && D == FFN_D &&
-                          Mtot >= ffn_min_rows && cur_a.ld == src_a.ld && cur_a.ld % 8 == 0;
     if (ffn_norm) {
       FfnParams q = ffn_params(2);
       FfnSeg& g = q.seg[0];
@@ -798,6 +824,7 @@
       q.byp = W.bypass; q.nb = W.norm_bias; q.log_scale = W.norm_log_scale;
       g.rowvec = temb; q.rowvec_ld = D; q.rows_per_group = L;
       g.C2h = has_next ? cur_a.h : nullptr; g.C2l = has_next ? cur_a.l : nullptr;
+      if (pre_site[1]) ffn_pre_operands(q, 1);
       ffn_site(q, ws, s, "ffn_norm_bf16");
     } else {
       Out e = res;
diff --git a/zipvoice_amd/csrc/zv_ffn.inc b/zipvoice_amd/csrc/zv_ffn.inc
--- a/zipvoice_amd/csrc/zv_ffn.inc
+++ b/zipvoice_amd/csrc/zv_ffn.inc
@@ -11,6 +11,7 @@
 struct FfnSeg {
   int M, rb0;
   const bf16* X;
+  const bf16* A;
   const float* resid; float* C;
   bf16* Ch;
   const float* rowvec;
@@ -26,6 +27,7 @@
   const bf16* W1f; const float* b1;
   const bf16* W2f; const float* b2;
   const float* byp;
+  const bf16* Wpf; const float* bp; long lda; int nkp;
   const float* nb; float log_scale;
   float norm_scale;
   float* sink;
@@ -131,7 +133,7 @@
 #endif
 constexpr unsigned long long FFN_SPIN_TICKS = 200000000;
 
-template <bool RV, bool ORIG, bool COPY, int ABL = 0, int NORM = 0, bool TP = true>
+template <bool RV, bool ORIG, bool COPY, int ABL = 0, int NORM = 0, bool TP = true, bool PRE = false>
 __global__ __launch_bounds__(256, 1) void zv_ffn_kernel(FfnParams p) {
   extern __shared__ __attribute__((aligned(16))) unsigned char smem[];
   const int tid = threadIdx.x, lane = tid & 63;
@@ -230,12 +232,14 @@
                         v[2][0], v[2][1], v[2][2], v[2][3], v[3][0], v[3][1], v[3][2], v[3][3]};
         __builtin_amdgcn_sched_barrier(0);
       });
-    } else {
+    } else if constexpr (!PRE) {
 #pragma unroll
       for (int j = 0; j < 16; ++j) out[j] = f32x16{};
     }
-#pragma unroll
-    for (int j = 0; j < 16; ++j) asm volatile("" : "+a"(out[j]));
+    if constexpr (!PRE || split_in) {
+#pragma unroll
+      for (int j = 0; j < 16; ++j) asm volatile("" : "+a"(out[j]));
+    }
 #if FFN_TIMING
     const unsigned long long tx0 = __builtin_amdgcn_s_memtime();
     ++tm_items;
@@ -255,13 +259,21 @@
       }
     }
     bf16x8 xf[32];
-    {
+    if constexpr (!PRE) {
       const int tr = min(t0 + tl, S.M - 1);
       const bf16* xr = S.X + (long)tr * p.ldx + 8 * hh;
 #pragma unroll
       for (int s = 0; s < 32; ++s) xf[s] = *reinterpret_cast<const bf16x8*>(xr + 16 * s);
+    } else if constexpr (split_in) {
+      const int tr = min(t0 + tl, S.M - 1);
+      const bf16* xr = S.Ch + (long)tr * p.ldch + 4 * hh;
+#pragma unroll
+      for (int s = 0; s < 32; ++s) {
+        const bf16x4 lo = *reinterpret_cast<const bf16x4*>(xr + 16 * s), hi = *reinterpret_cast<const bf16x4*>(xr + 16 * s + 8);
+        xf[s] = bf16x8{lo[0], lo[1], lo[2], lo[3], hi[0], hi[1], hi[2], hi[3]};
+      }
     }
-    wait_vmcnt<FFN_XOVL ? 32 : 0>();
+    wait_vmcnt<(FFN_XOVL && !PRE) ? 32 : 0>();
     if constexpr (NLDS && !split_out) {
       if (nrv) {
 #pragma unroll
@@ -273,6 +285,132 @@
 #if FFN_TIMING
     tm_x += __builtin_amdgcn_s_memtime() - tx0;
 #endif
+
+    if constexpr (PRE && !split_in) {
+      int lvp = lane;
+      asm volatile("" : "+v"(lvp));
+      const int ptl = lvp & 31, phh = lvp >> 5;
+      const int wr = max(0, min(32, S.M - t0));
+      const __amdgpu_buffer_rsrc_t rs_a =
+          __builtin_amdgcn_make_buffer_rsrc(const_cast<bf16*>(S.A + (long)t0 * p.lda), 0, wr * (int)p.lda * 2, 0x00020000);
+      const __amdgpu_buffer_rsrc_t rs_pr =
+          __builtin_amdgcn_make_buffer_rsrc(const_cast<float*>(S.resid + (long)t0 * p.ldc), 0, wr * (int)p.ldc * 4, 0x00020000);
+      const int a_off = (ptl * (int)p.lda + 8 * phh) * 2, r_off = (ptl * (int)p.ldc + 4 * phh) * 4;
+      auto load_a = [&](int kc, int s) {
+        return __builtin_bit_cast(bf16x8, __builtin_amdgcn_raw_buffer_load_b128(rs_a, a_off + kc * 64 + s * 32, 0, 0));
+      };
+      dma(p.Wpf, 0, 2, 0); dma(p.Wpf, 0, 2, 1);
+      bf16x8 ac[2], an[2];
+      ac[0] = load_a(0, 0); ac[1] = load_a(0, 1);
+      const bool hrv = S.rowvec != nullptr;
+      const int rpg = hrv ? p.rows_per_group : 1;
+      auto tile_of = [&](const f32x4 (&v)[4]) {
+        return f32x16{v[0][0], v[0][1], v[0][2], v[0][3], v[1][0], v[1][1], v[1][2], v[1][3],
+                      v[2][0], v[2][1], v[2][2], v[2][3], v[3][0], v[3][1], v[3][2], v[3][3]};
+      };
+      if (!hrv || rpg >= 32) {
+        float* cvs = reinterpret_cast<float*>(smem + 3 * FFN_SLOT) + wave * 2 * FFN_D;
+        const int g0 = hrv ? min(t0, S.M - 1) / rpg : 0;
+        const int g1 = hrv ? min(g0 + 1, (S.M - 1) / rpg) : 0;
+#pragma unroll
+        for (int q = 0; q < 4; ++q) {
+          const int f = (q * 64 + lvp) * 4, ch = f & (FFN_D - 1);
+          f32x4 v = *reinterpret_cast<const f32x4*>(p.bp + ch);
+          if (hrv) v += *reinterpret_cast<const f32x4*>(S.rowvec + (long)(f < FFN_D ? g0 : g1) * p.rowvec_ld + ch);
+          *reinterpret_cast<f32x4*>(cvs + f) = v;
+        }
+        asm volatile("s_waitcnt lgkmcnt(0)" ::: "memory");
+        __builtin_amdgcn_wave_barrier();
+        const float* cvp = cvs + ((hrv && t0 + ptl >= (g0 + 1) * rpg) ? FFN_D : 0) + 4 * phh;
+        constexpr int PDT = 6;
+        f32x4 ri[16][4];
+        auto pf = [&](int j) {
+          if (j < 16) {
+#pragma unroll
+            for (int q = 0; q < 4; ++q)
+              ri[j][q] = __builtin_bit_cast(f32x4, __builtin_amdgcn_raw_buffer_load_b128(rs_pr, r_off + (32 * j + 8 * q) * 4, 0, 0));
+          }
+        };
+#pragma unroll
+        for (int j = 0; j < PDT; ++j) pf(j);
+        static_for<16>([&](auto J_) {
+          constexpr int j = decltype(J_)::value;
+          pf(j + PDT);
+          f32x4 v[4];
+#pragma unroll
+          for (int q = 0; q < 4; ++q) v[q] = ri[j][q] + *reinterpret_cast<const f32x4*>(cvp + 32 * j + 8 * q);
+          out[j] = tile_of(v);
+          asm volatile("" : "+a"(out[j]));
+          __builtin_amdgcn_sched_barrier(0);
+        });
+      } else {
+        const int grp = min(t0 + ptl, S.M - 1) / rpg;
+        const float* vrow = S.rowvec + (long)grp * p.rowvec_ld + 4 * phh;
+        const float* bpl = p.bp + 4 * phh;
+        static_for<16>([&](auto J_) {
+          constexpr int j = decltype(J_)::value;
+          f32x4 v[4];
+#pragma unroll
+          for (int q = 0; q < 4; ++q) {
+            const f32x4 r4 = __builtin_bit_cast(f32x4, __builtin_amdgcn_raw_buffer_load_b128(rs_pr, r_off + (32 * j + 8 * q) * 4, 0, 0));
+            v[q] = r4 + (*reinterpret_cast<const f32x4*>(bpl + 32 * j + 8 * q) + *reinterpret_cast<const f32x4*>(vrow + 32 * j + 8 * q));
+          }
+          out[j] = tile_of(v);
+          asm volatile("" : "+a"(out[j]));
+          if constexpr ((j & 3) == 3) __builtin_amdgcn_sched_barrier(0);
+        });
+      }
+      auto pstep = [&](auto PAR_, int kc) {
+        constexpr int PAR = decltype(PAR_)::value;
+        wait_vmcnt<0>();
+        asm volatile("s_waitcnt lgkmcnt(0)" ::: "memory");
+        __builtin_amdgcn_s_barrier();
+        asm volatile("s_nop 7\n\ts_nop 7\n\ts_nop 3" ::: "memory");
+        if (kc + 1 < p.nkp) { dma(p.Wpf, kc + 1, 3 - PAR, 0); dma(p.Wpf, kc + 1, 3 - PAR, 1); }
+        const int kn = min(kc + 1, p.nkp - 1);
+        an[0] = load_a(kn, 0); an[1] = load_a(kn, 1);
+        bf16x8 fb[4];
+#pragma unroll
+        for (int q = 0; q < 4; ++q) fb[q] = w2f(PAR, q);
+        static_for<32>([&](auto I_) {
+          constexpr int i = decltype(I_)::value;
+          ffn_mma_a(out[i >> 1], fb[i & 3], ac[i & 1]);
+          if constexpr (i + 4 < 32) fb[i & 3] = w2f(PAR, i + 4);
+        });
+        asm volatile("" ::"v"(ac[0]), "v"(ac[1]), "v"(fb[0]), "v"(fb[1]), "v"(fb[2]), "v"(fb[3]));
+        ac[0] = an[0]; ac[1] = an[1];
+      };
+      int kc = 0;
+      for (; kc + 1 < p.nkp; kc += 2) {
+        pstep(std::integral_constant<int, 0>{}, kc);
+        pstep(std::integral_constant<int, 1>{}, kc + 1);
+      }
+      if (kc < p.nkp) pstep(std::integral_constant<int, 0>{}, kc);
+      asm volatile("s_nop 7\n\ts_nop 7\n\ts_nop 3" ::: "memory");
+#pragma unroll
+      for (int j = 0; j < 16; ++j) asm volatile("" : "+a"(out[j]));
+      static_for<32>([&](auto S_) {
+        constexpr int s = decltype(S_)::value, jt = s >> 1, pp = s & 1;
+#pragma unroll
+        for (int e = 0; e < 8; ++e) xf[s][e] = (bf16)out[jt][8 * pp + e];
+      });
+#pragma unroll
+      for (int j = 0; j < 16; ++j) asm volatile("" : "+a"(out[j]));
+      if constexpr (split_out) {
+        const __amdgpu_buffer_rsrc_t rs_xh =
+            __builtin_amdgcn_make_buffer_rsrc(S.Ch + (long)t0 * p.ldch, 0, wr * (int)p.ldch * 2, 0x00020000);
+        const int h_off = (ptl * (int)p.ldch + 4 * phh) * 2;
+        static_for<32>([&](auto S_) {
+          constexpr int s = decltype(S_)::value;
+          const v4u32_t w = __builtin_bit_cast(v4u32_t, xf[s]);
+          __builtin_amdgcn_raw_buffer_store_b64(v2u32_t{w[0], w[1]}, rs_xh, h_off + 32 * s, 0, 16);
+          __builtin_amdgcn_raw_buffer_store_b64(v2u32_t{w[2], w[3]}, rs_xh, h_off + 32 * s + 16, 0, 16);
+        });
+      }
+#pragma unroll
+      for (int s = 0; s < 32; ++s) asm volatile("" : "+v"(xf[s]));
+      asm volatile("s_nop 7\n\ts_nop 7\n\ts_nop 3" ::: "memory");
+    }
 
     auto bias4 = [&](int c, int q) { return *reinterpret_cast<const f32x4*>(b1s + c * FFN_HC + 8 * q + 4 * hh); };
     auto bias_tile = [&](int c) {
@@ -360,8 +498,10 @@
     auto prefetch = [&](int g) {
       if (g < 32) {
         const int n = 16 * g + 8 * hh;
-        rr[g][0] = *reinterpret_cast<const f32x4*>(rrow + n);
-        rr[g][1] = *reinterpret_cast<const f32x4*>(rrow + n + 4);
+        if constexpr (!PRE) {
+          rr[g][0] = *reinterpret_cast<const f32x4*>(rrow + n);
+          rr[g][1] = *reinterpret_cast<const f32x4*>(rrow + n + 4);
+        }
         if constexpr (OPRE) {
           ro[g][0] = *reinterpret_cast<const f32x4*>(orow + n);
           ro[g][1] = *reinterpret_cast<const f32x4*>(orow + n + 4);
@@ -407,7 +547,7 @@
     };
     auto tprefetch = [&](int k) {
       if constexpr (EPN) {
-        if (k < 128) {
+        if (k < 128 && !(PRE && k < 64)) {
           int so = (k & 15) * tstep;
           asm volatile("" : "+s"(so));
           tq[k] = __builtin_bit_cast(f32x4, __builtin_amdgcn_raw_buffer_load_b128(
@@ -417,7 +557,7 @@
       if constexpr (EPT) {
         if (k < 64) {
           const int off = toff + (k & 15) * tstep + (k >> 4) * 512;
-          tq[k] = __builtin_bit_cast(f32x4, __builtin_amdgcn_raw_buffer_load_b128(rs_r, off, 0, 0));
+          if constexpr (!PRE) tq[k] = __builtin_bit_cast(f32x4, __builtin_amdgcn_raw_buffer_load_b128(rs_r, off, 0, 0));
           if constexpr (ORIG) to[k] = __builtin_bit_cast(f32x4, __builtin_amdgcn_raw_buffer_load_b128(rs_o, off, 0, 0));
         }
       }
@@ -431,7 +571,7 @@
         if constexpr ((EPT || EPN) && !split_out) {
           load_consts();
 #pragma unroll
-          for (int k = 0; k < PT; ++k) tprefetch(k);
+          for (int k = 0; k < PT; ++k) tprefetch((PRE && EPN) ? 64 + k : k);
         } else {
 #pragma unroll
           for (int g = 0; g < PD; ++g) prefetch(g);
@@ -567,14 +707,15 @@
         const f32x4 nbv = *reinterpret_cast<const f32x4*>(ncs + FFN_D + col);
         static_for<16>([&](auto I_) {
           constexpr int i = decltype(I_)::value, k = 16 * ps + i;
-          tprefetch(k + PT);
+          if constexpr (!PRE) tprefetch(k + PT);
           const int row = 2 * i + plr;
           const f32x4 a = *reinterpret_cast<const f32x4*>(tb + row * 128 + ((plc ^ (row & 7)) * 4));
 #pragma unroll
           for (int e = 0; e < 4; ++e) {
-            const float x = tq[k][e] + (a[e] + bb[e]);
+            const float x = PRE ? a[e] + bb[e] : tq[k][e] + (a[e] + bb[e]);
             const float d = x - nbv[e];
-            ssr[i] += d * d;
+            if constexpr (PRE) ssr[i] = __builtin_fmaf(d, d, ssr[i]);
+            else ssr[i] += d * d;
             out[4 * ps + (i >> 2)][4 * (i & 3) + e] = x;
           }
           if constexpr ((i & 3) == 3) asm volatile("" : "+a"(out[4 * ps + (i >> 2)]));
@@ -620,7 +761,8 @@
 #pragma unroll
           for (int e = 0; e < 4; ++e) {
             const float o = tq[64 + k][e];
-            y[e] = o + (out[4 * ps + (i >> 2)][4 * (i & 3) + e] * ssr[i] - o) * byv[e];
+            if constexpr (PRE) y[e] = __builtin_fmaf(__builtin_fmaf(out[4 * ps + (i >> 2)][4 * (i & 3) + e], ssr[i], -o), byv[e], o);
+            else y[e] = o + (out[4 * ps + (i >> 2)][4 * (i & 3) + e] * ssr[i] - o) * byv[e];
           }
           int fo = i * tstep, ho = i * hstep;
           asm volatile("" : "+s"(fo), "+s"(ho));
@@ -685,10 +827,11 @@
         const f32x4 n1 = *reinterpret_cast<const f32x4*>(nbc + n + 4);
 #pragma unroll
         for (int e = 0; e < 4; ++e) {
-          v[e] = rr[g][0][e] + (v[e] + b0[e]);
-          v[4 + e] = rr[g][1][e] + (v[4 + e] + b1[e]);
+          v[e] = PRE ? v[e] + b0[e] : rr[g][0][e] + (v[e] + b0[e]);
+          v[4 + e] = PRE ? v[4 + e] + b1[e] : rr[g][1][e] + (v[4 + e] + b1[e]);
           const float d0 = v[e] - n0[e], d1 = v[4 + e] - n1[e];
-          ss += d0 * d0 + d1 * d1;
+          if constexpr (PRE) ss = __builtin_fmaf(d1, d1, __builtin_fmaf(d0, d0, ss));
+          else ss += d0 * d0 + d1 * d1;
           out[j][8 * pp + e] = v[e];
           out[j][8 * pp + 4 + e] = v[4 + e];
         }
@@ -721,8 +864,13 @@
         float y[8];
 #pragma unroll
         for (int e = 0; e < 4; ++e) {
-          y[e] = rq[g][0][e] + (out[j][8 * pp + e] * scale - rq[g][0][e]) * c0v[e];
-          y[4 + e] = rq[g][1][e] + (out[j][8 * pp + 4 + e] * scale - rq[g][1][e]) * c1v[e];
+          if constexpr (PRE) {
+            y[e] = __builtin_fmaf(__builtin_fmaf(out[j][8 * pp + e], scale, -rq[g][0][e]), c0v[e], rq[g][0][e]);
+            y[4 + e] = __builtin_fmaf(__builtin_fmaf(out[j][8 * pp + 4 + e], scale, -rq[g][1][e]), c1v[e], rq[g][1][e]);
+          } else {
+            y[e] = rq[g][0][e] + (out[j][8 * pp + e] * scale - rq[g][0][e]) * c0v[e];
+            y[4 + e] = rq[g][1][e] + (out[j][8 * pp + 4 + e] * scale - rq[g][1][e]) * c1v[e];
+          }
         }
         const long o = (long)m * p.ldc + n, oh = (long)m * p.ldch + n;
         GLOBAL f32x4* ca = adr32(Cp, o);
@@ -791,7 +939,7 @@
           const f32x4 a = *reinterpret_cast<const f32x4*>(tb + row * 128 + ((lc ^ (row & 7)) * 4));
           f32x4 v;
 #pragma unroll
-          for (int e = 0; e < 4; ++e) v[e] = tq[k][e] + (a[e] + bb[e]);
+          for (int e = 0; e < 4; ++e) v[e] = PRE ? a[e] + bb[e] : tq[k][e] + (a[e] + bb[e]);
           const int mrow = t0 + row;
           if constexpr (RV) {
             const bool second = row >= rv_bnd;
@@ -803,7 +951,8 @@
           }
           if constexpr (ORIG) {
 #pragma unroll
-            for (int e = 0; e < 4; ++e) v[e] = to[k][e] + (v[e] - to[k][e]) * sc4[e];
+            for (int e = 0; e < 4; ++e)
+              v[e] = PRE ? __builtin_fmaf(v[e] - to[k][e], sc4[e], to[k][e]) : to[k][e] + (v[e] - to[k][e]) * sc4[e];
           }
           __builtin_amdgcn_raw_buffer_store_b128(__builtin_bit_cast(v4u32_t, v), rs_c, toff + i * tstep + ps * 512, 0, 0);
           if constexpr (COPY) {
@@ -833,8 +982,8 @@
         const f32x4 b1 = *reinterpret_cast<const f32x4*>(p.b2 + n + 4);
 #pragma unroll
         for (int e = 0; e < 4; ++e) {
-          v[e] = rr[g][0][e] + (v[e] + b0[e]);
-          v[4 + e] = rr[g][1][e] + (v[4 + e] + b1[e]);
+          v[e] = PRE ? v[e] + b0[e] : rr[g][0][e] + (v[e] + b0[e]);
+          v[4 + e] = PRE ? v[4 + e] + b1[e] : rr[g][1][e] + (v[4 + e] + b1[e]);
         }
         if constexpr (RV) {
           const f32x4 w0 = *reinterpret_cast<const f32x4*>(vrow + n);
@@ -914,6 +1063,34 @@
   const int jb = (int)(r & 15), c = (int)(r >> 4);
   out[i] = W[(long)(32 * jb + (l & 31)) * ldw + 32 * c + 16 * s + 8 * (j >> 2) + 4 * (l >> 5) + (j & 3)];
 }
+static __global__ void zv_ffn_pack_w1p_kernel(const bf16* W, long ldw, int H, bf16* out) {
+  const long i = blockIdx.x * 256L + threadIdx.x;
+  if (i >= (long)H * FFN_D) return;
+  const int j = (int)(i & 7);
+  long r = i >> 3;
+  const int l = (int)(r & 63); r >>= 6;
+  const int s = (int)(r & 31), c = (int)(r >> 5);
+  out[i] = W[(long)(32 * c + (l & 31)) * ldw + 16 * s + 8 * (j >> 2) + 4 * (l >> 5) + (j & 3)];
+}
+static __global__ void zv_ffn_pack_wp_kernel(const bf16* W, long ldw, int K, int nkp, bf16* out) {
+  const long i = blockIdx.x * 256L + threadIdx.x;
+  if (i >= (long)nkp * FFN_HC * FFN_D) return;
+  const int j = (int)(i & 7);
+  long r = i >> 3;
+  const int l = (int)(r & 63); r >>= 6;
+  const int s = (int)(r & 1); r >>= 1;
+  const int jb = (int)(r & 15), kc = (int)(r >> 4);
+  const int k = 32 * kc + 16 * s + 8 * (l >> 5) + j;
+  out[i] = k < K ? W[(long)(32 * jb + (l & 31)) * ldw + k] : (bf16)0.f;
+}
+inline int ffn_pre_chunks(int K) { return (K + FFN_HC - 1) / FFN_HC; }
+static void ffn_pack_pre_weights(const Linear& L1, int H, bf16* w1fp, const Linear& Lp, bf16* wpf, hipStream_t s) {
+  const long n = (long)H * FFN_D, np = (long)ffn_pre_chunks(Lp.K) * FFN_HC * FFN_D;
+  hipLaunchKernelGGL(zv_ffn_pack_w1p_kernel, dim3(cdiv(n, 256)), dim3(256), 0, s, L1.hi, (long)L1.Kpad, H, w1fp);
+  hipLaunchKernelGGL(zv_ffn_pack_wp_kernel, dim3(cdiv(np, 256)), dim3(256), 0, s, Lp.hi, (long)Lp.Kpad, Lp.K,
+                     ffn_pre_chunks(Lp.K), wpf);
+  ZV_LAUNCH_CHECK();
+}
 static void ffn_pack_weights(const Linear& L1, const Linear& L2, int H, bf16* w1f, bf16* w2f, hipStream_t s) {
   const long n = (long)H * FFN_D;
   hipLaunchKernelGGL(zv_ffn_pack_w1_kernel, dim3(cdiv(n, 256)), dim3(256), 0, s, L1.hi, (long)L1.Kpad, H, w1f);
@@ -930,12 +1107,12 @@
   return {(int)w, (int)((W + w - 1) / w)};
 }
 
-template <bool RV, bool ORIG, bool COPY, int ABL = 0, int NORM = 0, bool TP = true>
+template <bool RV, bool ORIG, bool COPY, int ABL = 0, int NORM = 0, bool TP = true, bool PRE = false>
 static void launch_ffn_t(const FfnParams& p, int blocks, hipStream_t s, const char* tag) {
   static unsigned long long attr = 0;
   const size_t lds = ffn_lds_bytes(p.H, NORM != 0);
   if (!((attr >> zv_cur_device()) & 1)) {
-    ZV_CHECK(hipFuncSetAttribute((const void*)zv_ffn_kernel<RV, ORIG, COPY, ABL, NORM, TP>,
+    ZV_CHECK(hipFuncSetAttribute((const void*)zv_ffn_kernel<RV, ORIG, COPY, ABL, NORM, TP, PRE>,
                                  hipFuncAttributeMaxDynamicSharedMemorySize, 160 * 1024));
     attr |= 1ull << zv_cur_device();
   }
@@ -946,12 +1123,13 @@
     if (NORM) extra += (double)g.M * FFN_D * ((g.Cl ? 2 : 0) + (g.C2h ? 2 : 0) + (g.C2l ? 2 : 0));
   }
   const double outs = M * FFN_D;
-  const double bytes = outs * 2 + 2.0 * FFN_D * p.H * 2 +
+  const double Kp = PRE ? (double)p.nkp * FFN_HC : 0.0;
+  const double bytes = (PRE ? (M + FFN_D) * Kp * 2 : outs * 2) + 2.0 * FFN_D * p.H * 2 +
                        (NORM ? outs * (4 + 4 + 4 + 2) + extra : outs * (8 + (COPY ? 2 : 0) + (ORIG ? 4 : 0)));
-  g_zv_last_launch = ZvLaunchRec{FFN_BM, FFN_D, 1, (int)RV | (int)ORIG << 1 | (int)COPY << 2 | (int)TP << 3, NORM,
+  g_zv_last_launch = ZvLaunchRec{FFN_BM, FFN_D, 1, (int)RV | (int)ORIG << 1 | (int)COPY << 2 | (int)TP << 3 | (int)PRE << 4, NORM,
                                  0, blocks, p.w};
-  ZvProfScope prof(tag, 4.0 * M * FFN_D * (double)p.H, bytes, s);
-  hipLaunchKernelGGL((zv_ffn_kernel<RV, ORIG, COPY, ABL, NORM, TP>), dim3(blocks), dim3(256), lds, s, p);
+  ZvProfScope prof(tag, 4.0 * M * FFN_D * (double)p.H + 2.0 * M * FFN_D * Kp, bytes, s);
+  hipLaunchKernelGGL((zv_ffn_kernel<RV, ORIG, COPY, ABL, NORM, TP, PRE>), dim3(blocks), dim3(256), lds, s, p);
   ZV_LAUNCH_CHECK();
 }
 
@@ -960,14 +1138,18 @@
   ZV_REQUIRE(p.H > 0 && p.H % (2 * FFN_HC) == 0 && ffn_lds_bytes(p.H, p.nb != nullptr) <= 160 * 1024,
              "fused FeedForward: hidden width a multiple of 64 (LDS: at most 8160, 2496 with the BiasNorm epilogue)");
   ZV_REQUIRE(p.nseg >= 1 && p.nseg <= FFN_MAXSEG, "fused FeedForward: 1..4 row ranges");
-  ZV_REQUIRE(p.W1f && p.W2f && p.b1 && p.b2 && p.ldx % 8 == 0 && p.ldx >= FFN_D && p.ldc % 4 == 0 &&
+  ZV_REQUIRE(p.W1f && p.W2f && p.b1 && p.b2 && (p.Wpf || (p.ldx % 8 == 0 && p.ldx >= FFN_D)) && p.ldc % 4 == 0 &&
                  p.ldc >= FFN_D && (p.ldch == 0 || (p.ldch % 8 == 0 && p.ldch >= FFN_D)),
              "fused FeedForward operands (16-B aligned rows of at least 512)");
   const bool rv = p.seg[0].rowvec != nullptr, og = p.seg[0].orig != nullptr, cp = p.seg[0].Ch != nullptr;
+  const bool pre = p.Wpf != nullptr;
+  ZV_REQUIRE(!pre || (p.bp && p.nkp >= 1 && p.lda >= (long)p.nkp * FFN_HC && p.lda % 8 == 0 && cp && og),
+             "fused FeedForward pre-projection operands (lda >= Kp, 16-B aligned rows, the bypass or BiasNorm site)");
   int R = 0;
   for (int i = 0; i < p.nseg; ++i) {
     FfnSeg& g = p.seg[i];
-    ZV_REQUIRE(g.M > 0 && g.X && g.resid && g.C && (g.Ch != nullptr) == cp && (g.rowvec != nullptr) == rv &&
+    ZV_REQUIRE(!pre || g.A, "fused FeedForward pre-projection operand");
+    ZV_REQUIRE(g.M > 0 && (g.X || pre) && g.resid && g.C && (g.Ch != nullptr) == cp && (g.rowvec != nullptr) == rv &&
                    (g.orig != nullptr) == og && (!g.Ch || p.ldch > 0),
                "fused FeedForward row range operands");
     g.rb0 = R;
@@ -993,11 +1175,20 @@
                  "fused FeedForward + BiasNorm operands");
     ZV_REQUIRE(p.byp, "fused FeedForward + BiasNorm bypass");
     p.norm_scale = expf(p.log_scale);
-    if (p.seg[0].rowvec && p.rows_per_group < 32) launch_ffn_t<false, false, true, 0, 1, false>(p, sc.blocks, s, tag);
-    else launch_ffn_t<false, false, true, 0, 1>(p, sc.blocks, s, tag);
+    const bool tp = !(p.seg[0].rowvec && p.rows_per_group < 32);
+    if (pre) {
+      if (tp) launch_ffn_t<false, false, true, 0, 1, true, true>(p, sc.blocks, s, tag);
+      else launch_ffn_t<false, false, true, 0, 1, false, true>(p, sc.blocks, s, tag);
+    } else if (tp) launch_ffn_t<false, false, true, 0, 1>(p, sc.blocks, s, tag);
+    else launch_ffn_t<false, false, true, 0, 1, false>(p, sc.blocks, s, tag);
     return;
   }
   if constexpr (ABL != 0) { launch_ffn_t<false, false, true, ABL>(p, sc.blocks, s, tag); return; }
+  if (pre) {
+    ZV_REQUIRE(og && cp, "fused FeedForward pre-projection: the bypass site");
+    launch_ffn_t<false, true, true, 0, 0, true, true>(p, sc.blocks, s, tag);
+    return;
+  }
   if (!rv && !og && cp) launch_ffn_t<false, false, true>(p, sc.blocks, s, tag);
   else if (!rv && !og && !cp) launch_ffn_t<false, false, false>(p, sc.blocks, s, tag);
   else if (rv && !og && cp) {
diff --git a/zipvoice_amd/engine.py b/zipvoice_amd/engine.py
--- a/zipvoice_amd/engine.py
+++ b/zipvoice_amd/engine.py
@@ -60,7 +60,8 @@
         ("C", ctypes.c_void_p), ("ldc", ctypes.c_int64),
         ("Ch", ctypes.c_void_p), ("Cl", ctypes.c_void_p), ("C2h", ctypes.c_void_p), ("C2l", ctypes.c_void_p),
         ("ldch", ctypes.c_int64),
-        ("launch", ctypes.c_int * 8), ("num_cus", ctypes.c_int)]
+        ("launch", ctypes.c_int * 8), ("num_cus", ctypes.c_int),
+        ("K", ctypes.c_int), ("A", ctypes.c_void_p), ("Wp", ctypes.c_void_p), ("bp", ctypes.c_void_p)]
 
 
 class ZvDwconvCheckArgs(ctypes.Structure):
```
